# Terence-23/RayTracing-in-a-weekend

Measured on AMD Instinct MI355X. Metric: Msamples/s (rays x bounces) at 1920x1080x500spp, higher is better.
Workload: dtype f32

## Files before the change

### include/rtw.h

```cpp
#ifndef RTW_H
#define RTW_H

#include <stdint.h>
#include <stddef.h>

#ifdef __cplusplus
extern "C" {
#endif

#define RTW_ABI_VERSION 4

#define RTW_OK              0
#define RTW_E_INVALID      -1
#define RTW_E_NO_DEVICE    -2
#define RTW_E_HIP          -3
#define RTW_E_NOMEM        -4
#define RTW_E_UNSUPPORTED  -5
#define RTW_E_NO_SCENE     -6
#define RTW_E_INTERNAL     -7
#define RTW_E_RUNTIME_CONFLICT -8

enum {
    RTW_INTEGRATOR_GRADIENT = 0,
    RTW_INTEGRATOR_BG_COLOR = 1,
// ... 12 lines not shown
};

enum {
    RTW_ACCEL_BRUTE = 0,
    RTW_ACCEL_BVH   = 1
};


typedef struct RtwCamera {
    float origin[3];
    float u[3];
    float v[3];
    float pixel00[3];
    float delta_u[3];
    float delta_v[3];
    float lens_radius;
    float time0;
    float shutter;
} RtwCamera;

typedef struct RtwSphere {
    float center[3];
    float radius;
    float velocity[3];
    float col_mod[3];
    float tex_color[3];
    float metallicness;
    float opacity;
    float ir;
    float emitted[3];
    int32_t tex;
} RtwSphere;

typedef struct RtwTexture {
    uint32_t row;
    uint32_t col;
    uint32_t texel_offset;
    uint32_t emit_tex;
} RtwTexture;

typedef struct RtwQuad {
    float origin[3];
    float u[3];
    float v[3];
    float velocity[3];
    float tex_color[3];
    float metallicness;
    float opacity;
    float ir;
    float emitted[3];
    int32_t tex;
} RtwQuad;

enum { RTW_MEDIUM_SURFACE = 0, RTW_MEDIUM_CONST_DENSITY = 1 };
typedef struct RtwInstance {
    uint32_t first_sphere, n_spheres;
    uint32_t first_quad, n_quads;
    float translation[3];
    float rotation[3];
    float density;
    uint32_t medium;
} RtwInstance;

typedef struct RtwScene {
    const RtwSphere  *spheres;
    const RtwTexture *textures;
    const float      *texels;
    uint32_t n_spheres;
    uint32_t n_textures;
    uint32_t n_texels;
    float    background[3];
    const RtwQuad     *quads;
    const RtwInstance *instances;
    const RtwSphere   *inst_spheres;
    const RtwQuad     *inst_quads;
    uint32_t n_quads;
    uint32_t n_instances;
    uint32_t n_inst_spheres;
    uint32_t n_inst_quads;
} RtwScene;

typedef struct RtwParams {
    uint32_t width, height;
    uint32_t samples;
    uint32_t depth;
    float    gamma;
    float    mint, maxt;
    uint32_t integrator;
    uint32_t sampler;
    uint32_t accel;
    uint32_t flags;
    uint64_t seed;
    uint32_t row_block;
    uint32_t part_index;
    uint32_t part_count;
    uint32_t reserved;
} RtwParams;

#define RTW_FLAG_NONE            0u
#define RTW_FLAG_RECURSIVE_ORDER 1u
#define RTW_FLAG_CPP_DIELECTRIC  2u
#define RTW_FLAG_GLOBAL_NODES    4u
#define RTW_FLAG_CPP_DIFFUSE     8u
#define RTW_FLAG_CHUNK_SUMS     16u
#define RTW_SUM_CHUNK            4u
#define RTW_FLAG_MIXED_MATERIAL 32u

typedef struct RtwStats {
    uint64_t camera_rays;
    uint64_t segments;
    uint64_t sphere_tests;
    uint64_t node_tests;
    uint32_t nan_pixels;
    uint32_t rows;
    float    kernel_ms;
    float    total_ms;
    uint64_t phase_steps[6];
    uint64_t phase_lanes[6];
    uint64_t quad_tests;
    float    enqueue_ms;
    float    start_ms;
} RtwStats;

typedef struct rtw_ctx rtw_ctx;


int         rtw_abi_version(void);
int         rtw_device_count(void);
const char *rtw_strerror(int status);
int         rtw_last_hip_error(void);
int         rtw_hip_runtime_count(void);

int  rtw_ctx_create(int device, rtw_ctx **out);
void rtw_ctx_destroy(rtw_ctx *ctx);
int  rtw_ctx_set_stream(rtw_ctx *ctx, void *hip_stream);
int  rtw_ctx_set_scene(rtw_ctx *ctx, const RtwScene *scene, float t_begin, float t_end);
int  rtw_ctx_render(rtw_ctx *ctx, const RtwCamera *cam, const RtwParams *params,
                    float *out_rgb, RtwStats *stats);
int  rtw_ctx_render_multi(rtw_ctx *ctx, const RtwCamera *cam, const RtwParams *params, float fps,
                          uint32_t start_frame, uint32_t n_frames, float *out_rgb, RtwStats *stats);
int  rtw_render(const RtwCamera *cam, const RtwScene *scene, const RtwParams *params,
                float *out_rgb, RtwStats *stats);

enum {
    RTW_OPT_CHUNK_LEN        = 1,
    RTW_OPT_SAMPLE_BANK_GB   = 2,
    RTW_OPT_LDS_GEOM         = 3,
    RTW_OPT_BLOCKS_PER_CU    = 4,
    RTW_OPT_LIST_WALK_MAX    = 5,
    RTW_OPT_TILE_ORDER       = 6,
    RTW_OPT_GRAB_BLOCKS      = 7,
    RTW_OPT_TAIL_UNITS       = 9,
    RTW_OPT_SUB_QUEUES       = 8,
    RTW_OPT_GUIDED_LAYOUT    = 10
};
int  rtw_ctx_set_option(rtw_ctx *ctx, uint32_t key, double value);

typedef struct rtw_mgpu rtw_mgpu;
int  rtw_mgpu_create(const int *devices, uint32_t n_devices, rtw_mgpu **out);
void rtw_mgpu_destroy(rtw_mgpu *m);
int  rtw_mgpu_set_scene(rtw_mgpu *m, const RtwScene *scene, float t_begin, float t_end);
int  rtw_mgpu_set_option(rtw_mgpu *m, uint32_t key, double value);
int  rtw_mgpu_render(rtw_mgpu *m, const RtwCamera *cam, const RtwParams *params, float *out_rgb,
                     RtwStats *per_device, RtwStats *total);
int  rtw_render_multi_gpu(const int *devices, uint32_t n_devices, const RtwCamera *cam, const RtwScene *scene,
                          const RtwParams *params, float *out_rgb, RtwStats *per_device);

typedef struct RtwPerlin {
    float   ranvec[256][3];
    uint8_t perm_x[256], perm_y[256], perm_z[256];
} RtwPerlin;
typedef struct RtwTextureNoise {
    int32_t perlin;
    float   scale;
} RtwTextureNoise;
int rtw_perlin_new(uint64_t seed, RtwPerlin *out);
int rtw_perlin_eval(const RtwPerlin *t, const float *points, uint32_t n, uint32_t turb_depth, float *out);
int rtw_ctx_perlin_eval(rtw_ctx *ctx, const RtwPerlin *t, const float *points, uint32_t n, uint32_t turb_depth, float *out);
int rtw_ctx_set_texture_noise(rtw_ctx *ctx, const RtwPerlin *tables, uint32_t n_tables,
                              const RtwTextureNoise *per_texture, uint32_t n_textures);
int rtw_mgpu_set_texture_noise(rtw_mgpu *m, const RtwPerlin *tables, uint32_t n_tables,
                               const RtwTextureNoise *per_texture, uint32_t n_textures);

#define RTW_BILATERAL_MAX_SIZE 64u
enum { RTW_PROXIMITY_SQUARE = 0, RTW_PROXIMITY_EDGES = 1 };
enum { RTW_PIXELS_U8 = 0,
       RTW_PIXELS_F32_RUST2 = 1 };
typedef struct RtwBilateral {
    uint32_t size;
    uint32_t proximity;
    uint32_t in_format;
    float    avg_gradient;
} RtwBilateral;
typedef struct RtwFilterStats {
    float    avg_gradient;
    float    spatial;
    float    gradient_ms;
    float    table_ms;
    float    filter_ms;
    float    total_ms;
    uint64_t taps;
} RtwFilterStats;
int rtw_bilateral_filter(const void *in, uint32_t w, uint32_t h, const RtwBilateral *params, uint8_t *out, RtwFilterStats *stats);
int rtw_ctx_bilateral_filter(rtw_ctx *ctx, const void *in, uint32_t w, uint32_t h, const RtwBilateral *params, uint8_t *out,
                             RtwFilterStats *stats);

typedef struct RtwGuidedFilter {
    RtwBilateral base;
    float    sigma_depth;
    float    sigma_normal;
    uint32_t same_object;
} RtwGuidedFilter;
int rtw_guided_filter(const void *in, uint32_t w, uint32_t h, const float *depth, const float *normal, const int32_t *idx,
                      const RtwGuidedFilter *params, uint8_t *out, RtwFilterStats *stats);
int rtw_ctx_guided_filter(rtw_ctx *ctx, const void *in, uint32_t w, uint32_t h, const float *depth, const float *normal,
                          const int32_t *idx, const RtwGuidedFilter *params, uint8_t *out, RtwFilterStats *stats);

typedef struct RtwTriangle {
    float origin[3];
    float u[3];
    float v[3];
    float normal[3];
    float d;
    float w[3];
    float tex_color[3];
    float metallicness;
    float opacity;
    float ir;
    float emitted[3];
    int32_t tex;
} RtwTriangle;
int rtw_triangle_new(const float origin[3], const float u[3], const float v[3], const float *mat3, const float *emitted,
                     const float color[3], int32_t tex, RtwTriangle *out);
int rtw_ctx_set_triangles(rtw_ctx *ctx, const RtwTriangle *tris, uint32_t n);
int rtw_mgpu_set_triangles(rtw_mgpu *m, const RtwTriangle *tris, uint32_t n);
int rtw_triangle_bvh_validate(const RtwTriangle *tris, uint32_t n, uint32_t *n_nodes, uint32_t *depth, uint32_t *list_walk);
int rtw_triangle_hits(const RtwTriangle *tris, uint32_t n, const float *rays, uint32_t n_rays, float mint, float maxt,
                      float *t_out, int32_t *idx_out);
int rtw_ctx_triangle_hits(rtw_ctx *ctx, const float *rays, uint32_t n_rays, float mint, float maxt, uint32_t accel,
                          float *t_out, int32_t *idx_out, RtwStats *stats);

int rtw_depth_rays(const RtwCamera *cam, uint32_t width, uint32_t height, float *rays_out );
int rtw_ctx_scene_hits(rtw_ctx *ctx, const float *rays, uint32_t n_rays, float time, float mint, float maxt, uint32_t accel,
                       float *t_out, int32_t *idx_out, float *normal_out, RtwStats *stats);
int rtw_ctx_depth_map(rtw_ctx *ctx, const RtwCamera *cam, uint32_t width, uint32_t height, float time, float mint, float maxt,
                      uint32_t accel, float *depth_out, int32_t *idx_out, float *normal_out, RtwStats *stats);

#define RTW_MAX_LIGHTS 16u
enum { RTW_LIGHT_SPHERE = 0, RTW_LIGHT_QUAD = 1 };
typedef struct RtwLight {
    uint32_t kind;
    uint32_t index;
} RtwLight;
int rtw_ctx_set_lights(rtw_ctx *ctx, const RtwLight *lights, uint32_t n, float biased_weight);
int rtw_mgpu_set_lights(rtw_mgpu *m, const RtwLight *lights, uint32_t n, float biased_weight);
int rtw_lights_validate(const RtwScene *scene, const RtwLight *lights, uint32_t n);
int rtw_light_mid(const RtwScene *scene, const RtwLight *light, float mid[3]);
float rtw_material_pdf(const float mat3[3], const float p[3], const float n[3], const float dir_in[3], float time_in,
                       const float ray_o[3], const float ray_d[3], float ray_time);
int rtw_light_term(uint32_t integrator, float pdf, const float e[3], float t, const float dir[3], float biased_weight, float S[3], float *count);

int rtw_mixed_validate(const RtwScene *scene, const RtwParams *params, uint32_t n_triangles, uint32_t texture_noise);
int rtw_mixed_dir(float exp, float xi_phi, float xi_cos, const float n[3], float out_dir[3]);
int rtw_mixed_pdf(float exp, const float p[3], const float n[3], const float dir_in[3], const float ray_o[3], const float ray_d[3], float *out);
int rtw_pow_plain(const float *x, const float *y, size_t n, float *out);
int rtw_exp_plain(const float *x, size_t n, float *out);
int rtw_sin_plain(const float *phi, size_t n, float *out);
int rtw_cos_plain(const float *phi, size_t n, float *out);

int rtw_ctx_set_instance_rotations(rtw_ctx *ctx, const float (*quat)[4] , uint32_t n);
int rtw_mgpu_set_instance_rotations(rtw_mgpu *m, const float (*quat)[4], uint32_t n);
int rtw_instance_rotations_validate(const RtwScene *scene, const float (*quat)[4], uint32_t n);
int rtw_quat_rotate(const float q[4], const float v[3], float out[3]);
int rtw_quat_mul(const float a[4], const float b[4], float out[4]);
int rtw_quat_from_axis(float angle, const float axis[3], float out[4]);
int rtw_quat_from_euler(const float euler[3], float out[4]);


int rtw_viewport_new(uint32_t width, float aspect_ratio, const float *vfov, const float *origin,
                     const float *direction, const float *vup, const float *lens_radius,
                     RtwCamera *cam, uint32_t *height);
int rtw_viewport_new_from_res(uint32_t width, uint32_t height, const float *vfov, const float *origin,
                              const float *direction, const float *vup, const float *lens_radius,
                              RtwCamera *cam, uint32_t *height_out);
int rtw_camera2_new(float aspect, const float origin[3], const float vup[3], const float dir[3], float vfov,
                    float lens_radius, RtwCamera *cam);
int rtw_sphere_new(const float origin[3], float radius, const float *col_mod,
                   const float *mat3 , const float *velocity,
                   RtwSphere *out);
int rtw_sphere_new_with_texture(const float origin[3], float radius, const float *col_mod,
                                const float *mat3, const float *velocity, int32_t tex, RtwSphere *out);
int rtw_quad_new(const float origin[3], const float u[3], const float v[3], const float *mat3,
                 const float *emitted, const float color[3], RtwQuad *out);
int rtw_box_quads(const float a[3], const float b[3], const float *mat3, const float color[3], RtwQuad quads6[6]);
void rtw_vec3_rotated(const float v[3], const float rot[3], float out[3]);
int rtw_tile_order(uint32_t mode, uint32_t width, uint32_t height, const RtwCamera *cam, const RtwScene *scene,
                   uint32_t *order, uint32_t cap);
uint32_t rtw_part_rows(uint32_t height, uint32_t row_block, uint32_t part_index, uint32_t part_count);
void rtw_quantize_u8(const float *rgb, size_t n_values, uint8_t *out);
void rtw_quantize_u8_rust2(const float *rgb, size_t n_values, uint8_t *out);

size_t rtw_scene_to_json(const RtwScene *scene, char *buf, size_t cap);
int rtw_scene_from_json(const char *text, size_t len,
                        RtwSphere *spheres, uint32_t sphere_cap, uint32_t *n_spheres,
                        RtwTexture *textures, uint32_t texture_cap, uint32_t *n_textures,
                        float *texels, uint32_t texel_cap, uint32_t *n_texels);
int rtw_write_png_f32(const char *path, const float *rgb, uint32_t width, uint32_t height);
int rtw_write_ppm_f32(const char *path, const float *rgb, uint32_t width, uint32_t height);

// ... 31 lines not shown
```

### raytracing-in-a-weekend_amd/__init__.py

```python
from __future__ import annotations

import ctypes as C
import os
from typing import Optional, Sequence

import numpy as np

_HERE = os.path.dirname(os.path.abspath(__file__))
LIB_PATH = os.environ.get("RTW_HIP_LIB", os.path.join(_HERE, "librtw_hip.so"))

RTW_OK = 0
INTEGRATOR_GRADIENT, INTEGRATOR_BG_COLOR, INTEGRATOR_NORMAL, INTEGRATOR_FLAG, INTEGRATOR_RUST2 = 0, 1, 2, 3, 4
INTEGRATOR_LIGHT_CAST, INTEGRATOR_LIGHT_BIASED = 5, 6
LIGHT_SPHERE, LIGHT_QUAD = 0, 1
MAX_LIGHTS = 16
SAMPLER_ROW, SAMPLER_STRATIFIED, SAMPLER_CENTRES, SAMPLER_NO_RAND = 0, 1, 2, 3
ACCEL_BRUTE, ACCEL_BVH = 0, 1
FLAG_RECURSIVE_ORDER, FLAG_CPP_DIELECTRIC, FLAG_GLOBAL_NODES, FLAG_CPP_DIFFUSE, FLAG_CHUNK_SUMS = 1, 2, 4, 8, 16
FLAG_CPP = FLAG_CPP_DIELECTRIC | FLAG_CPP_DIFFUSE
FLAG_MIXED_MATERIAL = 32
OPT_CHUNK_LEN, OPT_SAMPLE_BANK_GB, OPT_LDS_GEOM, OPT_BLOCKS_PER_CU, OPT_LIST_WALK_MAX, OPT_TILE_ORDER, OPT_GRAB_BLOCKS, OPT_SUB_QUEUES = 1, 2, 3, 4, 5, 6, 7, 8
OPT_TAIL_UNITS = 9
OPT_GUIDED_LAYOUT = 10
SCENE_C1, SCENE_C2, SCENE_C4, SCENE_C5, SCENE_METAL_TEST, SCENE_QUAD_TEST, SCENE_PRESENTATION, SCENE_FIRST_FRAME = 1, 2, 4, 5, 6, 7, 8, 9
MEDIUM_SURFACE, MEDIUM_CONST_DENSITY = 0, 1
PROXIMITY_SQUARE, PROXIMITY_EDGES = 0, 1
PIXELS_U8, PIXELS_F32_RUST2 = 0, 1
BILATERAL_MAX_SIZE = 64

METALLIC_M = (1.0, 0.0, 1.0)
SCATTER_M = (0.0, 0.0, 1.0)
FUZZY3_M = (0.7, 0.0, 1.0)
GLASS_M = (1.0, 1.0, 1.5)
GLASSR_M = (1.0, 1.0, float(np.float32(1.0) / np.float32(1.5)))
EMPTY_M = SCATTER_M


class RtwError(RuntimeError):
    def __init__(self, status: int, what: str):
        super().__init__(f"{what}: status {status} ({_strerror(status)})")
        self.status = status


class RtwCamera(C.Structure):
    _fields_ = [("origin", C.c_float * 3), ("u", C.c_float * 3), ("v", C.c_float * 3),
                ("pixel00", C.c_float * 3), ("delta_u", C.c_float * 3), ("delta_v", C.c_float * 3),
                ("lens_radius", C.c_float), ("time0", C.c_float), ("shutter", C.c_float)]


class RtwSphere(C.Structure):
    _fields_ = [("center", C.c_float * 3), ("radius", C.c_float), ("velocity", C.c_float * 3),
                ("col_mod", C.c_float * 3), ("tex_color", C.c_float * 3),
                ("metallicness", C.c_float), ("opacity", C.c_float), ("ir", C.c_float),
                ("emitted", C.c_float * 3), ("tex", C.c_int32)]


class RtwTexture(C.Structure):
    _fields_ = [("row", C.c_uint32), ("col", C.c_uint32), ("texel_offset", C.c_uint32), ("emit_tex", C.c_uint32)]


class RtwQuad(C.Structure):
    _fields_ = [("origin", C.c_float * 3), ("u", C.c_float * 3), ("v", C.c_float * 3), ("velocity", C.c_float * 3),
                ("tex_color", C.c_float * 3), ("metallicness", C.c_float), ("opacity", C.c_float), ("ir", C.c_float),
                ("emitted", C.c_float * 3), ("tex", C.c_int32)]


class RtwTriangle(C.Structure):
    _fields_ = [("origin", C.c_float * 3), ("u", C.c_float * 3), ("v", C.c_float * 3), ("normal", C.c_float * 3), ("d", C.c_float),
                ("w", C.c_float * 3), ("tex_color", C.c_float * 3), ("metallicness", C.c_float), ("opacity", C.c_float), ("ir", C.c_float),
                ("emitted", C.c_float * 3), ("tex", C.c_int32)]


class RtwLight(C.Structure):
    _fields_ = [("kind", C.c_uint32), ("index", C.c_uint32)]


class RtwInstance(C.Structure):
    _fields_ = [("first_sphere", C.c_uint32), ("n_spheres", C.c_uint32), ("first_quad", C.c_uint32), ("n_quads", C.c_uint32),
                ("translation", C.c_float * 3), ("rotation", C.c_float * 3), ("density", C.c_float), ("medium", C.c_uint32)]


class RtwScene(C.Structure):
    _fields_ = [("spheres", C.POINTER(RtwSphere)), ("textures", C.POINTER(RtwTexture)),
                ("texels", C.POINTER(C.c_float)), ("n_spheres", C.c_uint32), ("n_textures", C.c_uint32),
                ("n_texels", C.c_uint32), ("background", C.c_float * 3),
                ("quads", C.POINTER(RtwQuad)), ("instances", C.POINTER(RtwInstance)),
                ("inst_spheres", C.POINTER(RtwSphere)), ("inst_quads", C.POINTER(RtwQuad)),
                ("n_quads", C.c_uint32), ("n_instances", C.c_uint32), ("n_inst_spheres", C.c_uint32), ("n_inst_quads", C.c_uint32)]


class RtwParams(C.Structure):
    _fields_ = [("width", C.c_uint32), ("height", C.c_uint32), ("samples", C.c_uint32), ("depth", C.c_uint32),
                ("gamma", C.c_float), ("mint", C.c_float), ("maxt", C.c_float),
                ("integrator", C.c_uint32), ("sampler", C.c_uint32), ("accel", C.c_uint32), ("flags", C.c_uint32),
                ("seed", C.c_uint64),
                ("row_block", C.c_uint32), ("part_index", C.c_uint32), ("part_count", C.c_uint32), ("reserved", C.c_uint32)]


class RtwStats(C.Structure):
    _fields_ = [("camera_rays", C.c_uint64), ("segments", C.c_uint64), ("sphere_tests", C.c_uint64),
                ("node_tests", C.c_uint64), ("nan_pixels", C.c_uint32), ("rows", C.c_uint32),
                ("kernel_ms", C.c_float), ("total_ms", C.c_float),
                ("phase_steps", C.c_uint64 * 6), ("phase_lanes", C.c_uint64 * 6), ("quad_tests", C.c_uint64),
                ("enqueue_ms", C.c_float), ("start_ms", C.c_float)]

    def as_dict(self):
        return {k: (list(getattr(self, k)) if k.startswith("phase_") else getattr(self, k)) for k, _ in self._fields_}


class RtwPerlin(C.Structure):
    _fields_ = [("ranvec", (C.c_float * 3) * 256), ("perm_x", C.c_uint8 * 256), ("perm_y", C.c_uint8 * 256), ("perm_z", C.c_uint8 * 256)]


class RtwTextureNoise(C.Structure):
    _fields_ = [("perlin", C.c_int32), ("scale", C.c_float)]


class RtwBilateral(C.Structure):
    _fields_ = [("size", C.c_uint32), ("proximity", C.c_uint32), ("in_format", C.c_uint32), ("avg_gradient", C.c_float)]


class RtwGuidedFilter(C.Structure):
    _fields_ = [("base", RtwBilateral), ("sigma_depth", C.c_float), ("sigma_normal", C.c_float), ("same_object", C.c_uint32)]


class RtwFilterStats(C.Structure):
    _fields_ = [("avg_gradient", C.c_float), ("spatial", C.c_float), ("gradient_ms", C.c_float), ("table_ms", C.c_float),
                ("filter_ms", C.c_float), ("total_ms", C.c_float), ("taps", C.c_uint64)]

    def as_dict(self):
        return {k: getattr(self, k) for k, _ in self._fields_}


_lib = None


def lib() -> C.CDLL:
    global _lib
    if _lib is not None:
        return _lib
    if not os.path.exists(LIB_PATH):
        raise ImportError(f"{LIB_PATH} is missing: run `python -c 'import __graft_entry__ as g; g.build()'` "
                          f"(hipcc --offload-arch=gfx950); there is no CPU fallback")
    L = C.CDLL(LIB_PATH)
    fp = C.POINTER(C.c_float)
    L.rtw_abi_version.restype = C.c_int
    L.rtw_device_count.restype = C.c_int
    L.rtw_strerror.restype = C.c_char_p
    L.rtw_strerror.argtypes = [C.c_int]
    L.rtw_last_hip_error.restype = C.c_int
    L.rtw_ctx_create.argtypes = [C.c_int, C.POINTER(C.c_void_p)]
    L.rtw_ctx_destroy.argtypes = [C.c_void_p]
    L.rtw_ctx_destroy.restype = None
    L.rtw_ctx_set_stream.argtypes = [C.c_void_p, C.c_void_p]
    L.rtw_ctx_set_scene.argtypes = [C.c_void_p, C.POINTER(RtwScene), C.c_float, C.c_float]
    L.rtw_ctx_render.argtypes = [C.c_void_p, C.POINTER(RtwCamera), C.POINTER(RtwParams), C.c_void_p, C.POINTER(RtwStats)]
    L.rtw_ctx_render_multi.argtypes = [C.c_void_p, C.POINTER(RtwCamera), C.POINTER(RtwParams), C.c_float, C.c_uint32, C.c_uint32,
                                       C.c_void_p, C.POINTER(RtwStats)]
    L.rtw_render.argtypes = [C.POINTER(RtwCamera), C.POINTER(RtwScene), C.POINTER(RtwParams), C.c_void_p, C.POINTER(RtwStats)]
    L.rtw_ctx_set_option.argtypes = [C.c_void_p, C.c_uint32, C.c_double]
    L.rtw_mgpu_create.argtypes = [C.POINTER(C.c_int), C.c_uint32, C.POINTER(C.c_void_p)]
    L.rtw_mgpu_destroy.argtypes = [C.c_void_p]
    L.rtw_mgpu_destroy.restype = None
    L.rtw_mgpu_set_scene.argtypes = [C.c_void_p, C.POINTER(RtwScene), C.c_float, C.c_float]
    L.rtw_mgpu_set_option.argtypes = [C.c_void_p, C.c_uint32, C.c_double]
    L.rtw_mgpu_render.argtypes = [C.c_void_p, C.POINTER(RtwCamera), C.POINTER(RtwParams), C.c_void_p, C.POINTER(RtwStats), C.POINTER(RtwStats)]
    L.rtw_render_multi_gpu.argtypes = [C.POINTER(C.c_int), C.c_uint32, C.POINTER(RtwCamera), C.POINTER(RtwScene), C.POINTER(RtwParams),
                                       C.c_void_p, C.POINTER(RtwStats)]
    L.rtw_viewport_new.argtypes = [C.c_uint32, C.c_float, fp, fp, fp, fp, fp, C.POINTER(RtwCamera), C.POINTER(C.c_uint32)]
    L.rtw_viewport_new_from_res.argtypes = [C.c_uint32, C.c_uint32, fp, fp, fp, fp, fp, C.POINTER(RtwCamera), C.POINTER(C.c_uint32)]
    L.rtw_sphere_new.argtypes = [fp, C.c_float, fp, fp, fp, C.POINTER(RtwSphere)]
    L.rtw_sphere_new_with_texture.argtypes = [fp, C.c_float, fp, fp, fp, C.c_int32, C.POINTER(RtwSphere)]
    L.rtw_vec3_rotated.restype = None
    L.rtw_vec3_rotated.argtypes = [fp, fp, fp]
    L.rtw_tile_order.argtypes = [C.c_uint32, C.c_uint32, C.c_uint32, C.POINTER(RtwCamera), C.POINTER(RtwScene), C.POINTER(C.c_uint32), C.c_uint32]
    L.rtw_part_rows.restype = C.c_uint32
    L.rtw_part_rows.argtypes = [C.c_uint32] * 4
    L.rtw_quantize_u8.restype = None
    L.rtw_quantize_u8.argtypes = [fp, C.c_size_t, C.POINTER(C.c_uint8)]
    L.rtw_camera2_new.argtypes = [C.c_float, fp, fp, fp, C.c_float, C.c_float, C.POINTER(RtwCamera)]
    L.rtw_quantize_u8_rust2.restype = None
    L.rtw_quantize_u8_rust2.argtypes = [fp, C.c_size_t, C.POINTER(C.c_uint8)]
    L.rtw_scene_to_json.restype = C.c_size_t
    L.rtw_scene_to_json.argtypes = [C.POINTER(RtwScene), C.c_char_p, C.c_size_t]
    L.rtw_scene_from_json.argtypes = [C.c_char_p, C.c_size_t, C.POINTER(RtwSphere), C.c_uint32, C.POINTER(C.c_uint32),
                                      C.POINTER(RtwTexture), C.c_uint32, C.POINTER(C.c_uint32), fp, C.c_uint32, C.POINTER(C.c_uint32)]
    L.rtw_write_png_f32.argtypes = [C.c_char_p, fp, C.c_uint32, C.c_uint32]
    L.rtw_write_ppm_f32.argtypes = [C.c_char_p, fp, C.c_uint32, C.c_uint32]
    L.rtw_bvh_validate.argtypes = [C.POINTER(RtwScene), C.c_float, C.c_float] + [C.POINTER(C.c_uint32)] * 4
    L.rtw_bvh_dump.argtypes = [C.POINTER(RtwScene), C.c_float, C.c_float, C.c_void_p, C.c_uint32, C.POINTER(C.c_uint32), C.POINTER(C.c_int32),
                               C.POINTER(C.c_uint32), C.POINTER(C.c_uint32), C.c_void_p, C.c_uint32, C.POINTER(C.c_uint32), C.c_void_p]
    L.rtw_bvh_query_host.argtypes = [C.POINTER(RtwScene), C.c_float, C.c_float, C.c_void_p, C.c_uint32, C.c_float, C.c_float, C.c_float,
                                     C.c_uint32, C.c_void_p, C.c_void_p, C.c_void_p]
    L.rtw_scene_generate.argtypes = [C.c_uint32, C.c_uint64, C.POINTER(RtwSphere), C.c_uint32, C.POINTER(C.c_uint32),
                                     C.POINTER(RtwTexture), C.c_uint32, C.POINTER(C.c_uint32),
                                     fp, C.c_uint32, C.POINTER(C.c_uint32)]
    L.rtw_scene_default_view.argtypes = [C.c_uint32, C.POINTER(RtwCamera), C.POINTER(RtwParams)]
    L.rtw_quad_new.argtypes = [fp, fp, fp, fp, fp, fp, C.POINTER(RtwQuad)]
    L.rtw_box_quads.argtypes = [fp, fp, fp, fp, C.POINTER(RtwQuad)]
    L.rtw_scene_generate_geom.argtypes = [C.c_uint32, C.c_uint64, C.POINTER(RtwSphere), C.POINTER(RtwQuad), C.POINTER(RtwInstance),
                                          C.POINTER(RtwSphere), C.POINTER(RtwQuad), C.POINTER(C.c_uint32), C.POINTER(C.c_uint32), fp]
    L.rtw_perlin_new.argtypes = [C.c_uint64, C.POINTER(RtwPerlin)]
    L.rtw_perlin_eval.argtypes = [C.POINTER(RtwPerlin), fp, C.c_uint32, C.c_uint32, fp]
    L.rtw_ctx_perlin_eval.argtypes = [C.c_void_p, C.POINTER(RtwPerlin), fp, C.c_uint32, C.c_uint32, fp]
    L.rtw_ctx_set_texture_noise.argtypes = [C.c_void_p, C.POINTER(RtwPerlin), C.c_uint32, C.POINTER(RtwTextureNoise), C.c_uint32]
    L.rtw_mgpu_set_texture_noise.argtypes = [C.c_void_p, C.POINTER(RtwPerlin), C.c_uint32, C.POINTER(RtwTextureNoise), C.c_uint32]
    L.rtw_bilateral_filter.argtypes = [C.c_void_p, C.c_uint32, C.c_uint32, C.POINTER(RtwBilateral), C.c_void_p, C.POINTER(RtwFilterStats)]
    L.rtw_ctx_bilateral_filter.argtypes = [C.c_void_p, C.c_void_p, C.c_uint32, C.c_uint32, C.POINTER(RtwBilateral), C.c_void_p,
                                           C.POINTER(RtwFilterStats)]
    L.rtw_guided_filter.argtypes = [C.c_void_p, C.c_uint32, C.c_uint32, C.c_void_p, C.c_void_p, C.c_void_p, C.POINTER(RtwGuidedFilter), C.c_void_p,
                                    C.POINTER(RtwFilterStats)]
    L.rtw_ctx_guided_filter.argtypes = [C.c_void_p, C.c_void_p, C.c_uint32, C.c_uint32, C.c_void_p, C.c_void_p, C.c_void_p,
                                        C.POINTER(RtwGuidedFilter), C.c_void_p, C.POINTER(RtwFilterStats)]
    L.rtw_triangle_new.argtypes = [fp, fp, fp, fp, fp, fp, C.c_int32, C.POINTER(RtwTriangle)]
    L.rtw_ctx_set_triangles.argtypes = [C.c_void_p, C.POINTER(RtwTriangle), C.c_uint32]
    L.rtw_mgpu_set_triangles.argtypes = [C.c_void_p, C.POINTER(RtwTriangle), C.c_uint32]
    L.rtw_triangle_bvh_validate.argtypes = [C.POINTER(RtwTriangle), C.c_uint32] + [C.POINTER(C.c_uint32)] * 3
    L.rtw_triangle_hits.argtypes = [C.POINTER(RtwTriangle), C.c_uint32, fp, C.c_uint32, C.c_float, C.c_float, fp, C.POINTER(C.c_int32)]
    L.rtw_ctx_triangle_hits.argtypes = [C.c_void_p, fp, C.c_uint32, C.c_float, C.c_float, C.c_uint32, fp, C.POINTER(C.c_int32),
                                        C.POINTER(RtwStats)]
    L.rtw_depth_rays.argtypes = [C.POINTER(RtwCamera), C.c_uint32, C.c_uint32, fp]
    L.rtw_ctx_scene_hits.argtypes = [C.c_void_p, C.c_void_p, C.c_uint32, C.c_float, C.c_float, C.c_float, C.c_uint32, C.c_void_p, C.c_void_p,
                                     C.c_void_p, C.POINTER(RtwStats)]
    L.rtw_ctx_depth_map.argtypes = [C.c_void_p, C.POINTER(RtwCamera), C.c_uint32, C.c_uint32, C.c_float, C.c_float, C.c_float, C.c_uint32,
                                    C.c_void_p, C.c_void_p, C.c_void_p, C.POINTER(RtwStats)]
    L.rtw_ctx_set_lights.argtypes = [C.c_void_p, C.POINTER(RtwLight), C.c_uint32, C.c_float]
    L.rtw_mgpu_set_lights.argtypes = [C.c_void_p, C.POINTER(RtwLight), C.c_uint32, C.c_float]
    L.rtw_lights_validate.argtypes = [C.POINTER(RtwScene), C.POINTER(RtwLight), C.c_uint32]
    L.rtw_light_mid.argtypes = [C.POINTER(RtwScene), C.POINTER(RtwLight), fp]
    L.rtw_material_pdf.argtypes = [fp, fp, fp, fp, C.c_float, fp, fp, C.c_float]
    L.rtw_material_pdf.restype = C.c_float
    L.rtw_light_term.argtypes = [C.c_uint32, C.c_float, fp, C.c_float, fp, C.c_float, fp, fp]
    L.rtw_mixed_validate.argtypes = [C.POINTER(RtwScene), C.POINTER(RtwParams), C.c_uint32, C.c_uint32]
    L.rtw_mixed_dir.argtypes = [C.c_float, C.c_float, C.c_float, fp, fp]
    L.rtw_mixed_pdf.argtypes = [C.c_float, fp, fp, fp, fp, fp, fp]
    L.rtw_ctx_set_instance_rotations.argtypes = [C.c_void_p, fp, C.c_uint32]
    L.rtw_mgpu_set_instance_rotations.argtypes = [C.c_void_p, fp, C.c_uint32]
    L.rtw_instance_rotations_validate.argtypes = [C.POINTER(RtwScene), fp, C.c_uint32]
    L.rtw_quat_rotate.argtypes = [fp, fp, fp]
    L.rtw_quat_mul.argtypes = [fp, fp, fp]
    L.rtw_quat_from_axis.argtypes = [C.c_float, fp, fp]
    L.rtw_quat_from_euler.argtypes = [fp, fp]
    L.rtw_pow_plain.argtypes = [fp, fp, C.c_size_t, fp]
    L.rtw_sin_plain.argtypes = [fp, C.c_size_t, fp]
    L.rtw_exp_plain.argtypes = [fp, C.c_size_t, fp]
    L.rtw_cos_plain.argtypes = [fp, C.c_size_t, fp]
    _lib = L
    return L


def _strerror(status: int) -> str:
    try:
        return lib().rtw_strerror(status).decode()
    except Exception:
        return "?"


def _check(status: int, what: str):
    if status != RTW_OK:
        raise RtwError(status, what)


def _f3(v) -> Optional[C.Array]:
    if v is None:
        return None
    return (C.c_float * 3)(*[float(x) for x in v])


def _fptr(arr):
    return None if arr is None else C.cast(arr, C.POINTER(C.c_float))


def _f1(v):
    return None if v is None else C.pointer(C.c_float(float(v)))


class Sphere:

    def __init__(self, pod: RtwSphere):
        self.pod = pod

    @staticmethod
    def new(origin, r, col_mod=None, mat=None) -> "Sphere":
        s = RtwSphere()
        _check(lib().rtw_sphere_new(_fptr(_f3(origin)), float(r), _fptr(_f3(col_mod)), _fptr(_f3(mat)), None, C.byref(s)), "rtw_sphere_new")
        return Sphere(s)

    @staticmethod
    def new_moving(origin, r, col_mod, mat, velocity) -> "Sphere":
        s = RtwSphere()
        _check(lib().rtw_sphere_new(_fptr(_f3(origin)), float(r), _fptr(_f3(col_mod)), _fptr(_f3(mat)), _fptr(_f3(velocity)), C.byref(s)), "rtw_sphere_new")
        return Sphere(s)

    @staticmethod
    def new_with_texture(origin, r, col_mod, mat, tex_index: int, velocity=None) -> "Sphere":
        s = RtwSphere()
        _check(lib().rtw_sphere_new_with_texture(_fptr(_f3(origin)), float(r), _fptr(_f3(col_mod)), _fptr(_f3(mat)),
                                                 _fptr(_f3(velocity)), int(tex_index), C.byref(s)), "rtw_sphere_new_with_texture")
        return Sphere(s)

    @staticmethod
    def with_albedo(origin, r, albedo, mat=None, velocity=None) -> "Sphere":
        sp = Sphere.new_moving(origin, r, (1.0, 1.0, 1.0), mat, velocity or (0.0, 0.0, 0.0))
        for k in range(3):
            sp.pod.tex_color[k] = float(albedo[k])
        return sp


class Quad:

    def __init__(self, pod: RtwQuad):
        self.pod = pod

# ... 388 lines not shown
    def new_sphere(spheres: Sequence) -> "Scene":
        return Scene(spheres)

    @staticmethod
    def new_quad(quads: Sequence) -> "Scene":
        return Scene((), quads=quads)

    @staticmethod
    def new(spheres: Sequence, quads: Sequence, instances: Sequence) -> "Scene":
        return Scene(spheres, quads=quads, instances=instances)

    @staticmethod
    def generate_geom(which: int, scene_seed: int = 42) -> "Scene":
        L = lib()
        counts = (C.c_uint32 * 5)()
        bg = (C.c_float * 3)()
        _check(L.rtw_scene_generate_geom(which, scene_seed, None, None, None, None, None, None, counts, bg), "rtw_scene_generate_geom")
        n = [int(x) for x in counts]
        sp, qd, ins = (RtwSphere * max(1, n[0]))(), (RtwQuad * max(1, n[1]))(), (RtwInstance * max(1, n[2]))()
        isp, iqd = (RtwSphere * max(1, n[3]))(), (RtwQuad * max(1, n[4]))()
        caps = (C.c_uint32 * 5)(*n)
        _check(L.rtw_scene_generate_geom(which, scene_seed, sp, qd, ins, isp, iqd, caps, counts, bg), "rtw_scene_generate_geom")
        sc = Scene(list(sp)[:n[0]], background=tuple(bg))
        sc._install_geom(list(qd)[:n[1]], list(ins)[:n[2]], list(isp)[:n[3]], list(iqd)[:n[4]])
        return sc

    def noise_pods(self):
        if not self.noise:
            return None
        tables, index = [], {}
        per = (RtwTextureNoise * max(1, self.n_textures))(*[RtwTextureNoise(-1, 1.0) for _ in range(max(1, self.n_textures))])
        for t, (perlin, scale) in self.noise.items():
            if not 0 <= int(t) < self.n_textures:
                raise RtwError(-1, f"noise for texture {t}: the scene has {self.n_textures} textures")
            if id(perlin) not in index:
                index[id(perlin)] = len(tables)
                tables.append(perlin.pod)
            per[int(t)] = RtwTextureNoise(index[id(perlin)], float(scale))
        tb = (RtwPerlin * len(tables))(*tables)
        return tb, len(tables), per, self.n_textures

    def to_json(self) -> str:
        n = lib().rtw_scene_to_json(C.byref(self.pod), None, 0)
        buf = C.create_string_buffer(n + 1)
        lib().rtw_scene_to_json(C.byref(self.pod), buf, n + 1)
        return buf.value.decode()

    @staticmethod
    def from_json(text: str) -> "Scene":
        L = lib()
        raw = text.encode()
        ns, nt, nx = C.c_uint32(), C.c_uint32(), C.c_uint32()
        _check(L.rtw_scene_from_json(raw, len(raw), None, 0, C.byref(ns), None, 0, C.byref(nt), None, 0, C.byref(nx)), "rtw_scene_from_json")
        sp = (RtwSphere * max(1, ns.value))()
        tx = (RtwTexture * max(1, nt.value))()
        tl = np.zeros((max(1, nx.value), 3), np.float32)
        _check(L.rtw_scene_from_json(raw, len(raw), sp, ns.value, C.byref(ns), tx, nt.value, C.byref(nt),
                                     tl.ctypes.data_as(C.POINTER(C.c_float)), nx.value, C.byref(nx)), "rtw_scene_from_json")
        return Scene._from_arrays(sp, ns.value, tx, nt.value, tl, nx.value)

    @staticmethod
    def _from_arrays(sp, ns, tx, nt, tl, nx) -> "Scene":
        sc = Scene(list(sp)[:ns])
        sc._textures, sc.n_textures, sc._texels, sc.n_texels = tx, nt, tl, nx
        sc.pod.textures = C.cast(tx, C.POINTER(RtwTexture))
        sc.pod.texels = tl.ctypes.data_as(C.POINTER(C.c_float))
        sc.pod.n_textures, sc.pod.n_texels = nt, nx
        return sc

    @staticmethod
    def generate(which: int, scene_seed: int = 42) -> "Scene":
        L = lib()
        ns, nt, nx = C.c_uint32(), C.c_uint32(), C.c_uint32()
        _check(L.rtw_scene_generate(which, scene_seed, None, 0, C.byref(ns), None, 0, C.byref(nt), None, 0, C.byref(nx)), "rtw_scene_generate")
        sp = (RtwSphere * max(1, ns.value))()
        tx = (RtwTexture * max(1, nt.value))()
        tl = np.zeros((max(1, nx.value), 3), np.float32)
        _check(L.rtw_scene_generate(which, scene_seed, sp, ns.value, C.byref(ns), tx, nt.value, C.byref(nt),
                                    tl.ctypes.data_as(C.POINTER(C.c_float)), nx.value, C.byref(nx)), "rtw_scene_generate")
        return Scene._from_arrays(sp, ns.value, tx, nt.value, tl, nx.value)


class Viewport:

    def __init__(self, cam: RtwCamera, width: int, height: int, samples: int, depth: int, gamma: float):
        self.cam, self.width, self.height = cam, width, height
        self.samples, self.depth, self.gamma = samples, depth, gamma
        self.shutter_speed, self.fps, self.frame = 0.0, 30.0, 0
        self.seed = 1
        self.mint, self.maxt = 0.001, 100000.0
        self.flags = 0

    @staticmethod
    def new(width, aspect_ratio, samples, depth, gamma, vfov=None, origin=None, direction=None, vup=None, msg=None, lens_radius=None):
        cam, h = RtwCamera(), C.c_uint32()
        _check(lib().rtw_viewport_new(int(width), float(aspect_ratio), _f1(vfov), _fptr(_f3(origin)), _fptr(_f3(direction)),
                                      _fptr(_f3(vup)), _f1(lens_radius), C.byref(cam), C.byref(h)), "rtw_viewport_new")
        return Viewport(cam, int(width), h.value, samples, depth, gamma)

    @staticmethod
    def new_from_res(width, height, samples, depth, gamma, vfov=None, origin=None, direction=None, vup=None, msg=None, lens_radius=None):
        cam, h = RtwCamera(), C.c_uint32()
        _check(lib().rtw_viewport_new_from_res(int(width), int(height), _f1(vfov), _fptr(_f3(origin)), _fptr(_f3(direction)),
                                               _fptr(_f3(vup)), _f1(lens_radius), C.byref(cam), C.byref(h)), "rtw_viewport_new_from_res")
        return Viewport(cam, int(width), h.value, samples, depth, gamma)

    def params(self, integrator=INTEGRATOR_GRADIENT, sampler=SAMPLER_STRATIFIED, accel=ACCEL_BVH) -> RtwParams:
        p = RtwParams()
        p.width, p.height, p.samples, p.depth = self.width, self.height, self.samples, self.depth
        p.gamma, p.mint, p.maxt = self.gamma, self.mint, self.maxt
        p.integrator, p.sampler, p.accel, p.flags, p.seed = integrator, sampler, accel, int(self.flags), self.seed
        p.row_block, p.part_index, p.part_count = 8, 0, 1
        return p

    def camera(self) -> RtwCamera:
        cam = RtwCamera.from_buffer_copy(self.cam)
        cam.time0 = float(np.float32(self.frame) / np.float32(self.fps))
        cam.shutter = float(self.shutter_speed)
        return cam

    def render(self, ray_color: int, scene: Scene, device: int = 0, accel: int = ACCEL_BVH) -> np.ndarray:
        return self._render(ray_color, SAMPLER_STRATIFIED, scene, device, accel)

    def async_render(self, ray_color: int, scene: Scene, device: int = 0, accel: int = ACCEL_BVH) -> np.ndarray:
        return self._render(ray_color, SAMPLER_ROW, scene, device, accel)

    def render_multi(self, ray_color: int, scene: Scene, device: int = 0, accel: int = ACCEL_BVH):
        start = getattr(self, "start_frame", 0)
        count = getattr(self, "number_of_frames", 1)
        with Renderer(device) as r:
            t0 = float(np.float32(start) / np.float32(self.fps))
            t1 = float(np.float32(start + max(count, 1) - 1) / np.float32(self.fps)) + float(self.shutter_speed)
            r.set_scene(scene, t0, t1)
            p = self.params(ray_color, SAMPLER_ROW, accel)
            video = np.empty((max(count, 0), self.height, self.width, 3), np.float32)
            st = (RtwStats * max(count, 1))()
            cam = self.camera()
            _check(lib().rtw_ctx_render_multi(r._h, C.byref(cam), C.byref(p), float(self.fps), int(start), int(count),
                                              C.c_void_p(video.ctypes.data), st), "rtw_ctx_render_multi")
        self.frame = start + max(count, 1) - 1
        return [video[i] for i in range(count)]

    def render_no_rand(self, ray_color: int, scene: Scene, device: int = 0, accel: int = ACCEL_BVH) -> np.ndarray:
        return self._render(ray_color, SAMPLER_NO_RAND, scene, device, accel)

    def _render(self, ray_color, sampler, scene, device, accel):
        with Renderer(device) as r:
            cam = self.camera()
            r.set_scene(scene, cam.time0, cam.time0 + cam.shutter)
            img, _ = r.render(cam, self.params(ray_color, sampler, accel))
        return img


class Renderer:

    def __init__(self, device: int = 0):
        self._h = C.c_void_p()
        _check(lib().rtw_ctx_create(int(device), C.byref(self._h)), "rtw_ctx_create")
        self._scene = None

    def close(self):
        if self._h:
            lib().rtw_ctx_destroy(self._h)
            self._h = C.c_void_p()

    def __enter__(self):
        return self

    def __exit__(self, *a):
        self.close()

    def __del__(self):
        try:
            self.close()
        except Exception:
            pass

    def set_stream(self, hip_stream: int):
        _check(lib().rtw_ctx_set_stream(self._h, C.c_void_p(hip_stream)), "rtw_ctx_set_stream")

    def set_scene(self, scene: Scene, t_begin: float = 0.0, t_end: float = 0.0):
        self._scene = scene
        _check(lib().rtw_ctx_set_scene(self._h, C.byref(scene.pod), float(t_begin), float(t_end)), "rtw_ctx_set_scene")
        nz = scene.noise_pods()
        if nz is not None:
            _check(lib().rtw_ctx_set_texture_noise(self._h, *nz), "rtw_ctx_set_texture_noise")
        if scene.n_triangles:
            _check(lib().rtw_ctx_set_triangles(self._h, scene.triangles, scene.n_triangles), "rtw_ctx_set_triangles")

    def set_triangles(self, triangles=None):
        if triangles is None or len(triangles) == 0:
            _check(lib().rtw_ctx_set_triangles(self._h, None, 0), "rtw_ctx_set_triangles")
            return
        self._tris = _triangle_array(triangles)
        _check(lib().rtw_ctx_set_triangles(self._h, *self._tris), "rtw_ctx_set_triangles")

    def set_lights(self, lights=None, biased_weight: float = 100.0):
        arr, n = _light_array(lights)
        _check(lib().rtw_ctx_set_lights(self._h, arr, n, float(biased_weight)), "rtw_ctx_set_lights")

    def set_instance_rotations(self, quats=None):
        ptr, n, _keep = _quat_array(quats)
        _check(lib().rtw_ctx_set_instance_rotations(self._h, ptr, n), "rtw_ctx_set_instance_rotations")

    def triangle_hits(self, rays, mint: float, maxt: float, accel: int = ACCEL_BVH):
        r = _rays(rays)
        t = np.empty(len(r), np.float32)
        idx = np.empty(len(r), np.int32)
        st = RtwStats()
        _check(lib().rtw_ctx_triangle_hits(self._h, r.ctypes.data_as(C.POINTER(C.c_float)), len(r), float(mint), float(maxt), int(accel),
                                           t.ctypes.data_as(C.POINTER(C.c_float)), idx.ctypes.data_as(C.POINTER(C.c_int32)), C.byref(st)),
               "rtw_ctx_triangle_hits")
        return t, idx, st

    def scene_hits(self, rays, mint: float, maxt: float, time: float = 0.0, accel: int = ACCEL_BVH, normals: bool = False):
        r = _rays(rays)
        t = np.empty(len(r), np.float32)
        idx = np.empty(len(r), np.int32)
        nrm = np.empty((len(r), 3), np.float32) if normals else None
        st = RtwStats()
        _check(lib().rtw_ctx_scene_hits(self._h, r.ctypes.data, len(r), float(time), float(mint), float(maxt), int(accel), t.ctypes.data,
                                        idx.ctypes.data, nrm.ctypes.data if normals else None, C.byref(st)), "rtw_ctx_scene_hits")
        return (t, idx, nrm, st) if normals else (t, idx, st)

    def depth_map(self, cam: RtwCamera, width: int, height: int, mint: float, maxt: float, time: float = 0.0, accel: int = ACCEL_BVH,
                  ids: bool = False, normals: bool = False):
        width, height = int(width), int(height)
        depth = np.empty((height, width), np.float32)
        idx = np.empty((height, width), np.int32) if ids else None
        nrm = np.empty((height, width, 3), np.float32) if normals else None
        st = RtwStats()
        _check(lib().rtw_ctx_depth_map(self._h, C.byref(cam), width, height, float(time), float(mint), float(maxt), int(accel), depth.ctypes.data,
                                       idx.ctypes.data if ids else None, nrm.ctypes.data if normals else None, C.byref(st)), "rtw_ctx_depth_map")
        return (depth,) + ((idx,) if ids else ()) + ((nrm,) if normals else ()) + (st,)

    def set_texture_noise(self, tables=None, n_tables: int = 0, per_texture=None, n_textures: int = 0):
        _check(lib().rtw_ctx_set_texture_noise(self._h, tables, n_tables, per_texture, n_textures), "rtw_ctx_set_texture_noise")

    def perlin_eval(self, perlin: PerlinNoise, p, depth: int = 0) -> np.ndarray:
        pts = np.ascontiguousarray(p, dtype=np.float32).reshape(-1, 3)
        out = np.empty(len(pts), np.float32)
        _check(lib().rtw_ctx_perlin_eval(self._h, C.byref(perlin.pod), pts.ctypes.data_as(C.POINTER(C.c_float)), len(pts), int(depth),
                                         out.ctypes.data_as(C.POINTER(C.c_float))), "rtw_ctx_perlin_eval")
        return out

    def set_option(self, key: int, value: float):
        _check(lib().rtw_ctx_set_option(self._h, int(key), float(value)), "rtw_ctx_set_option")

    def bilateral_filter(self, img, size: int, proximity: int = PROXIMITY_SQUARE, avg_gradient: float = 0.0, out=None, shape=None,
                         in_format: Optional[int] = None):
        src, w, h, fmt, _keep = _filter_source("bilateral_filter", img, shape, in_format)
        out, dst = _filter_out(out, h, w)
        st = RtwFilterStats()
        prm = RtwBilateral(int(size), int(proximity), fmt, float(avg_gradient))
        _check(lib().rtw_ctx_bilateral_filter(self._h, src, w, h, C.byref(prm), dst, C.byref(st)), "rtw_ctx_bilateral_filter")
        return out, st

    def guided_filter(self, img, size: int, depth=None, normal=None, ids=None, sigma_depth: float = 0.0, sigma_normal: float = 0.0,
                      same_object: bool = False, proximity: int = PROXIMITY_SQUARE, avg_gradient: float = 0.0, out=None, shape=None,
                      in_format: Optional[int] = None):
        src, w, h, fmt, _keep = _filter_source("guided_filter", img, shape, in_format)
        guides, _keep_g = _guide_pointers(h, w, depth, normal, ids)
        out, dst = _filter_out(out, h, w)
        st = RtwFilterStats()
        prm = RtwGuidedFilter(RtwBilateral(int(size), int(proximity), fmt, float(avg_gradient)), float(sigma_depth), float(sigma_normal),
                              int(same_object))
        _check(lib().rtw_ctx_guided_filter(self._h, src, w, h, *guides, C.byref(prm), dst, C.byref(st)), "rtw_ctx_guided_filter")
        return out, st

    def render(self, cam: RtwCamera, params: RtwParams, out=None):
        rows = lib().rtw_part_rows(params.height, params.row_block, params.part_index, params.part_count)
        st = RtwStats()
        if out is None:
            out = np.empty((rows, params.width, 3), np.float32)
        if isinstance(out, np.ndarray):
            assert out.dtype == np.float32 and out.flags["C_CONTIGUOUS"] and out.size == rows * params.width * 3
            ptr = C.c_void_p(out.ctypes.data)
        else:
            ptr = C.c_void_p(int(out))
        _check(lib().rtw_ctx_render(self._h, C.byref(cam), C.byref(params), ptr, C.byref(st)), "rtw_ctx_render")
        return out, st


class MultiRenderer:

    def __init__(self, devices: Sequence[int]):
        self._h = C.c_void_p()
        self.n = len(devices)
        arr = (C.c_int * max(1, self.n))(*[int(d) for d in devices])
        _check(lib().rtw_mgpu_create(arr, self.n, C.byref(self._h)), "rtw_mgpu_create")
        self._scene = None

    def close(self):
        if self._h:
            lib().rtw_mgpu_destroy(self._h)
            self._h = C.c_void_p()

    def __enter__(self):
        return self

    def __exit__(self, *a):
        self.close()

    def __del__(self):
        try:
            self.close()
        except Exception:
            pass

    def set_scene(self, scene: Scene, t_begin: float = 0.0, t_end: float = 0.0):
        self._scene = scene
        _check(lib().rtw_mgpu_set_scene(self._h, C.byref(scene.pod), float(t_begin), float(t_end)), "rtw_mgpu_set_scene")
        nz = scene.noise_pods()
        if nz is not None:
            _check(lib().rtw_mgpu_set_texture_noise(self._h, *nz), "rtw_mgpu_set_texture_noise")
        if scene.n_triangles:
            _check(lib().rtw_mgpu_set_triangles(self._h, scene.triangles, scene.n_triangles), "rtw_mgpu_set_triangles")

    def set_triangles(self, triangles=None):
        if triangles is None or len(triangles) == 0:
            _check(lib().rtw_mgpu_set_triangles(self._h, None, 0), "rtw_mgpu_set_triangles")
            return
        self._tris = _triangle_array(triangles)
        _check(lib().rtw_mgpu_set_triangles(self._h, *self._tris), "rtw_mgpu_set_triangles")

    def set_lights(self, lights=None, biased_weight: float = 100.0):
        arr, n = _light_array(lights)
        _check(lib().rtw_mgpu_set_lights(self._h, arr, n, float(biased_weight)), "rtw_mgpu_set_lights")

    def set_instance_rotations(self, quats=None):
        ptr, n, _keep = _quat_array(quats)
        _check(lib().rtw_mgpu_set_instance_rotations(self._h, ptr, n), "rtw_mgpu_set_instance_rotations")

    def set_option(self, key: int, value: float):
        _check(lib().rtw_mgpu_set_option(self._h, int(key), float(value)), "rtw_mgpu_set_option")

    def render(self, cam: RtwCamera, params: RtwParams, out=None):
        if out is None:
            out = np.empty((params.height, params.width, 3), np.float32)
        if isinstance(out, np.ndarray):
            assert out.dtype == np.float32 and out.flags["C_CONTIGUOUS"] and out.size == params.height * params.width * 3
            ptr = C.c_void_p(out.ctypes.data)
        else:
            ptr = C.c_void_p(int(out))
        per = (RtwStats * max(1, self.n))()
        tot = RtwStats()
        _check(lib().rtw_mgpu_render(self._h, C.byref(cam), C.byref(params), ptr, per, C.byref(tot)), "rtw_mgpu_render")
        return out, tot, list(per)[: self.n]


def default_view(which: int):
    cam, p = RtwCamera(), RtwParams()
    _check(lib().rtw_scene_default_view(which, C.byref(cam), C.byref(p)), "rtw_scene_default_view")
    return cam, p


def quantize_u8(img: np.ndarray) -> np.ndarray:
    a = np.ascontiguousarray(img, np.float32)
    out = np.empty(a.shape, np.uint8)
    lib().rtw_quantize_u8(a.ctypes.data_as(C.POINTER(C.c_float)), a.size, out.ctypes.data_as(C.POINTER(C.c_uint8)))
    return out


def camera2_new(aspect, origin, vup, direction, vfov, lens_radius) -> RtwCamera:
    cam = RtwCamera()
    _check(lib().rtw_camera2_new(float(aspect), _fptr(_f3(origin)), _fptr(_f3(vup)), _fptr(_f3(direction)), float(vfov),
                                 float(lens_radius), C.byref(cam)), "rtw_camera2_new")
    return cam


def quantize_u8_rust2(img: np.ndarray) -> np.ndarray:
    a = np.ascontiguousarray(img, np.float32)
    out = np.empty(a.shape, np.uint8)
    lib().rtw_quantize_u8_rust2(a.ctypes.data_as(C.POINTER(C.c_float)), a.size, out.ctypes.data_as(C.POINTER(C.c_uint8)))
    return out


def _pixel_format(img: np.ndarray) -> int:
    if img.dtype == np.uint8:
        return PIXELS_U8
    if img.dtype == np.float32:
        return PIXELS_F32_RUST2
    raise ValueError(f"bilateral_filter: dtype {img.dtype}, expected uint8 or float32")


def _filter_source(what, img, shape, in_format):
    if isinstance(img, np.ndarray):
        fmt = _pixel_format(img) if in_format is None else int(in_format)
        a = np.ascontiguousarray(img, np.uint8 if fmt == PIXELS_U8 else np.float32)
        if a.ndim != 3 or a.shape[2] != 3:
            raise ValueError(f"{what}: image of shape {a.shape}, expected [h][w][3]")
        return C.c_void_p(a.ctypes.data), a.shape[1], a.shape[0], fmt, a
    if shape is None or in_format is None:
        raise ValueError(f"{what}: a device pointer needs shape=(h, w) and in_format")
    h, w = (int(v) for v in shape)
    return C.c_void_p(int(img)), w, h, int(in_format), None


def _filter_out(out, h, w):
    if out is None:
# ... 63 lines not shown
```

### raytracing-in-a-weekend_amd/csrc/rtw_kernels.h

```cpp
#pragma once
#include "rtw_device.h"
#include "rtw_tri.h"
#include "rtw_light.h"
#include "rtw_mixed.h"
#include "rtw_host.h"

#define RTW_QUEUE_BYTES 4096u
#define RTW_QUEUE_STRIDE 256u
#ifndef RTW_SUB_SHIFT
#define RTW_SUB_SHIFT 3u
#endif
#ifndef RTW_BLOCK
#define RTW_BLOCK 256
#endif
#define RTW_N_STATS 64
#ifndef RTW_LIST_WALK_MAX_DEFAULT
#define RTW_LIST_WALK_MAX_DEFAULT 48u
#endif

namespace rtw {

struct DevBvh {
    const BvhNode *nodes;
    const BvhNode16 *nodes16;
    uint32_t n_nodes;
    const f4 *big_geom;
    const f4 *big_vel;
    const uint32_t *big_index;
    uint32_t n_big;
    uint32_t depth;
    int32_t root;
    float cx, cy, cz;
    float centre_radius;
    float r_max2;
    float inv_2rmin;
    float abs_max;
};

struct KArgs {
    RtwCamera cam;
    DevScene  sc;
    DevBvh    bvh;
    DevGeom   geom;
    uint32_t width, height;
    uint32_t k_base, k_end;
    uint32_t n_tiles;
    uint32_t chunk_len, n_chunks;
    uint32_t bank_len;
    uint32_t reg_q1, reg_q2;
    uint32_t reg_len[3], reg_nc[3];
    uint32_t flags;
    float *samples;
    uint32_t row_block, part_index, part_count;
    uint32_t tiles_x;
    uint32_t total_work;
    uint32_t sub_shift;
    uint32_t grab_shift, grab_max;
    const uint32_t *tile_order;
    uint32_t n_samples;
    uint32_t s_root;
    uint32_t sampler, integrator, depth;
    uint32_t has_textures;
    uint32_t lds_bytes;
    uint32_t lds_stack_off, lds_geom_off;
    uint32_t seed_lo, seed_hi;
    float inv_gamma, mint, maxt;
    float bg[3];
    float *out;
    uint32_t *queue;
    unsigned long long endtimes_ref;
    unsigned long long *stats;
    DevNoise noise;
    DevTris tris;
    DevLights lights;
    const f4 *inst_quats;
};

void launch_render(const KArgs &a, bool moving, uint32_t accel, uint32_t grid, hipStream_t stream);
void launch_perlin_eval(const RtwPerlin *t, const float *points, uint32_t n, uint32_t depth, float *out, hipStream_t stream);
void launch_tri_hits(const DevTris &T, const float *rays, uint32_t n, float mint, float maxt, float *t_out, int32_t *idx_out,
                     unsigned long long *counters, hipStream_t stream);
struct QueryArgs {
    DevScene sc;
    DevBvh   bvh;
    DevGeom  geom;
    DevTris  tris;
    const f4 *inst_quats;
    RtwCamera cam;
    uint32_t width, height;
    const float *rays;
    uint32_t n;
    uint32_t levels;
    float time, mint, maxt;
    float miss_t;
    float span;
    float *t_out;
    int32_t *idx_out;
    float *normal_out;
    unsigned long long *counters;
};
#define RTW_QUERY_SLOTS 64u
#define RTW_QUERY_STRIDE 16u
void launch_scene_hits(const QueryArgs &q, bool from_camera, bool tree, hipStream_t stream);
uint32_t kernel_blocks_per_cu(const KArgs &a, bool moving, uint32_t accel, bool lds_nodes);
bool kernel_has_lds_geom(const KArgs &a);
const void *kernel_id(const KArgs &a, bool moving, uint32_t accel, bool lds_nodes);

}
```

### raytracing-in-a-weekend_amd/csrc/rtw_kernels.hip

```cpp
#include "rtw_kernels.h"
#include <type_traits>

#ifndef RTW_MAX_TRIPS
#define RTW_MAX_TRIPS 0x30000000u
#endif

namespace rtw {


constexpr bool gradient_spec(int spec) { return spec >= 1 && spec <= 3; }
constexpr bool generic_spec(int spec) { return spec == 0 || spec == 7 || spec == 8 || spec == 9 || spec == 10 || spec == 11; }
constexpr bool light_spec(int spec) { return spec == 9 || spec == 10 || spec == 11; }
constexpr int mixed_spec(int spec) { return spec == 10 ? 1 : spec == 11 ? 2 : 0; }
constexpr bool quat_spec(int spec) { return spec == 11; }
constexpr bool noise_spec(int spec) { return spec == 7; }
constexpr bool tri_spec(int spec) { return spec == 8; }
template <int SPEC> __device__ __forceinline__ uint32_t integ(const KArgs &A) {
    return SPEC == 5 ? (uint32_t)RTW_INTEGRATOR_RUST2 : SPEC == 4 ? (uint32_t)RTW_INTEGRATOR_BG_COLOR : !generic_spec(SPEC) ? (uint32_t)RTW_INTEGRATOR_GRADIENT : A.integrator;
}
template <int SPEC> __device__ __forceinline__ uint32_t samp(const KArgs &A) {
    return SPEC == 6 ? (uint32_t)RTW_SAMPLER_STRATIFIED : SPEC == 5 ? (uint32_t)RTW_SAMPLER_CENTRES : !generic_spec(SPEC) ? (uint32_t)RTW_SAMPLER_ROW : A.sampler;
}

struct Pixel {
    uint32_t ij;
    uint32_t rng_base;
    uint32_t s;
    uint32_t slot;
};
__device__ __forceinline__ uint32_t px_i(const Pixel &px) { return px.ij & 0xFFFFu; }
__device__ __forceinline__ uint32_t px_j(const Pixel &px) { return px.ij >> 16; }
__device__ __forceinline__ uint32_t px_s(const Pixel &px) { return px.s & 0xFFFFFFu; }
__device__ __forceinline__ bool px_advance(Pixel &px) { px.s += 1u - (1u << 24); return px.s < (1u << 24); }

struct Path {
    v3 o, d;
    float tm;
    v3 thr;
    v3 L;
    uint32_t k;
    Rng rng;
    bool poison;
};

struct Reserve {
    uint32_t next, end;
    uint32_t limit;
    uint32_t sub, tries;
    uint32_t i0, k0;
    uint32_t s0, s1;
    uint32_t slot0;
#ifdef RTW_ENDTIMES
    unsigned long long t_dry;
#endif
};

struct SubQ { uint32_t t1, t2, b1, b2, total; };
__device__ __forceinline__ SubQ subq_layout(const KArgs &A, uint32_t sub) {
    const uint32_t up = (1u << A.sub_shift) - 1u - sub;
    SubQ q;
    q.t1 = (A.reg_q1 + up) >> A.sub_shift; q.t2 = (A.reg_q2 + up) >> A.sub_shift;
    const uint32_t t3 = (A.n_tiles + up) >> A.sub_shift;
    q.b1 = q.t1 * A.reg_nc[0]; q.b2 = q.b1 + (q.t2 - q.t1) * A.reg_nc[1];
    q.total = (q.b2 + (t3 - q.t2) * A.reg_nc[2]) * 64u;
    return q;
}

__device__ __forceinline__ bool fetch_pixel(const KArgs &A, bool need, Pixel &px, bool &exhausted, Reserve &rs) {
    const unsigned long long m = ballot64(need);
    if (m == 0ull) return false;
    if (rs.next == rs.end) {
        if (rs.end == rs.limit) {
            const uint32_t n_sub = 1u << A.sub_shift;
            const uint32_t leader = (uint32_t)__ffsll((long long)m) - 1u;
            bool got = false;
            while (rs.tries < n_sub) {
                const uint32_t total = subq_layout(A, rs.sub).total;
                uint32_t grab = 64u;
                if (rs.tries == 0u && rs.limit < total) {
                    grab = ((total - rs.limit) >> A.grab_shift) & ~63u;
                    grab = grab > A.grab_max ? A.grab_max : (grab < 64u ? 64u : grab);
                }
                uint32_t base = 0;
                if ((threadIdx.x & 63u) == leader) base = atomicAdd(A.queue + rs.sub * (RTW_QUEUE_STRIDE / 4u), grab);
                base = (uint32_t)__builtin_amdgcn_readlane((int)base, (int)leader);
                if (base < total) {
                    rs.next = base;
                    rs.limit = total - base > grab ? base + grab : total;
                    got = true;
                    break;
                }
                rs.sub = (rs.sub + 1u) & (n_sub - 1u); rs.tries++; rs.limit = 0u;
            }
            if (!got) {
                rs.next = rs.limit = 0u;
#ifdef RTW_ENDTIMES
                if (rs.t_dry == 0ull) rs.t_dry = wall_clock64();
#endif
            }
        }
        rs.end = rs.next + (rs.next < rs.limit ? 64u : 0u);
        if (rs.next < rs.limit) {
            uint32_t u = rs.next >> 6;
            const SubQ sq = subq_layout(A, rs.sub);
            uint32_t lt, chunk, len;
            if (u < sq.b1) { lt = u / A.reg_nc[0]; chunk = u - lt * A.reg_nc[0]; len = A.reg_len[0]; }
            else if (u < sq.b2) { u -= sq.b1; lt = u / A.reg_nc[1]; chunk = u - lt * A.reg_nc[1]; lt += sq.t1; len = A.reg_len[1]; }
            else { u -= sq.b2; lt = u / A.reg_nc[2]; chunk = u - lt * A.reg_nc[2]; lt += sq.t2; len = A.reg_len[2]; }
            const uint32_t qt = (lt << A.sub_shift) + rs.sub;
            const uint32_t tile = A.tile_order ? A.tile_order[qt] : qt;
            const uint32_t trow = tile / A.tiles_x, tcol = tile - trow * A.tiles_x;
            rs.i0 = tcol * 8u;
            rs.k0 = A.k_base + trow * 8u;
            rs.s0 = chunk * len;
            rs.s1 = rs.s0 + len < A.n_samples ? rs.s0 + len : A.n_samples;
            rs.slot0 = (A.bank_len ? tile * A.n_chunks + chunk : tile * A.n_samples + rs.s0) * 64u;
        }
    }
    const uint32_t avail = rs.end - rs.next;
    const uint32_t rank = __builtin_amdgcn_mbcnt_hi((uint32_t)(m >> 32), __builtin_amdgcn_mbcnt_lo((uint32_t)m, 0u));
    const uint32_t w = rs.next + rank;
    const uint32_t cnt = (uint32_t)__popcll(m);
    rs.next += cnt < avail ? cnt : avail;
    if (!need) return false;
    if (avail == 0u) { exhausted = true; return false; }
    if (rank >= avail) return false;
    const uint32_t p = w & 63u;
    const uint32_t i = rs.i0 + (p & 7u);
    const uint32_t k = rs.k0 + (p >> 3);
    if (!(i < A.width && k < A.k_end)) return false;
    uint32_t j = k;
    if (A.part_count > 1) {
        if (A.row_block == 8u) j = ((rs.k0 >> 3) * A.part_count + A.part_index) * 8u + (p >> 3);
        else j = ((k / A.row_block) * A.part_count + A.part_index) * A.row_block + (k % A.row_block);
    }
    px.ij = i | (j << 16);
    px.rng_base = rng_pixel_base(A.seed_lo, A.seed_hi, j * A.width + i);
    px.s = rs.s0 | ((rs.s1 - rs.s0) << 24);
    px.slot = rs.slot0 + (w & 63u);
    return rs.s0 < rs.s1;
}

struct CamRegs { RtwCamera c; };
typedef float f16v __attribute__((ext_vector_type(16)));
typedef float f8v __attribute__((ext_vector_type(8)));
static_assert(sizeof(RtwCamera) == 84 && offsetof(KArgs, cam) == 0, "start_path reads KArgs.cam as 16 + 8 dwords at offset 0");
__device__ __forceinline__ RtwCamera load_camera() {
    f16v lo; f8v hi;
    asm volatile("s_load_dwordx16 %0, %2, 0x0\n\ts_load_dwordx8 %1, %2, 0x40\n\ts_waitcnt lgkmcnt(0)"
                 : "=&s"(lo), "=&s"(hi) : "s"(__builtin_amdgcn_kernarg_segment_ptr()));
    RtwCamera c;
    c.origin[0] = lo[0]; c.origin[1] = lo[1]; c.origin[2] = lo[2]; c.u[0] = lo[3]; c.u[1] = lo[4]; c.u[2] = lo[5];
    c.v[0] = lo[6]; c.v[1] = lo[7]; c.v[2] = lo[8]; c.pixel00[0] = lo[9]; c.pixel00[1] = lo[10]; c.pixel00[2] = lo[11];
    c.delta_u[0] = lo[12]; c.delta_u[1] = lo[13]; c.delta_u[2] = lo[14]; c.delta_v[0] = lo[15]; c.delta_v[1] = hi[0]; c.delta_v[2] = hi[1];
    c.lens_radius = hi[2]; c.time0 = hi[3]; c.shutter = hi[4];
    return c;
}

template <int SPEC>
__device__ __forceinline__ void start_path(const KArgs &A, const Pixel &px, Path &pt, Cen *cn = nullptr) {
    RTW_CEN(cn, CEN_START_PATH);
    const RtwCamera cam = load_camera();
    const v3 cam_o = ld3(cam.origin), p00 = ld3(cam.pixel00), du = ld3(cam.delta_u), dv = ld3(cam.delta_v);
    pt.rng = rng_start(px.rng_base, px_s(px));
    pt.thr = mk(1.0f, 1.0f, 1.0f); pt.L = mk(0, 0, 0); pt.poison = false; pt.k = 0;
    v3 o, d; float tm = 0.0f;
    if (samp<SPEC>(A) == RTW_SAMPLER_NO_RAND) {
        o = cam_o;
        d = (p00 + du * (float)px_i(px)) + dv * (float)px_j(px);
    } else {
        float jx, jy, rx, ry;
        if (samp<SPEC>(A) == RTW_SAMPLER_CENTRES) {
            const uint32_t kx = px_s(px) / A.s_root, ly = px_s(px) % A.s_root;
            jx = ((float)px_i(px) + ((float)kx + 0.5f) / (float)A.s_root) / (float)A.width;
            jy = ((float)px_j(px) + ((float)ly + 0.5f) / (float)A.s_root) / (float)A.height;
            random_in_unit_disk(pt.rng, rx, ry, false, cn);
            o = cam_o + mk(rx, ry, 0.0f) * cam.lens_radius;
        } else {
            random_in_unit_disk(pt.rng, rx, ry, generic_spec(SPEC) && (A.flags & RTW_FLAG_CPP_DIFFUSE), cn);
            o = cam_o + (ld3(cam.u) * rx + ld3(cam.v) * ry) * cam.lens_radius;
            if (samp<SPEC>(A) == RTW_SAMPLER_ROW) {
                jx = rng_offset(pt.rng, (float)px_i(px));
                jy = rng_offset(pt.rng, (float)px_j(px));
                tm = cam.time0 + cam.shutter * rng_f32(pt.rng);
            } else {
                const uint32_t sx = px_s(px) / A.s_root, sy = px_s(px) % A.s_root;
                jx = (float)px_i(px) + (((float)sx + rng_f32(pt.rng)) / (float)A.s_root);
                jy = (float)px_j(px) + (((float)sy + rng_f32(pt.rng)) / (float)A.s_root);
            }
        }
        d = (p00 + du * jx) + dv * jy;
    }
    pt.o = o; pt.d = d; pt.tm = tm;
}

template <int SPEC>
__device__ __forceinline__ void shade_miss(const KArgs &A, Path &pt, v3 ud) {
    v3 miss;
    if (integ<SPEC>(A) == RTW_INTEGRATOR_BG_COLOR || integ<SPEC>(A) == RTW_INTEGRATOR_RUST2) miss = ld3(A.bg);
    else if (integ<SPEC>(A) == RTW_INTEGRATOR_FLAG) miss = mk(0.0f, 0.0f, 1.0f);
    else miss = sky_gradient(ud);
    if (gradient_spec(SPEC)) pt.L = miss * pt.thr;
    else pt.L = pt.L + miss * pt.thr;
}

template <int SPEC>
__device__ __forceinline__ bool shade_surface(const KArgs &A, Path &pt, v3 ud, v3 point, v3 normal, v3 cm, MatP mat, v3 emitted, Cen *cn = nullptr) {
    if (integ<SPEC>(A) == RTW_INTEGRATOR_NORMAL) {
        pt.L = mk(normal.x + 1.0f, normal.y + 1.0f, normal.z + 1.0f) * 0.5f;
        return true;
    }
    if (integ<SPEC>(A) == RTW_INTEGRATOR_FLAG && mat.metallicness != 1.0f) {
        pt.L = mk(1.0f, 1.0f, 0.0f) * pt.thr;
        return true;
    }
    if (integ<SPEC>(A) == RTW_INTEGRATOR_RUST2) {
        const v3 nd2 = on_hit_rust2(mat, normal, pt.d, pt.rng, A.flags);
        pt.L = pt.L + emitted * pt.thr;
        pt.thr = pt.thr * cm;
        pt.o = point; pt.d = nd2;
        pt.k++;
        if (pt.k >= A.depth) { pt.L = pt.L + ld3(A.bg) * pt.thr; return true; }
        return false;
    }
    float cos_theta;
    const v3 nd = on_hit(mat, point, normal, pt.d, ud, pt.rng, cos_theta, generic_spec(SPEC) ? A.flags : 0u, cn);
    if (integ<SPEC>(A) == RTW_INTEGRATOR_BG_COLOR) {
        const float pdf = cos_theta > 0.0f ? cos_theta * 0.318309886183790671538f : 0.0f;
        if (mat.metallicness != 1.0f && !(pdf > 0.0f)) pt.poison = true;
        pt.L = pt.L + emitted * pt.thr;
    }
    pt.thr = pt.thr * cm;
    pt.o = point; pt.d = nd;
    pt.k++;
    if (pt.k >= A.depth) {
        RTW_CEN(cn, CEN_DEPTH_END);
        if (integ<SPEC>(A) != RTW_INTEGRATOR_BG_COLOR) pt.L = mk(0, 0, 0);
        return true;
    }
    return false;
}

template <bool MOVING, int SPEC>
__device__ __forceinline__ bool shade_hit(const KArgs &A, Path &pt, v3 ud, int best, float best_t, Cen *cn = nullptr) {
    RTW_CEN(cn, CEN_HIT);
    const DevScene &sc = A.sc;
    f4 g = sc.geom[best];
    v3 c = mk(g.x, g.y, g.z);
    if (MOVING) { f4 vv = sc.vel[best]; c = c + mk(vv.x, vv.y, vv.z) * pt.tm; }
    const v3 point = pt.o + pt.d * best_t;
    const v3 normal = unit(point - c);
    const DevMat mat = sc.mat[best];
    v3 cm, emitted = ld3(mat.emitted);
    if ((generic_spec(SPEC) || SPEC == 5) && integ<SPEC>(A) == RTW_INTEGRATOR_RUST2 && mat.tex >= 0) rust2_sphere_color(sc, mat, normal, cm, emitted);
    else if constexpr (noise_spec(SPEC)) cm = sphere_albedo_noise(sc, A.noise, mat, normal, point);
    else cm = (SPEC == 1 || SPEC == 3) ? ld3(mat.cm) : sphere_albedo(sc, mat, normal);
    return shade_surface<SPEC>(A, pt, ud, point, normal, cm, mat_params(mat), emitted, cn);
}

template <bool MOVING, int SPEC>
__device__ __forceinline__ bool shade(const KArgs &A, Path &pt, int best, float best_t, Cen *cn = nullptr) {
    RTW_CEN(cn, CEN_INFLIGHT);
    const v3 ud = unit(pt.d);
    if (best < 0) { RTW_CEN(cn, CEN_MISS); shade_miss<SPEC>(A, pt, ud); return true; }
    return shade_hit<MOVING, SPEC>(A, pt, ud, best, best_t, cn);
}

template <bool MOVING, int SPEC>
__device__ __forceinline__ void shade_hit_first(const KArgs &A, Path &pt, v3 ud, int best, float best_t, bool &need_ball, v3 &nrm, float &metal, bool &front, Cen *cn = nullptr) {
    RTW_CEN(cn, CEN_HIT);
// ... 82 lines not shown

template <int MIXED>
__device__ __forceinline__ bool light_walks_on(const KArgs &A) {
    return MIXED ? A.integrator != RTW_INTEGRATOR_LIGHT_CAST : A.integrator == RTW_INTEGRATOR_LIGHT_BIASED;
}
template <int MIXED>
__device__ __forceinline__ bool mixed_surface(const KArgs &A, float opacity) {
    if (MIXED == 2) return (A.flags & RTW_FLAG_MIXED_MATERIAL) != 0u && opacity < 0.0f;
    return MIXED && opacity < 0.0f;
}
template <int MIXED>
__device__ __forceinline__ void light_surface(const KArgs &A, Path &pt, v3 point, v3 normal, v3 cm, const MatP m, v3 emitted, v3 din, LightPath &lp) {
    const bool biased = light_walks_on<MIXED>(A);
    lp.n = normal; lp.din = din; lp.tm = pt.tm;
    lp.metallicness = m.metallicness; lp.opacity = m.opacity; lp.ir = m.ir;
    lp.cm = cm; lp.e = emitted;
    lp.S = mk(0, 0, 0); lp.count = biased ? 1.0f : 0.0f;
    v3 scat = mk(0, 0, 0);
    if (biased) {
        if (mixed_surface<MIXED>(A, m.opacity)) {
            const float xi_phi = rng_f32(pt.rng), xi_cos = rng_f32(pt.rng);
            const lv3 dir = mixed_dir(m.ir, xi_phi, xi_cos, tol(normal));
            scat = mk(dir.x, dir.y, dir.z);
        } else {
            scat = on_hit_rust2(m, normal, din, pt.rng, A.flags);
        }
    }
    lp.scat = scat;
    pt.o = point;
}

__device__ __forceinline__ void light_ray(uint32_t i, Path &pt) {
    const f4 row = light_row((uint32_t)offsetof(KArgs, lights), i);
    const v3 mid = mk(row.x, row.y, row.z);
    const v3 to = mid - pt.o;
    pt.d = to / len(to);
    pt.tm = 0.0f;
}

template <bool MOVING, bool GEOM, int MIXED, bool QUAT>
__device__ __forceinline__ void light_result(const KArgs &A, uint32_t i, const Path &pt, int best, float best_t, LightPath &lp, uint32_t &n_sph, uint32_t &n_quad) {
    uint32_t code = best >= 0 ? (uint32_t)best : LIGHT_HIT_NONE;
    float t = best_t;
    if constexpr (GEOM) {
        float tg;
        uint32_t cg;
        if constexpr (QUAT) cg = shadow_geom_pick<true>(A.geom, pt.o, pt.d, pt.tm, A.mint, A.maxt, best >= 0, best_t, tg, n_sph, n_quad, A.inst_quats);
        else cg = shadow_geom_pick(A.geom, pt.o, pt.d, pt.tm, A.mint, A.maxt, best >= 0, best_t, tg, n_sph, n_quad);
        if (cg != LIGHT_HIT_NONE) { code = cg; t = tg; }
    }
    const f4 row = light_row((uint32_t)offsetof(KArgs, lights), i);
    const float code_bits = row.w;
    if (code != __float_as_uint(code_bits) || code >= LIGHT_HIT_NONE) return;
    v3 e;
    if (code & LIGHT_HIT_QUAD) {
        e = ld3(A.geom.quads[code & ~LIGHT_HIT_QUAD].emitted);
    } else {
        const DevMat mat = A.sc.mat[code];
        e = ld3(mat.emitted);
        if (mat.tex >= 0) {
            f4 g = A.sc.geom[code];
            v3 c = mk(g.x, g.y, g.z);
            if (MOVING) { f4 vv = A.sc.vel[code]; c = c + mk(vv.x, vv.y, vv.z) * pt.tm; }
            v3 cm_unused;
            rust2_sphere_color(A.sc, mat, unit((pt.o + pt.d * t) - c), cm_unused, e);
        }
    }
    float pdf;
    if (mixed_surface<MIXED>(A, lp.opacity)) pdf = mixed_pdf(lp.ir, tol(pt.o), tol(lp.n), tol(lp.din), tol(pt.o), tol(pt.d));
    else pdf = light_material_pdf(lp.metallicness, lp.opacity, lp.ir, tol(pt.o), tol(lp.n), tol(lp.din), lp.tm, tol(pt.o), tol(pt.d), pt.tm);
    lv3 S = tol(lp.S);
    light_add(light_walks_on<MIXED>(A), pdf, tol(e), t, tol(pt.d), A.lights.weight, S, lp.count);
    lp.S = mk(S.x, S.y, S.z);
}

template <int MIXED>
__device__ __forceinline__ bool light_finish(const KArgs &A, Path &pt, const LightPath &lp) {
    if (!light_walks_on<MIXED>(A)) {
        v3 c = mk(0, 0, 0);
        if (lp.count != 0.0f) c = (lp.S * lp.cm) / lp.count;
        pt.L = c + lp.e;
        return true;
    }
    pt.L = pt.L + pt.thr * ((lp.S * lp.cm) / lp.count + lp.e);
    pt.thr = pt.thr * (lp.cm / lp.count);
    pt.d = lp.scat; pt.tm = lp.tm;
    if (mixed_surface<MIXED>(A, lp.opacity)) pt.tm = 0.0f;
    pt.k++;
    if (pt.k >= A.depth) { pt.L = pt.L + ld3(A.bg) * pt.thr; return true; }
    return false;
}

template <bool MOVING, bool GEOM, int MIXED, bool QUAT>
__device__ __forceinline__ bool light_step_brute(const KArgs &A, Path &pt, int best, float best_t, uint32_t &n_seg, uint32_t &n_sph, uint32_t &n_quad) {
    v3 point, normal, cm, emitted, din; MatP m;
    if (!light_path_hit<MOVING, GEOM, QUAT>(A, pt, best, best_t, point, normal, cm, m, emitted, din, n_sph, n_quad)) {
        pt.L = pt.L + ld3(A.bg) * pt.thr;
        return true;
    }
    LightPath lp;
    light_surface<MIXED>(A, pt, point, normal, cm, m, emitted, din, lp);
    const uint32_t n = A.lights.n;
    for (uint32_t i = 0; i < n; ++i) {
        light_ray(i, pt);
        int sb; float st;
        closest_brute<MOVING>(A.sc, pt.o, pt.d, pt.tm, A.mint, A.maxt, sb, st);
        n_seg++;
        light_result<MOVING, GEOM, MIXED, QUAT>(A, i, pt, sb, st, lp, n_sph, n_quad);
    }
    return light_finish<MIXED>(A, pt, lp);
}

template <bool MOVING, bool GEOM, int MIXED, bool QUAT>
__device__ __forceinline__ bool light_step_bvh(const KArgs &A, Path &pt, LightPath &lp, uint32_t &fl, int best, float best_t, uint32_t &n_sph, uint32_t &n_quad) {
    const uint32_t n = A.lights.n;
    if (!(fl & LF_SHADOW)) {
        v3 point, normal, cm, emitted, din; MatP m;
        if (!light_path_hit<MOVING, GEOM, QUAT>(A, pt, best, best_t, point, normal, cm, m, emitted, din, n_sph, n_quad)) {
            pt.L = pt.L + ld3(A.bg) * pt.thr;
            return true;
        }
        light_surface<MIXED>(A, pt, point, normal, cm, m, emitted, din, lp);
        if (n == 0u) return light_finish<MIXED>(A, pt, lp);
        fl |= LF_SHADOW;
        light_ray(0u, pt);
        return false;
    }
    uint32_t i = (fl & LF_LIGHT_MASK) >> LF_LIGHT_SHIFT;
    light_result<MOVING, GEOM, MIXED, QUAT>(A, i, pt, best, best_t, lp, n_sph, n_quad);
    i++;
    if (i < n) { fl += 1u << LF_LIGHT_SHIFT; light_ray(i, pt); return false; }
    fl &= ~(LF_SHADOW | LF_LIGHT_MASK);
    return light_finish<MIXED>(A, pt, lp);
}

template <int SPEC>
__device__ __forceinline__ bool finish_path(const KArgs &A, Pixel &px, Path &pt, Cen *cn = nullptr) {
    RTW_CEN(cn, CEN_BANK);
    if (pt.poison) { const float qn = __builtin_nanf(""); pt.L = mk(qn, qn, qn); }
    float3 *dst = reinterpret_cast<float3 *>(A.samples + 3 * (size_t)px.slot);
    if (SPEC == 3 || (generic_spec(SPEC) && (A.flags & RTW_FLAG_CHUNK_SUMS))) {
        if (px_s(px) & (RTW_SUM_CHUNK - 1u)) {
            const float3 acc = *dst;
            pt.L = mk(acc.x, acc.y, acc.z) + pt.L;
        }
        *dst = make_float3(pt.L.x, pt.L.y, pt.L.z);
        return px_advance(px);
    }
    *dst = make_float3(pt.L.x, pt.L.y, pt.L.z);
    px.slot += 64u;
    return px_advance(px);
}

__global__ __launch_bounds__(RTW_BLOCK) void resolve_kernel(const KArgs A) {
    const uint32_t w = blockIdx.x * RTW_BLOCK + threadIdx.x;
    const uint32_t tile = w >> 6, p = w & 63u;
    uint32_t nan = 0;
    if (tile < A.n_tiles) {
        const uint32_t tcol = tile % A.tiles_x, trow = tile / A.tiles_x;
        const uint32_t i = tcol * 8u + (p & 7u), k = A.k_base + trow * 8u + (p >> 3);
        if (i < A.width && k < A.k_end) {
            v3 acc = mk(0, 0, 0);
            const uint32_t n_slots = A.bank_len ? A.n_chunks : A.n_samples;
            const float *src = A.samples + 3 * ((size_t)tile * n_slots * 64u + p);
            for (uint32_t q = 0; q < n_slots; q++) acc = acc + ld3(src + 3 * 64u * (size_t)q);
            v3 col = acc / (float)A.n_samples;
            if (A.inv_gamma != 1.0f) col = mk(powf(col.x, A.inv_gamma), powf(col.y, A.inv_gamma), powf(col.z, A.inv_gamma));
            *reinterpret_cast<float3 *>(A.out + 3 * ((size_t)k * A.width + i)) = make_float3(col.x, col.y, col.z);
            if (col.x != col.x || col.y != col.y || col.z != col.z) nan = 1;
        }
    }
    const unsigned long long m = ballot64(nan != 0);
    if ((threadIdx.x & 63u) == 0 && m) atomicAdd(&A.stats[4], (unsigned long long)__popcll(m));
}

__device__ __forceinline__ void flush_counters(const KArgs &A, uint32_t n_seg, uint32_t n_rays,
                                               unsigned long long tests, uint32_t n_nodes) {
    unsigned long long seg = n_seg, rays = n_rays, nodes = n_nodes;
    for (int off = 32; off > 0; off >>= 1) {
        seg += __shfl_down(seg, off);
        rays += __shfl_down(rays, off);
        nodes += __shfl_down(nodes, off);
        tests += __shfl_down(tests, off);
    }
    if ((threadIdx.x & 63u) == 0) {
        atomicAdd(&A.stats[0], rays);
        atomicAdd(&A.stats[1], seg);
        atomicAdd(&A.stats[2], tests);
        atomicAdd(&A.stats[3], nodes);
    }
}

__device__ __forceinline__ void flush_tests(const KArgs &A, uint32_t n) {
    unsigned long long q = n;
    for (int off = 32; off > 0; off >>= 1) q += __shfl_down(q, off);
    if ((threadIdx.x & 63u) == 0) atomicAdd(&A.stats[2], q);
}

__device__ __forceinline__ void tri_nodes_begin(const KArgs &A) {
    if (threadIdx.x == 0) *tri_node_counter(A.tris) = 0u;
    __syncthreads();
}
__device__ __forceinline__ void tri_nodes_end(const KArgs &A) {
    __syncthreads();
    if (threadIdx.x == 0) atomicAdd(&A.stats[3], (unsigned long long)*tri_node_counter(A.tris));
}

__device__ __forceinline__ void flush_quads(const KArgs &A, uint32_t n_quad) {
    unsigned long long q = n_quad;
    for (int off = 32; off > 0; off >>= 1) q += __shfl_down(q, off);
    if ((threadIdx.x & 63u) == 0) atomicAdd(&A.stats[14], q);
}

template <bool MOVING>
__device__ __forceinline__ void closest_brute(const DevScene &sc, v3 o, v3 d, float tm, float mint, float maxt,
                                              int &best, float &best_t) {
    cf4_ptr geom = (cf4_ptr)(uintptr_t)sc.geom;
    cf4_ptr vel = (cf4_ptr)(uintptr_t)sc.vel;
    const float a = dot(d, d);
    const float ra = rcp_refined(a);
    const bool a_plain = ballot64(!in_range(a, 0x1p-20f, 0x1p20f)) == 0ull;
    best = -1; best_t = 0.0f;
    const uint32_t n = sc.n;
    auto test = [&](f4 g, f4 vv, uint32_t s) {
        float cx = g.x, cy = g.y, cz = g.z;
        if (MOVING) { cx = cx + vv.x * tm; cy = cy + vv.y * tm; cz = cz + vv.z * tm; }
        float ocx = o.x - cx, ocy = o.y - cy, ocz = o.z - cz;
        float b = ocx * d.x + ocy * d.y + ocz * d.z;
        float c = (ocx * ocx + ocy * ocy + ocz * ocz) - g.w;
        float disc = b * b - a * c;
        if (!(disc < 0.0f)) {
            const float x = sphere_root(b, disc, a, ra, a_plain, mint);
            const bool take = !(x < mint || x > maxt) && (best < 0 || best_t > x);
            best = take ? (int)s : best; best_t = take ? x : best_t;
        }
    };
    const f4 zero = { 0, 0, 0, 0 };
    uint32_t s = 0;
    f4 n0 = zero, n1 = zero, n2 = zero, n3 = zero, w0 = zero, w1 = zero, w2 = zero, w3 = zero;
    if (n >= 4) {
        n0 = geom[0]; n1 = geom[1]; n2 = geom[2]; n3 = geom[3];
        if (MOVING) { w0 = vel[0]; w1 = vel[1]; w2 = vel[2]; w3 = vel[3]; }
    }
    for (; s + 4 <= n; s += 4) {
        const f4 g0 = n0, g1 = n1, g2 = n2, g3 = n3, v0 = w0, v1 = w1, v2 = w2, v3 = w3;
        if (s + 8 <= n) {
            n0 = geom[s + 4]; n1 = geom[s + 5]; n2 = geom[s + 6]; n3 = geom[s + 7];
            if (MOVING) { w0 = vel[s + 4]; w1 = vel[s + 5]; w2 = vel[s + 6]; w3 = vel[s + 7]; }
        }
        test(g0, v0, s); test(g1, v1, s + 1); test(g2, v2, s + 2); test(g3, v3, s + 3);
    }
    for (; s < n; ++s) test(geom[s], MOVING ? vel[s] : zero, s);
}

#ifndef RTW_GEOM_BRUTE_WAVES
#define RTW_GEOM_BRUTE_WAVES 4
#endif
template <bool MOVING, int SPEC, bool GEOM>
__global__ __launch_bounds__(RTW_BLOCK, GEOM ? RTW_GEOM_BRUTE_WAVES : 1) void render_brute(const KArgs A) {
    bool dead = false, have = false, newpath = false;
    Pixel px; px.ij = px.rng_base = px.s = px.slot = 0;
    Reserve rs; rs.next = rs.end = rs.limit = rs.i0 = rs.k0 = rs.s0 = rs.s1 = rs.slot0 = rs.tries = 0; rs.sub = blockIdx.x & ((1u << A.sub_shift) - 1u);
#ifdef RTW_ENDTIMES
    rs.t_dry = 0ull;
#endif
    Path pt; pt.o = pt.d = pt.L = mk(0, 0, 0); pt.thr = mk(1, 1, 1); pt.tm = 0; pt.k = 0; pt.poison = false; pt.rng.state = 0; pt.rng.inc = 1;
    uint32_t n_seg = 0, n_rays = 0, n_isph = 0, n_quad = 0;
    uint32_t trips = 0; bool aborted = false;
    if constexpr (tri_spec(SPEC)) tri_nodes_begin(A);

    for (;;) {
        if (fetch_pixel(A, !have && !dead, px, dead, rs)) { have = true; newpath = true; }
        if (ballot64(!dead) == 0ull) break;
        if (++trips > RTW_MAX_TRIPS) { aborted = true; break; }
        if (have && newpath) { newpath = false; start_path<SPEC>(A, px, pt); n_rays++; }
        if (have) {
            bool finished;
            if (light_spec(SPEC) ? (A.depth == 0 && (mixed_spec(SPEC) ? A.integrator != RTW_INTEGRATOR_LIGHT_CAST : A.integrator == RTW_INTEGRATOR_LIGHT_BIASED))
                                 : (generic_spec(SPEC) && A.depth == 0 && A.integrator != RTW_INTEGRATOR_NORMAL)) {
                pt.L = (light_spec(SPEC) || A.integrator == RTW_INTEGRATOR_RUST2) ? ld3(A.bg) : mk(0, 0, 0); finished = true;
            } else {
                int best; float best_t;
                closest_brute<MOVING>(A.sc, pt.o, pt.d, pt.tm, A.mint, A.maxt, best, best_t);
                n_seg++;
                if constexpr (light_spec(SPEC)) finished = light_step_brute<MOVING, GEOM, mixed_spec(SPEC), quat_spec(SPEC)>(A, pt, best, best_t, n_seg, n_isph, n_quad);
                else finished = GEOM ? shade_geom<MOVING, SPEC>(A, pt, best, best_t, n_isph, n_quad) : shade<MOVING, SPEC>(A, pt, best, best_t);
            }
            if (finished) {
                if (finish_path<SPEC>(A, px, pt)) have = false;
                else newpath = true;
            }
        }
    }
    if constexpr (tri_spec(SPEC)) tri_nodes_end(A);
    flush_counters(A, n_seg, n_rays, (unsigned long long)n_seg * A.sc.n + n_isph, 0);
    if (GEOM) flush_quads(A, n_quad);
    if (aborted && (threadIdx.x & 63u) == 0) atomicAdd(&A.stats[23], 1ull);
}


template <bool MOVING>
__device__ __forceinline__ void exact_sphere(f4 g, f4 vv, uint32_t s, v3 o, v3 d, float tm, float a, float ra, bool a_plain, float mint, float maxt,
                                             int &best, float &best_t) {
    float cx = g.x, cy = g.y, cz = g.z;
    if (MOVING) { cx = cx + vv.x * tm; cy = cy + vv.y * tm; cz = cz + vv.z * tm; }
    float ocx = o.x - cx, ocy = o.y - cy, ocz = o.z - cz;
    float b = ocx * d.x + ocy * d.y + ocz * d.z;
    float c = (ocx * ocx + ocy * ocy + ocz * ocz) - g.w;
    float disc = b * b - a * c;
    if (!(disc < 0.0f)) {
        const float x = sphere_root(b, disc, a, ra, a_plain, mint);
        const bool take = !(x < mint || x > maxt) && (x < best_t || (x == best_t && s < (uint32_t)best));
        best = take ? (int)s : best; best_t = take ? x : best_t;
    }
}

#define RTW_KU 1.4305115e-6f
#ifndef RTW_S_HI
#define RTW_S_HI 52u
#endif
#ifndef RTW_TRAV_UNROLL
#define RTW_TRAV_UNROLL 3
#endif
#ifndef RTW_T_LO
#define RTW_T_LO 6u
#endif
// ... 83 lines not shown
    const float M = (__builtin_fabsf(ex) + __builtin_fabsf(ey) + __builtin_fabsf(ez)) * 1.0001f + bv.centre_radius;
#endif
    const float q = (M * M + bv.r_max2) * RTW_KU;
    const float sq_q = __builtin_amdgcn_sqrtf(q) * 1.0001f;
    float rho = fminf(q * bv.inv_2rmin, sq_q);
    rho = rho * 1.0001f + 4.8e-7f * (fabsf(o.x) + fabsf(o.y) + fabsf(o.z) + bv.abs_max);
    tr.tau_t = sq_q * 1.0002f * __builtin_amdgcn_rsqf(tr.a) + 1e-30f;
    float ix = __builtin_amdgcn_rcpf(d.x), iy = __builtin_amdgcn_rcpf(d.y), iz = __builtin_amdgcn_rcpf(d.z);
#ifdef RTW_BEGIN_GUARD_PER_LANE
    if (!(fabsf(d.x) >= 1e-20f)) ix = copysignf(1e20f, d.x);
    if (!(fabsf(d.y) >= 1e-20f)) iy = copysignf(1e20f, d.y);
    if (!(fabsf(d.z) >= 1e-20f)) iz = copysignf(1e20f, d.z);
#else
    if (ballot64(!(fminf(fminf(fabsf(d.x), fabsf(d.y)), fabsf(d.z)) >= 1e-20f) || d.x != d.x || d.y != d.y || d.z != d.z) != 0ull) {
        if (!(fabsf(d.x) >= 1e-20f)) ix = copysignf(1e20f, d.x);
        if (!(fabsf(d.y) >= 1e-20f)) iy = copysignf(1e20f, d.y);
        if (!(fabsf(d.z) >= 1e-20f)) iz = copysignf(1e20f, d.z);
    }
#endif
    tr.ix = ix; tr.iy = iy; tr.iz = iz;
    if (sizeof(S) == 2) {
        const float ox = -o.x * ix, oy = -o.y * iy, oz = -o.z * iz;
        const float rx = rho * fabsf(ix), ry = rho * fabsf(iy), rz = rho * fabsf(iz);
        tr.kpx = ox - rx; tr.kpy = oy - ry; tr.kpz = oz - rz;
        tr.kmx = ox + rx; tr.kmy = oy + ry; tr.kmz = oz + rz;
        const uint32_t ID = 0x03020100u, FLIP = 0x03020100u ^ 0x01000302u;
        tr.selx = ID ^ ((uint32_t)((int32_t)__float_as_uint(ix) >> 31) & FLIP);
        tr.sely = ID ^ ((uint32_t)((int32_t)__float_as_uint(iy) >> 31) & FLIP);
        tr.selz = ID ^ ((uint32_t)((int32_t)__float_as_uint(iz) >> 31) & FLIP);
    } else {
        tr.kpx = -(o.x + rho) * ix; tr.kpy = -(o.y + rho) * iy; tr.kpz = -(o.z + rho) * iz;
        tr.kmx = -(o.x - rho) * ix; tr.kmy = -(o.y - rho) * iy; tr.kmz = -(o.z - rho) * iz;
    }
    tr.lo_lim = A.mint - tr.tau_t;
    tr.hi_lim = tr.best_t + tr.tau_t;
}


template <class S>
__device__ __forceinline__ void trav_pop(Trav &tr) {
    tr.node = (int)(uint32_t)lds_get<typename std::make_unsigned<S>::type>(tr.sp);
    tr.sp -= RTW_BLOCK * (uint32_t)sizeof(S);
}

template <class S> __device__ __forceinline__ int entry_to_node(uint32_t raw);
template <> __device__ __forceinline__ int entry_to_node<short>(uint32_t raw) { return (int)(raw & 0xFFFFu); }
template <> __device__ __forceinline__ int entry_to_node<int>(uint32_t raw) { return (int)raw; }

template <class S>
__device__ __forceinline__ void trav_descend(Trav &tr, float e0, float x0, float e1, float x1,
                                             uint32_t c0, uint32_t c1, uint32_t popped) {
    const float n0 = fmaxf(e0, tr.lo_lim), n1 = fmaxf(e1, tr.lo_lim);
    const bool h0 = n0 <= fminf(x0, tr.hi_lim);
    const bool h1 = n1 <= fminf(x1, tr.hi_lim);
    const bool le = n0 <= n1;
    const bool both = h0 && h1, none = !(h0 || h1);
    const bool near0 = h0 && (!h1 || le);
    const uint32_t level = RTW_BLOCK * (uint32_t)sizeof(S);
    if (sizeof(S) == 2) {
        const uint64_t H0 = __builtin_amdgcn_ballot_w64(h0), H1 = __builtin_amdgcn_ballot_w64(h1), LE = __builtin_amdgcn_ballot_w64(le);
        const bool far0 = __builtin_amdgcn_inverse_ballot_w64(~H0 | (H1 & ~LE));
        const uint32_t nf = __builtin_amdgcn_alignbit(c0, c0, far0 ? 16u : 0u);
        lds_put<unsigned short>(tr.sp + level, (unsigned short)(nf >> 16));
        tr.node = entry_to_node<S>(none ? popped : nf);
    } else {
        lds_put<S>(tr.sp + level, (S)(near0 ? c1 : c0));
        tr.node = entry_to_node<S>(none ? popped : (near0 ? c0 : c1));
    }
    tr.sp = (tr.sp + (both ? level : 0u)) - (none ? level : 0u);
}

typedef unsigned int u4 __attribute__((ext_vector_type(4)));
typedef unsigned int u3 __attribute__((ext_vector_type(3)));
typedef unsigned int u32a2 __attribute__((aligned(2)));
__device__ __forceinline__ float h_lo(unsigned int w) { return (float)__builtin_bit_cast(_Float16, (unsigned short)(w & 0xFFFFu)); }
__device__ __forceinline__ float h_hi(unsigned int w) { return (float)__builtin_bit_cast(_Float16, (unsigned short)(w >> 16)); }

__device__ __forceinline__ void trav_node_lds(const u4 *lnodes, Trav &tr) {
    const uint32_t popped = lds_get<unsigned short>(tr.sp);
    const uint32_t at = (uint32_t)tr.node;
    const u4 r0 = lds_get<u4>(at);
    const u3 r1 = lds_get<u3>(at + 16u);
#ifdef RTW_LDS_PROBE
    {
        const uint32_t pa = (uint32_t)tr.node * 32u + ((tr.selx & 1u) << RTW_LDS_PROBE_SH);
        #pragma unroll
        for (int k = 0; k < RTW_LDS_PROBE; k++) { const uint32_t x = lds_get<u32a2>(pa + 4u * k); asm volatile("" :: "v"(x)); }
    }
#endif
    const uint32_t c0 = r1.z, c1 = 0;
    const uint32_t ax = __builtin_amdgcn_perm(r0.x, r0.x, tr.selx), ay = __builtin_amdgcn_perm(r0.y, r0.y, tr.sely), az = __builtin_amdgcn_perm(r0.z, r0.z, tr.selz);
    const uint32_t bx = __builtin_amdgcn_perm(r0.w, r0.w, tr.selx), by = __builtin_amdgcn_perm(r1.x, r1.x, tr.sely), bz = __builtin_amdgcn_perm(r1.y, r1.y, tr.selz);
    const float e0 = fmaxf(fmaxf(__builtin_fmaf(h_lo(ax), tr.ix, tr.kpx), __builtin_fmaf(h_lo(ay), tr.iy, tr.kpy)), __builtin_fmaf(h_lo(az), tr.iz, tr.kpz));
    const float x0 = fminf(fminf(__builtin_fmaf(h_hi(ax), tr.ix, tr.kmx), __builtin_fmaf(h_hi(ay), tr.iy, tr.kmy)), __builtin_fmaf(h_hi(az), tr.iz, tr.kmz));
    const float e1 = fmaxf(fmaxf(__builtin_fmaf(h_lo(bx), tr.ix, tr.kpx), __builtin_fmaf(h_lo(by), tr.iy, tr.kpy)), __builtin_fmaf(h_lo(bz), tr.iz, tr.kpz));
    const float x1 = fminf(fminf(__builtin_fmaf(h_hi(bx), tr.ix, tr.kmx), __builtin_fmaf(h_hi(by), tr.iy, tr.kmy)), __builtin_fmaf(h_hi(bz), tr.iz, tr.kmz));
    trav_descend<short>(tr, e0, x0, e1, x1, c0, c1, popped);
}

__device__ __forceinline__ void trav_node(const DevBvh &bv, Trav &tr) {
    const uint32_t popped = lds_get<uint32_t>(tr.sp);
    const f4 *np = (const f4 *)(bv.nodes + tr.node);
    const f4 n0 = np[0], n1 = np[1], n2 = np[2];
    const uint32_t c0 = (uint32_t)bv.nodes[tr.node].c0, c1 = (uint32_t)bv.nodes[tr.node].c1;
    float t1, t2;
    t1 = __builtin_fmaf(n0.x, tr.ix, tr.kpx); t2 = __builtin_fmaf(n0.w, tr.ix, tr.kmx);
    float e0 = fminf(t1, t2), x0 = fmaxf(t1, t2);
    t1 = __builtin_fmaf(n0.y, tr.iy, tr.kpy); t2 = __builtin_fmaf(n1.x, tr.iy, tr.kmy);
    e0 = fmaxf(e0, fminf(t1, t2)); x0 = fminf(x0, fmaxf(t1, t2));
    t1 = __builtin_fmaf(n0.z, tr.iz, tr.kpz); t2 = __builtin_fmaf(n1.y, tr.iz, tr.kmz);
    e0 = fmaxf(e0, fminf(t1, t2)); x0 = fminf(x0, fmaxf(t1, t2));
    t1 = __builtin_fmaf(n1.z, tr.ix, tr.kpx); t2 = __builtin_fmaf(n2.y, tr.ix, tr.kmx);
    float e1 = fminf(t1, t2), x1 = fmaxf(t1, t2);
    t1 = __builtin_fmaf(n1.w, tr.iy, tr.kpy); t2 = __builtin_fmaf(n2.z, tr.iy, tr.kmy);
    e1 = fmaxf(e1, fminf(t1, t2)); x1 = fminf(x1, fmaxf(t1, t2));
    t1 = __builtin_fmaf(n2.x, tr.iz, tr.kpz); t2 = __builtin_fmaf(n2.w, tr.iz, tr.kmz);
    e1 = fmaxf(e1, fminf(t1, t2)); x1 = fminf(x1, fmaxf(t1, t2));
    trav_descend<int>(tr, e0, x0, e1, x1, c0, c1, popped);
}

#ifdef RTW_STAMP
#define RTW_SUB_STAMP(k) do { asm volatile("s_waitcnt vmcnt(0) lgkmcnt(0)" ::: "memory"); const unsigned long long t_now = __builtin_amdgcn_s_memtime(); sub[k] += t_now - t_sub; t_sub = t_now; } while (0)
#else
#define RTW_SUB_STAMP(k) do { } while (0)
#endif
#ifndef RTW_BVH_WAVES
#define RTW_BVH_WAVES 4
#endif
template <bool MOVING, class S>
__device__ __forceinline__ void wild_ray_query(const KArgs &A, const Path &pt, Trav &tr, uint32_t &n_tests) {
    const float m = (__builtin_fabsf(pt.o.x) + __builtin_fabsf(pt.o.y) + __builtin_fabsf(pt.o.z)) +
                    (__builtin_fabsf(pt.d.x) + __builtin_fabsf(pt.d.y) + __builtin_fabsf(pt.d.z));
    if (m < 0x1p60f) return;
    closest_brute<MOVING>(A.sc, pt.o, pt.d, pt.tm, A.mint, A.maxt, tr.best, tr.best_t);
    tr.node = (int)Code<S>::END;
    n_tests += A.sc.n - A.bvh.n_big;
}

#ifndef RTW_BVH_WAVES_GEOM
#define RTW_BVH_WAVES_GEOM 2
#endif
#ifndef RTW_BVH_WAVES_GEOM_SPEC
#define RTW_BVH_WAVES_GEOM_SPEC 5
#endif
#ifndef RTW_BVH_WAVES_SPEC
#define RTW_BVH_WAVES_SPEC 7
#endif
#ifndef RTW_BVH_WAVES_SPEC2
#define RTW_BVH_WAVES_SPEC2 RTW_BVH_WAVES_SPEC
#endif
#ifndef RTW_BVH_WAVES_FOLDED
#define RTW_BVH_WAVES_FOLDED RTW_BVH_WAVES
#endif
constexpr bool two_halves_step(int spec, bool geom, bool moving) {
#ifdef RTW_NO_TWO_HALVES
    return false;
#else
    return gradient_spec(spec) && !geom && !(moving && spec == 2);
#endif
}
template <bool MOVING, int NODES, int SPEC, bool GEOM>
__global__ __launch_bounds__(RTW_BLOCK, GEOM ? (!generic_spec(SPEC) ? RTW_BVH_WAVES_GEOM_SPEC : RTW_BVH_WAVES_GEOM) : (two_halves_step(SPEC, GEOM, MOVING) ? (SPEC == 2 ? RTW_BVH_WAVES_SPEC2 : RTW_BVH_WAVES_SPEC) : (gradient_spec(SPEC) ? RTW_BVH_WAVES_SPEC2 : (!generic_spec(SPEC) ? RTW_BVH_WAVES_FOLDED : RTW_BVH_WAVES)))) void render_bvh(const KArgs A) {
    constexpr bool LDSN = NODES != 0, geom_in_lds = NODES == 2;
    typedef typename std::conditional<LDSN, short, int>::type stack_t;
    extern __shared__ __attribute__((aligned(16))) unsigned char lds_raw[];
    *(stack_t *)(lds_raw + A.lds_stack_off + threadIdx.x * (uint32_t)sizeof(stack_t)) = (stack_t)Code<stack_t>::END;
    u4 *lnodes = (u4 *)lds_raw;
    if (LDSN && lds_addr(lds_raw) != 0u) { if (threadIdx.x == 0) atomicAdd(&A.stats[23], 1ull); return; }
    f4 *lgeom = (f4 *)(lds_raw + A.lds_geom_off);
    const DevScene &sc = A.sc;
    if (LDSN) {
        const u4 *src = (const u4 *)A.bvh.nodes16;
        for (uint32_t i = threadIdx.x; i < A.bvh.n_nodes * 2u; i += RTW_BLOCK) lnodes[i] = src[i];
        if (geom_in_lds) for (uint32_t i = threadIdx.x; i < sc.n; i += RTW_BLOCK) lgeom[i] = sc.geom[i];
        __syncthreads();
    }
    if constexpr (tri_spec(SPEC)) tri_nodes_begin(A);

    enum : uint32_t { F_HAVE = 1u,
                      F_INFLIGHT = 2u,
                      F_NEWPATH = 4u,
                      F_DONE = 8u,
                      F_K_SHIFT = 8u };
    uint32_t fl = 0u;
    Pixel px; px.ij = px.rng_base = px.s = px.slot = 0;
    Reserve rs; rs.next = rs.end = rs.limit = rs.i0 = rs.k0 = rs.s0 = rs.s1 = rs.slot0 = rs.tries = 0; rs.sub = blockIdx.x & ((1u << A.sub_shift) - 1u);
#ifdef RTW_ENDTIMES
    rs.t_dry = 0ull;
#endif
    Path pt; pt.o = pt.d = pt.L = mk(0, 0, 0); pt.thr = mk(1, 1, 1); pt.tm = 0; pt.k = 0; pt.poison = false; pt.rng.state = 0; pt.rng.inc = 1;
    typename std::conditional<light_spec(SPEC), LightPath, char>::type lp{};
    Trav tr; tr.node = (int)Code<stack_t>::END; tr.sp = 0; tr.best = -1; tr.best_t = 0; tr.a = tr.ra = 1; tr.ix = tr.iy = tr.iz = 0;
    tr.kpx = tr.kpy = tr.kpz = tr.kmx = tr.kmy = tr.kmz = 0; tr.selx = tr.sely = tr.selz = 0; tr.tau_t = tr.lo_lim = tr.hi_lim = 0;
    uint32_t w_seg = 0, w_rays = 0;
    uint32_t t_lo = RTW_T_LO;
    uint32_t trips = 0; bool aborted = false;
    bool a_plain = true;
    uint32_t n_isph = 0, n_quad = 0;
    uint32_t c_steps[3] = { 0, 0, 0 };
    uint32_t c_lanes[3] = { 0, 0, 0 };
#ifdef RTW_STAMP
    unsigned long long c_time[3] = { 0, 0, 0 };
    unsigned long long sub[5] = { 0, 0, 0, 0, 0 }, t_sub = 0;
#endif
#ifdef RTW_CENSUS
    Cen cen_store; for (int k = 0; k < CEN_N; k++) cen_store.n[k] = cen_store.w[k] = 0u;
    Cen *const cn = &cen_store;
#else
    Cen *const cn = nullptr;
#endif

#ifdef RTW_ENDTIMES
    const unsigned long long t_wave_start = __builtin_amdgcn_s_memtime();
    const unsigned long long rt_wave_start = wall_clock64();
    uint32_t dry_trips = 0, dry_steps[3] = { 0, 0, 0 }, dry_lanes[3] = { 0, 0, 0 };
    uint32_t dry_queries = 0;
#endif
    for (;;) {
        uint32_t nT = lanes_in(in_trav<stack_t>(tr.node));
        const uint32_t nL = lanes_in(in_leaf<stack_t>(tr.node));
        const uint32_t nS = lanes_in(in_shade<stack_t>(tr.node));
        if ((nT | nL | nS) == 0u) break;
        if (++trips > RTW_MAX_TRIPS) { aborted = true; break; }
        RTW_CEN(cn, CEN_BIG_ROOT);
        const bool run_shade = nS >= RTW_S_HI || (nT < t_lo && nL < t_lo && nS > 0u);
        const bool run_leaf = nL > nT;
#ifdef RTW_ENDTIMES
        if (rs.t_dry) {
            dry_trips++;
            const int ph = run_shade ? 2 : (run_leaf ? 1 : 0);
            dry_steps[ph]++; dry_lanes[ph] += ph == 2 ? nS : (ph == 1 ? nL : nT);
            if (run_shade && in_shade<stack_t>(tr.node) && (fl & F_INFLIGHT)) dry_queries++;
        }
#endif
#ifdef RTW_STAMP
        const unsigned long long t_begin = __builtin_amdgcn_s_memtime();
        const int which = run_shade ? 2 : (run_leaf ? 1 : 0);
#endif
        bool burst = false;
        if (run_shade) {
            c_steps[2]++; c_lanes[2] += nS;
            bool need_unit = false, started = false, a_odd = false;
            const bool shading = in_shade<stack_t>(tr.node);
            w_seg += (uint32_t)__popcll(ballot64(shading && (fl & F_INFLIGHT) != 0u));
#ifdef RTW_STAMP
            t_sub = t_begin;
#endif
            if constexpr (two_halves_step(SPEC, GEOM, MOVING)) {
            bool need_ball = false, need_disk = false, front = false;
            v3 nrm, ud; float metal;
            bool hit = false;
            if (shading) {
                RTW_CEN(cn, CEN_SHADING);
                if (fl & F_INFLIGHT) {
                    fl &= ~F_INFLIGHT;
                    RTW_CEN(cn, CEN_INFLIGHT);
                    ud = unit(pt.d);
                    if (tr.best < 0) { RTW_CEN(cn, CEN_MISS); fl |= F_DONE; }
                    else if ((fl >> F_K_SHIFT) + 1u >= A.depth) { RTW_CEN(cn, CEN_DEPTH_END); fl |= F_DONE; }
                    else { hit = true; fl += 1u << F_K_SHIFT; }
                }
            }
            RTW_SUB_STAMP(0);
            if (shading) {
                if (fl & F_DONE) {
                    fl &= ~F_DONE;
                    if (tr.best < 0) shade_miss<SPEC>(A, pt, ud); else pt.L = mk(0, 0, 0);
                    if (finish_path<SPEC>(A, px, pt, cn)) fl &= ~F_HAVE; else fl |= F_NEWPATH;
                }
                need_unit = (fl & F_HAVE) == 0u;
                if (need_unit) RTW_CEN(cn, CEN_NEED_UNIT);
            }
            bool exhausted = false;
            const bool got = fetch_pixel(A, need_unit, px, exhausted, rs);
            if (ballot64(exhausted) != 0ull) t_lo = RTW_T_LO_DRAIN;
            RTW_SUB_STAMP(1);
            if (shading) {
                if (got) fl |= F_HAVE | F_NEWPATH;
                if (exhausted) tr.node = (int)Code<stack_t>::DEAD;
                if ((fl & F_HAVE) && (fl & F_NEWPATH)) { fl &= F_HAVE | F_INFLIGHT | F_DONE; start_path_first(px, pt, cn); need_disk = true; started = true; }
            }
            if (hit) shade_hit_first<MOVING, SPEC>(A, pt, ud, tr.best, tr.best_t, need_ball, nrm, metal, front, cn);
            float sx, sy, sz, sl2;
            sample_ball_or_disk(pt.rng, need_ball || need_disk, need_ball, sx, sy, sz, sl2, cn);
            if (need_ball) pt.d = on_hit_second(metal, nrm, pt.d, front, mk(sx, sy, sz), sl2);
            if (need_disk) start_path_second(px, pt, sx, sy);
            RTW_SUB_STAMP(2);
            if (shading && (fl & F_HAVE)) {
                trav_begin<MOVING, stack_t>(A, pt, tr, lds_addr(lds_raw) + A.lds_stack_off + threadIdx.x * (uint32_t)sizeof(stack_t), a_plain, a_odd, cn);
                fl |= F_INFLIGHT;
            }
            RTW_SUB_STAMP(3);
            } else {
            if (shading) {
                RTW_CEN(cn, CEN_SHADING);
                if (fl & F_INFLIGHT) {
                    fl &= ~F_INFLIGHT;
                    bool done;
                    if constexpr (light_spec(SPEC)) done = light_step_bvh<MOVING, GEOM, mixed_spec(SPEC), quat_spec(SPEC)>(A, pt, lp, fl, tr.best, tr.best_t, n_isph, n_quad);
                    else done = GEOM ? shade_geom<MOVING, SPEC>(A, pt, tr.best, tr.best_t, n_isph, n_quad) : shade<MOVING, SPEC>(A, pt, tr.best, tr.best_t, cn);
                    if (done) fl |= F_DONE;
                }
            }
            RTW_SUB_STAMP(0);
            if (shading) {
                if (fl & F_DONE) { fl &= ~F_DONE; if (finish_path<SPEC>(A, px, pt, cn)) fl &= ~F_HAVE; else fl |= F_NEWPATH; }
                need_unit = (fl & F_HAVE) == 0u;
                if (need_unit) RTW_CEN(cn, CEN_NEED_UNIT);
            }
            bool exhausted = false;
            const bool got = fetch_pixel(A, need_unit, px, exhausted, rs);
            if (ballot64(exhausted) != 0ull) t_lo = RTW_T_LO_DRAIN;
            RTW_SUB_STAMP(1);
#ifdef RTW_STAMP
            if (shading) {
                if (got) fl |= F_HAVE | F_NEWPATH;
                if (exhausted) tr.node = (int)Code<stack_t>::DEAD;
                if ((fl & F_HAVE) && (fl & F_NEWPATH)) { fl &= ~F_NEWPATH; start_path<SPEC>(A, px, pt); started = true; }
            }
            RTW_SUB_STAMP(2);
#endif
            if (shading) {
                if (got) fl |= F_HAVE | F_NEWPATH;
                if (exhausted) tr.node = (int)Code<stack_t>::DEAD;
                if (fl & F_HAVE) {
                    if (fl & F_NEWPATH) { fl &= ~F_NEWPATH; start_path<SPEC>(A, px, pt, cn); started = true; }
                    if (light_spec(SPEC) ? (A.depth == 0 && (mixed_spec(SPEC) ? A.integrator != RTW_INTEGRATOR_LIGHT_CAST : A.integrator == RTW_INTEGRATOR_LIGHT_BIASED))
                                         : (generic_spec(SPEC) && A.depth == 0 && A.integrator != RTW_INTEGRATOR_NORMAL)) {
                        pt.L = (light_spec(SPEC) || A.integrator == RTW_INTEGRATOR_RUST2) ? ld3(A.bg) : mk(0, 0, 0);
                        fl |= F_DONE;
                    } else {
                        trav_begin<MOVING, stack_t>(A, pt, tr, lds_addr(lds_raw) + A.lds_stack_off + threadIdx.x * (uint32_t)sizeof(stack_t), a_plain, a_odd, cn);
                        if constexpr (GEOM || light_spec(SPEC)) wild_ray_query<MOVING, stack_t>(A, pt, tr, n_isph);
                        fl |= F_INFLIGHT;
                    }
                }
            }
            RTW_SUB_STAMP(3);
            }
            w_rays += (uint32_t)__popcll(ballot64(started));
            if (ballot64(a_odd) != 0ull) a_plain = false;
#ifndef RTW_STAMP
            nT = lanes_in(in_trav<stack_t>(tr.node)); burst = nT >= 33u;
#endif
        } else {
            burst = !run_leaf;
            if (run_leaf) {
                c_steps[1]++; c_lanes[1] += nL;
                if (in_leaf<stack_t>(tr.node)) {
                    const uint32_t s = leaf_sphere<stack_t>(tr.node);
                    const f4 gs = geom_in_lds ? lgeom[s] : sc.geom[s];
                    exact_sphere<MOVING>(gs, MOVING ? sc.vel[s] : f4{ 0, 0, 0, 0 }, s, pt.o, pt.d, pt.tm, tr.a, tr.ra, a_plain, A.mint, A.maxt, tr.best, tr.best_t);
                    tr.hi_lim = tr.best_t + tr.tau_t;
                    trav_pop<stack_t>(tr);
                }
#ifndef RTW_STAMP
                nT = lanes_in(in_trav<stack_t>(tr.node)); burst = nT >= 33u;
#endif
            }
        }
        if (burst) {
            static_assert(RTW_S_HI > 31u && RTW_T_LO <= 33u, "the shortcut below assumes the thresholds of the scheduler");
            uint32_t live = nT;
            for (;;) {
                uint32_t b_steps = 0, b_lanes = 0;
                for (int u = 0; u < RTW_TRAV_UNROLL; u++) {
                    b_steps++; b_lanes += live;
                    if (in_trav<stack_t>(tr.node)) { if (LDSN) trav_node_lds((const u4 *)lnodes, tr); else trav_node(A.bvh, tr); }
                    if (u + 1 >= RTW_TRAV_UNROLL) break;
                    live = lanes_in(in_trav<stack_t>(tr.node));
                    if (live == 0u) break;
                }
                asm volatile("" : "+s"(b_steps), "+s"(b_lanes));
                c_steps[0] += b_steps; c_lanes[0] += b_lanes;
#ifdef RTW_STAMP
                break;
#else
                if (live == 0u) break;
                live = lanes_in(in_trav<stack_t>(tr.node));
                if (live < 33u) break;
                if (++trips > RTW_MAX_TRIPS) break;
#endif
            }
        }
#ifdef RTW_STAMP
        asm volatile("s_waitcnt vmcnt(0) lgkmcnt(0)" ::: "memory");
        c_time[which] += __builtin_amdgcn_s_memtime() - t_begin;
#endif
    }
    if constexpr (tri_spec(SPEC)) tri_nodes_end(A);
    if (GEOM || light_spec(SPEC)) { flush_quads(A, n_quad); flush_tests(A, n_isph); }
#ifdef RTW_CENSUS
    for (int k = 0; k < CEN_N; k++) {
        unsigned long long w = cn->w[k], n = cn->n[k];
        for (int off = 32; off > 0; off >>= 1) { w += __shfl_down(w, off); n += __shfl_down(n, off); }
        if ((threadIdx.x & 63u) == 0) { atomicAdd(&A.stats[32 + 2 * k], w); atomicAdd(&A.stats[33 + 2 * k], n); }
    }
#endif
#ifdef RTW_ENDTIMES
    uint32_t dry_q_max = dry_queries, dry_q_sum = dry_queries;
    for (int off = 32; off > 0; off >>= 1) { const uint32_t o = __shfl_down(dry_q_max, off); dry_q_max = o > dry_q_max ? o : dry_q_max; dry_q_sum += __shfl_down(dry_q_sum, off); }
#endif
    if ((threadIdx.x & 63u) == 0) {
        atomicAdd(&A.stats[0], (unsigned long long)w_rays);
        atomicAdd(&A.stats[1], (unsigned long long)w_seg);
        atomicAdd(&A.stats[2], (unsigned long long)c_lanes[1] + (unsigned long long)w_seg * A.bvh.n_big);
        atomicAdd(&A.stats[3], (unsigned long long)c_lanes[0]);
        for (int k = 0; k < 3; k++) { atomicAdd(&A.stats[5 + k], (unsigned long long)c_steps[k]); atomicAdd(&A.stats[8 + k], (unsigned long long)c_lanes[k]); }
        if (aborted) atomicAdd(&A.stats[23], 1ull);
#ifdef RTW_STAMP
        for (int k = 0; k < 3; k++) atomicAdd(&A.stats[11 + k], c_time[k]);
        for (int k = 0; k < 4; k++) atomicAdd(&A.stats[16 + k], sub[k]);
#endif
#ifdef RTW_ENDTIMES
        const unsigned long long t_end = __builtin_amdgcn_s_memtime();
        atomicMax(&A.stats[12], t_end - t_wave_start);
        if (A.endtimes_ref) {
            const unsigned long long bin = (t_end - t_wave_start) * 32ull / A.endtimes_ref;
            const unsigned long long b = bin >= 32ull ? 11ull : (bin >= 21ull ? bin - 21ull : 0ull);
            atomicAdd(&A.stats[20 + b], 1ull);
        }
        atomicAdd(&A.stats[13], t_end - t_wave_start);
        atomicAdd(&A.stats[15], 1ull);
        const unsigned long long rt_end = wall_clock64();
        atomicMin(&A.stats[24 + 8 - 8], rt_wave_start + 0ull);
        atomicMax(&A.stats[25], rt_wave_start);
        atomicMin(&A.stats[26], rt_end);
        atomicMax(&A.stats[27], rt_end);
        if (rs.t_dry) { atomicMin(&A.stats[28], rs.t_dry); atomicMax(&A.stats[29], rs.t_dry); atomicMax(&A.stats[30], rt_end - rs.t_dry); atomicAdd(&A.stats[31], rt_end - rs.t_dry); }
        if (rs.t_dry && rt_end - rs.t_dry >= 60000ull) {
            atomicAdd(&A.stats[40], 1ull); atomicAdd(&A.stats[41], rt_end - rs.t_dry); atomicAdd(&A.stats[42], (unsigned long long)dry_trips);
            for (int k = 0; k < 3; k++) { atomicAdd(&A.stats[43 + k], (unsigned long long)dry_steps[k]); atomicAdd(&A.stats[46 + k], (unsigned long long)dry_lanes[k]); }
            atomicAdd(&A.stats[49], (unsigned long long)dry_q_max); atomicAdd(&A.stats[50], (unsigned long long)dry_q_sum);
        }
#endif
    }
}

typedef void (*kernel_fn)(const KArgs);
static bool is_common_config(const KArgs &a) {
    return a.integrator == RTW_INTEGRATOR_GRADIENT && a.sampler == RTW_SAMPLER_ROW && a.depth >= 1 &&
           (a.flags & (RTW_FLAG_CPP_DIELECTRIC | RTW_FLAG_CPP_DIFFUSE)) == 0u;
}
static bool is_demo_config(const KArgs &a) {
    return a.integrator == RTW_INTEGRATOR_BG_COLOR && a.sampler == RTW_SAMPLER_ROW && a.depth >= 1 &&
           (a.flags & (RTW_FLAG_CPP_DIELECTRIC | RTW_FLAG_CPP_DIFFUSE)) == 0u;
}
static bool is_serial_config(const KArgs &a) {
    return a.integrator == RTW_INTEGRATOR_GRADIENT && a.sampler == RTW_SAMPLER_STRATIFIED && a.depth >= 1 &&
           (a.flags & (RTW_FLAG_CPP_DIELECTRIC | RTW_FLAG_CPP_DIFFUSE)) == 0u;
}
static bool is_rust2_config(const KArgs &a) {
    return a.integrator == RTW_INTEGRATOR_RUST2 && a.sampler == RTW_SAMPLER_CENTRES && a.depth >= 1 &&
           (a.flags & (RTW_FLAG_CPP_DIELECTRIC | RTW_FLAG_CPP_DIFFUSE)) == 0u;
}
template <int SPEC>
static kernel_fn pick_kernel_spec(bool moving, uint32_t accel, int nodes) {
    if (accel == RTW_ACCEL_BVH) {
        if (nodes == 2) return moving ? render_bvh<true, 2, SPEC, false> : render_bvh<false, 2, SPEC, false>;
        if (nodes == 1) return moving ? render_bvh<true, 1, SPEC, false> : render_bvh<false, 1, SPEC, false>;
        return moving ? render_bvh<true, 0, SPEC, false> : render_bvh<false, 0, SPEC, false>;
    }
    return moving ? render_brute<true, SPEC, false> : render_brute<false, SPEC, false>;
}
template <int SPEC>
static kernel_fn pick_kernel_geom(bool moving, uint32_t accel, int nodes) {
    if (accel == RTW_ACCEL_BVH) {
        if (nodes) return moving ? render_bvh<true, 1, SPEC, true> : render_bvh<false, 1, SPEC, true>;
        return moving ? render_bvh<true, 0, SPEC, true> : render_bvh<false, 0, SPEC, true>;
    }
    return moving ? render_brute<true, SPEC, true> : render_brute<false, SPEC, true>;
}
static kernel_fn pick_kernel(const KArgs &a, bool moving, uint32_t accel, bool lds_nodes) {
    const int nodes = lds_nodes ? (a.lds_geom_off ? 2 : 1) : 0;
    if (a.inst_quats) return pick_kernel_geom<11>(moving, accel, nodes);
    if (a.flags & RTW_FLAG_MIXED_MATERIAL)
        return (a.geom.n_quads || a.geom.n_inst) ? pick_kernel_geom<10>(moving, accel, nodes) : pick_kernel_spec<10>(moving, accel, nodes);
    if (a.integrator == RTW_INTEGRATOR_LIGHT_CAST || a.integrator == RTW_INTEGRATOR_LIGHT_BIASED)
        return (a.geom.n_quads || a.geom.n_inst) ? pick_kernel_geom<9>(moving, accel, nodes) : pick_kernel_spec<9>(moving, accel, nodes);
    if (a.noise.tex) return (a.geom.n_quads || a.geom.n_inst) ? pick_kernel_geom<7>(moving, accel, nodes) : pick_kernel_spec<7>(moving, accel, nodes);
    if (a.tris.n) return pick_kernel_geom<8>(moving, accel, nodes);
    if (a.geom.n_quads || a.geom.n_inst) {
#ifndef RTW_GEOM_GENERIC_ONLY
        if (is_common_config(a) && !(a.flags & RTW_FLAG_CHUNK_SUMS)) return pick_kernel_geom<2>(moving, accel, nodes);
        if (is_demo_config(a) && !(a.flags & RTW_FLAG_CHUNK_SUMS)) return pick_kernel_geom<4>(moving, accel, nodes);
        if (is_rust2_config(a) && !(a.flags & RTW_FLAG_CHUNK_SUMS)) return pick_kernel_geom<5>(moving, accel, nodes);
        if (is_serial_config(a) && !(a.flags & RTW_FLAG_CHUNK_SUMS)) return pick_kernel_geom<6>(moving, accel, nodes);
#endif
        return pick_kernel_geom<0>(moving, accel, nodes);
    }
#ifndef RTW_GEOM_GENERIC_ONLY
    if (is_demo_config(a) && !(a.flags & RTW_FLAG_CHUNK_SUMS)) return pick_kernel_spec<4>(moving, accel, nodes);
    if (is_rust2_config(a) && !(a.flags & RTW_FLAG_CHUNK_SUMS)) return pick_kernel_spec<5>(moving, accel, nodes);
    if (is_serial_config(a) && !(a.flags & RTW_FLAG_CHUNK_SUMS)) return pick_kernel_spec<6>(moving, accel, nodes);
#endif
    if (!is_common_config(a)) return pick_kernel_spec<0>(moving, accel, nodes);
    if (a.flags & RTW_FLAG_CHUNK_SUMS) return a.has_textures ? pick_kernel_spec<0>(moving, accel, nodes) : pick_kernel_spec<3>(moving, accel, nodes);
    return a.has_textures ? pick_kernel_spec<2>(moving, accel, nodes) : pick_kernel_spec<1>(moving, accel, nodes);
}

__global__ __launch_bounds__(RTW_BLOCK) void perlin_eval_kernel(const RtwPerlin *t, const float *points, uint32_t n, uint32_t depth, float *out) {
    const uint32_t i = blockIdx.x * RTW_BLOCK + threadIdx.x;
    if (i >= n) return;
    out[i] = perlin_eval(*t, points[3 * (size_t)i], points[3 * (size_t)i + 1], points[3 * (size_t)i + 2], depth);
}

void launch_perlin_eval(const RtwPerlin *t, const float *points, uint32_t n, uint32_t depth, float *out, hipStream_t stream) {
    hipLaunchKernelGGL(perlin_eval_kernel, dim3((n + RTW_BLOCK - 1) / RTW_BLOCK), dim3(RTW_BLOCK), 0, stream, t, points, n, depth, out);
}

__global__ __launch_bounds__(RTW_BLOCK) void tri_hits_kernel(const DevTris T, const float *rays, uint32_t n, float mint, float maxt, float *t_out,
                                                             int32_t *idx_out, unsigned long long *counters) {
    const uint32_t i = blockIdx.x * RTW_BLOCK + threadIdx.x;
    uint32_t n_tests = 0, n_nodes = 0;
    if (i < n) {
        const float *r = rays + 6 * (size_t)i;
        float t;
        const int k = tri_closest(T, mk(r[0], r[1], r[2]), mk(r[3], r[4], r[5]), mint, maxt, false, 0.0f, t, n_tests, n_nodes);
        t_out[i] = k >= 0 ? t : __builtin_inff();
        idx_out[i] = k;
    }
    unsigned long long a = n_tests, b = n_nodes;
    for (int off = 32; off > 0; off >>= 1) { a += __shfl_down(a, off); b += __shfl_down(b, off); }
    if ((threadIdx.x & 63u) == 0) { atomicAdd(&counters[0], a); atomicAdd(&counters[1], b); }
}

void launch_tri_hits(const DevTris &T, const float *rays, uint32_t n, float mint, float maxt, float *t_out, int32_t *idx_out,
                     unsigned long long *counters, hipStream_t stream) {
    hipLaunchKernelGGL(tri_hits_kernel, dim3((n + RTW_BLOCK - 1) / RTW_BLOCK), dim3(RTW_BLOCK), 0, stream, T, rays, n, mint, maxt, t_out, idx_out, counters);
}

bool kernel_has_lds_geom(const KArgs &a) { return !(a.geom.n_quads || a.geom.n_inst || a.tris.n); }

void launch_render(const KArgs &a, bool moving, uint32_t accel, uint32_t grid, hipStream_t stream) {
    hipLaunchKernelGGL(pick_kernel(a, moving, accel, a.bvh.nodes16 != nullptr), dim3(grid), dim3(RTW_BLOCK), a.lds_bytes, stream, a);
    hipLaunchKernelGGL(resolve_kernel, dim3((a.n_tiles * 64u + RTW_BLOCK - 1) / RTW_BLOCK), dim3(RTW_BLOCK), 0, stream, a);
}

uint32_t kernel_blocks_per_cu(const KArgs &a, bool moving, uint32_t accel, bool lds_nodes) {
    int n = 0;
    if (hipOccupancyMaxActiveBlocksPerMultiprocessor(&n, pick_kernel(a, moving, accel, lds_nodes), RTW_BLOCK, a.lds_bytes) != hipSuccess || n < 1) n = 1;
    return (uint32_t)(n > 8 ? 8 : n);
}

const void *kernel_id(const KArgs &a, bool moving, uint32_t accel, bool lds_nodes) {
    return (const void *)pick_kernel(a, moving, accel, lds_nodes);
}

}
```

### raytracing-in-a-weekend_amd/csrc/rtw_shim.hip

```cpp
#include "rtw_kernels.h"
#include "rtw_host.h"
#include "rtw_filter.h"
#include "rtw_devmem.h"
#include "rtw_exp.h"

#include <link.h>

#include <chrono>
#include <cmath>
#include <cstdio>
#include <cstdlib>
#include <cstring>
#include <limits>
#include <map>
#include <new>
#include <utility>
#include <vector>

using namespace rtw;

static thread_local int g_last_hip = 0;

#define HIP_TRY(expr)                                                     \
    do {                                                                  \
        hipError_t e_ = (expr);                                           \
        if (e_ != hipSuccess) { g_last_hip = (int)e_; return RTW_E_HIP; } \
    } while (0)

struct SceneMem {
    DevMem geom, vel, mat, tex, texels;
    DevMem quads, inst, igeom, ivel, imat, iquads;
    DevMem nodes, nodes16, big_geom, big_vel, big_index;
};
struct NoiseMem { DevMem perlin, tex_noise; };
struct TriMem { DevMem list, leaf, nodes; };
struct QuatMem { DevMem rows; };
struct ScratchMem {
    DevMem queue, stats;
    PinnedMem h_stats;
    DevMem qstats; PinnedMem h_qstats;
    DevMem out;
    PinnedMem h_out;
    DevMem order;
    DevMem samples;
};

struct rtw_ctx {
    int device = 0;
    int n_cu = 0;
    hipStream_t own_stream = nullptr, stream = nullptr;
    hipEvent_t ev0 = nullptr, ev1 = nullptr;
    hipEvent_t ev_mark = nullptr;
    bool has_scene = false;
    bool has_textures = false;
    bool bvh_ok = true;
    double scene_span = 0.0;
    float t_begin = 0.0f, t_end = 0.0f;
    DevScene sc{};
    float bg[3] = { 0, 0, 0 };
    DevGeom geom{};
    DevBvh bvh{};
    SceneMem scene_mem;
    uint32_t n_textures = 0;
    std::vector<uint8_t> tex_used;
    bool noise_active = false;
    DevNoise noise{};
    NoiseMem noise_mem;
    FilterScratch *filter = nullptr;
    DevTris tris{};
    bool tri_tree = false;
    TriMem tri_mem;
    DevLights lights{};
    std::vector<RtwSphere> h_spheres;
    std::vector<RtwQuad> h_quads;
    bool has_medium = false;
    std::vector<RtwInstance> h_instances;
    const f4 *inst_quats = nullptr;
    QuatMem quat_mem;
    bool has_mixed = false, mixed_bad = false;
    ScratchMem scr;
    TileOrderKey order_key{};
    SceneCull cull{};
    uint32_t scene_serial = 0;
    uint32_t opt_chunk_len = 0;
    uint64_t opt_bank_bytes = 48ull << 30;
    int opt_lds_geom = -1;
    uint32_t opt_blocks_per_cu = 0;
    uint32_t opt_list_walk_max = RTW_LIST_WALK_MAX_DEFAULT;
    uint32_t opt_tile_order = 0;
    uint32_t opt_sub_queues = 0;
    double opt_tail_units = 0.0;
    uint32_t opt_guided_layout = 0;
    uint32_t opt_grab_blocks = 2;

    std::map<std::pair<const void *, uint32_t>, uint32_t> occupancy;
    bool attr_on_device = false; int attr_device = -1;
    struct Pending {
        bool active = false;
        bool marked = false;
        uint32_t n_rows = 0;
        std::chrono::steady_clock::time_point t0;
        float enqueue_ms = 0.0f;
        float *dst = nullptr; bool scatter = false, direct = false, staged = false;
        uint32_t width = 0, height = 0, row_block = 1, part_index = 0, part_count = 1;
        size_t out_bytes = 0;
    } pend;
};

struct OutSpec {
    float *base;
    bool scatter;
};

static void prepare_spheres(const RtwSphere *sp, uint32_t n, const RtwTexture *tex, std::vector<f4> &geom, std::vector<f4> &vel, std::vector<DevMat> &mat, bool &moving) {
    geom.resize(n); vel.resize(n); mat.resize(n);
    for (uint32_t i = 0; i < n; i++) {
        const RtwSphere &s = sp[i];
        geom[i] = f4{ s.center[0], s.center[1], s.center[2], host_mul(s.radius, s.radius) };
        vel[i] = f4{ s.velocity[0], s.velocity[1], s.velocity[2], 0.0f };
        if (s.velocity[0] != 0.0f || s.velocity[1] != 0.0f || s.velocity[2] != 0.0f) moving = true;
        DevMat &m = mat[i];
        std::memset(&m, 0, sizeof m);
        for (int k = 0; k < 3; k++) {
            m.cm[k] = s.tex < 0 ? host_mul(host_mul(s.tex_color[k], 1.0f), s.col_mod[k]) : s.col_mod[k];
            m.emitted[k] = s.emitted[k];
        }
        m.metallicness = s.metallicness; m.opacity = s.opacity; m.ir = s.ir; m.tex = s.tex;
        if (s.tex >= 0 && tex) { m.tex_row = tex[s.tex].row; m.tex_col = tex[s.tex].col; m.tex_offset = tex[s.tex].texel_offset; }
        m.inv_ir = host_div(1.0f, s.ir);
        m.r0_front = schlick_r0(m.inv_ir); m.r0_back = schlick_r0(s.ir);
    }
}

static void prepare_quads(const RtwQuad *q, uint32_t n, std::vector<DevQuad> &out) {
    out.resize(n);
    for (uint32_t i = 0; i < n; i++) {
        const RtwQuad &s = q[i];
        DevQuad &d = out[i];
        std::memset(&d, 0, sizeof d);
        const float nx = s.u[1] * s.v[2] - s.u[2] * s.v[1], ny = s.u[2] * s.v[0] - s.u[0] * s.v[2], nz = s.u[0] * s.v[1] - s.u[1] * s.v[0];
        const float len = std::sqrt(nx * nx + ny * ny + nz * nz);
        d.normal[0] = nx / len; d.normal[1] = ny / len; d.normal[2] = nz / len;
        d.d = d.normal[0] * s.origin[0] + d.normal[1] * s.origin[1] + d.normal[2] * s.origin[2];
        const float nn = nx * nx + ny * ny + nz * nz;
        d.w[0] = nx / nn; d.w[1] = ny / nn; d.w[2] = nz / nn;
        for (int k = 0; k < 3; k++) {
            d.origin[k] = s.origin[k]; d.u[k] = s.u[k]; d.v[k] = s.v[k];
            d.albedo[k] = host_mul(s.tex_color[k], 1.0f);
            d.emitted[k] = s.emitted[k];
        }
        d.metallicness = s.metallicness; d.opacity = s.opacity; d.ir = s.ir; d.tex = s.tex;
    }
}

template <class T>
static int upload(DevMem &dst, const std::vector<T> &src) {
    HIP_TRY(dst.reserve(src.empty() ? sizeof(T) : src.size() * sizeof(T)));
    if (!src.empty()) HIP_TRY(hipMemcpy(dst.ptr, src.data(), src.size() * sizeof(T), hipMemcpyHostToDevice));
    return RTW_OK;
}

static int count_hip_runtimes_cb(struct dl_phdr_info *info, size_t, void *data) {
    if (info->dlpi_name && std::strstr(info->dlpi_name, "libamdhip64")) ++*(int *)data;
    return 0;
}

extern "C" {

int rtw_abi_version(void) { return RTW_ABI_VERSION; }

int rtw_hip_runtime_count(void) {
    int n = 0;
    dl_iterate_phdr(count_hip_runtimes_cb, &n);
    return n;
}

int rtw_last_hip_error(void) { return g_last_hip; }

int rtw_device_count(void) {
    int n = 0;
    if (hipGetDeviceCount(&n) != hipSuccess) return 0;
    return n;
}

const char *rtw_strerror(int status) {
    switch (status) {
    case RTW_OK: return "ok";
    case RTW_E_INVALID: return "invalid argument";
    case RTW_E_NO_DEVICE: return "no HIP device";
    case RTW_E_HIP: return "HIP runtime error";
    case RTW_E_NOMEM: return "out of memory";
    case RTW_E_UNSUPPORTED: return "not implemented on the device";
    case RTW_E_NO_SCENE: return "no scene set";
    case RTW_E_INTERNAL: return "a render kernel gave up (internal error): the image is incomplete";
    case RTW_E_RUNTIME_CONFLICT: return "two copies of the HIP runtime (libamdhip64) are loaded in this process -- typically PyTorch imported AFTER the first rtw_* call: "
                                        "import torch before using this library (the runtimes then share one copy), or link both against the same runtime";
    default: return "unknown status";
    }
}

int rtw_ctx_create(int device, rtw_ctx **out) {
    if (!out) return RTW_E_INVALID;
    *out = nullptr;
    if (rtw_hip_runtime_count() > 1) return RTW_E_RUNTIME_CONFLICT;
    int n = rtw_device_count();
    if (n <= 0 || device < 0 || device >= n) return RTW_E_NO_DEVICE;
    rtw_ctx *c = new (std::nothrow) rtw_ctx();
    if (!c) return RTW_E_NOMEM;
    c->device = device;
    hipError_t e = hipSetDevice(device);
    hipDeviceProp_t prop;
    if (e == hipSuccess) e = hipGetDeviceProperties(&prop, device);
    if (e == hipSuccess) { c->n_cu = prop.multiProcessorCount; e = hipStreamCreateWithFlags(&c->own_stream, hipStreamNonBlocking); }
    if (e == hipSuccess) e = hipEventCreate(&c->ev0);
    if (e == hipSuccess) e = hipEventCreate(&c->ev1);
    if (e == hipSuccess) e = hipEventCreate(&c->ev_mark);
    if (e == hipSuccess) e = c->scr.queue.reserve(RTW_QUEUE_BYTES);
    if (e == hipSuccess) e = c->scr.stats.reserve(RTW_N_STATS * sizeof(unsigned long long));
    if (e == hipSuccess) e = c->scr.h_stats.reserve(RTW_N_STATS * sizeof(unsigned long long));
    if (e == hipSuccess) e = c->scr.qstats.reserve(RTW_QUERY_SLOTS * RTW_QUERY_STRIDE * sizeof(unsigned long long));
    if (e == hipSuccess) e = c->scr.h_qstats.reserve(RTW_QUERY_SLOTS * RTW_QUERY_STRIDE * sizeof(unsigned long long));
    if (e != hipSuccess) { g_last_hip = (int)e; rtw_ctx_destroy(c); return RTW_E_HIP; }
    c->stream = c->own_stream;
    *out = c;
    return RTW_OK;
}

static void free_noise(rtw_ctx *c) {
    c->noise_mem = NoiseMem{};
    c->noise = DevNoise{};
    c->noise_active = false;
}

static void free_tris(rtw_ctx *c) {
    c->tri_mem = TriMem{};
    c->tris = DevTris{};
    c->tri_tree = false;
}

static void free_quats(rtw_ctx *c) {
    c->quat_mem = QuatMem{};
    c->inst_quats = nullptr;
}

static void free_scene(rtw_ctx *c) {
// ... 490 lines not shown
    if (!c->has_scene) return RTW_E_NO_SCENE;
    HIP_TRY(hipSetDevice(c->device));
    bool tree = accel == RTW_ACCEL_BVH && c->bvh_ok && c->sc.n > c->opt_list_walk_max;
    if (mint != mint || maxt != maxt || time != time) tree = false;
    if (!(c->scene_span <= 1e18)) tree = false;
    if (c->sc.moving && !(time >= c->t_begin && time <= c->t_end)) tree = false;

    QueryArgs q;
    std::memset(&q, 0, sizeof q);
    q.sc = c->sc; q.bvh = c->bvh; q.geom = c->geom; q.inst_quats = c->inst_quats;
    if (c->tris.n) q.tris = tri_view(c, accel, mint, maxt);
    if (cam) { q.cam = *cam; q.width = width; q.height = height; }
    q.n = n; q.levels = c->bvh.depth + 2u;
    q.time = time; q.mint = mint; q.maxt = maxt; q.miss_t = miss_t; q.span = (float)c->scene_span;
    q.counters = c->scr.qstats.as<unsigned long long>();

    const size_t ray_bytes = 6 * sizeof(float) * (size_t)n, t_bytes = sizeof(float) * (size_t)n, i_bytes = sizeof(int32_t) * (size_t)n;
    DevMem d_r, d_t, d_i, d_n;
    hipError_t e = hipSuccess;
    if (rays) {
        if (query_on_device(c, rays)) q.rays = rays;
        else {
            e = d_r.reserve(ray_bytes);
            if (e == hipSuccess) e = hipMemcpyAsync(d_r.ptr, rays, ray_bytes, hipMemcpyDefault, c->stream);
            q.rays = d_r.as<const float>();
        }
    }
    if (query_on_device(c, t_out)) q.t_out = t_out;
    else { if (e == hipSuccess) e = d_t.reserve(t_bytes); q.t_out = d_t.as<float>(); }
    if (idx_out) {
        if (query_on_device(c, idx_out)) q.idx_out = idx_out;
        else { if (e == hipSuccess) e = d_i.reserve(i_bytes); q.idx_out = d_i.as<int32_t>(); }
    }
    if (normal_out) {
        if (query_on_device(c, normal_out)) q.normal_out = normal_out;
        else { if (e == hipSuccess) e = d_n.reserve(3 * t_bytes); q.normal_out = d_n.as<float>(); }
    }
    const size_t q_bytes = RTW_QUERY_SLOTS * RTW_QUERY_STRIDE * sizeof(unsigned long long);
    if (e == hipSuccess) e = hipMemsetAsync(c->scr.qstats.ptr, 0, q_bytes, c->stream);
    if (e == hipSuccess) e = hipEventRecord(c->ev0, c->stream);
    if (e == hipSuccess) {
        launch_scene_hits(q, cam != nullptr, tree, c->stream);
        e = hipGetLastError();
    }
    if (e == hipSuccess) e = hipEventRecord(c->ev1, c->stream);
    if (e == hipSuccess && d_t.ptr) e = hipMemcpyAsync(t_out, d_t.ptr, t_bytes, hipMemcpyDefault, c->stream);
    if (e == hipSuccess && d_i.ptr) e = hipMemcpyAsync(idx_out, d_i.ptr, i_bytes, hipMemcpyDefault, c->stream);
    if (e == hipSuccess && d_n.ptr) e = hipMemcpyAsync(normal_out, d_n.ptr, 3 * t_bytes, hipMemcpyDefault, c->stream);
    if (e == hipSuccess) e = hipMemcpyAsync(c->scr.h_qstats.ptr, c->scr.qstats.ptr, q_bytes, hipMemcpyDeviceToHost, c->stream);
    if (e == hipSuccess) e = hipStreamSynchronize(c->stream);
    float ms = 0.0f;
    if (e == hipSuccess) e = hipEventElapsedTime(&ms, c->ev0, c->ev1);
    if (const int rc = call_status(c, e)) return rc;
    const unsigned long long *h_qstats = c->scr.h_qstats.as<unsigned long long>();
    unsigned long long sum[4] = { 0, 0, 0, 0 };
    for (uint32_t s = 0; s < RTW_QUERY_SLOTS; s++) for (int k = 0; k < 4; k++) sum[k] += h_qstats[s * RTW_QUERY_STRIDE + k];
    if (stats) {
        std::memset(stats, 0, sizeof *stats);
        stats->segments = n;
        stats->sphere_tests = sum[0]; stats->node_tests = sum[1]; stats->quad_tests = sum[2];
        stats->kernel_ms = ms;
    }
    return sum[3] ? RTW_E_INTERNAL : RTW_OK;
}

int rtw_ctx_scene_hits(rtw_ctx *c, const float *rays, uint32_t n_rays, float time, float mint, float maxt, uint32_t accel,
                       float *t_out, int32_t *idx_out, float *normal_out, RtwStats *stats) {
    if (!c || !rays || !t_out || !idx_out || n_rays == 0 || accel > RTW_ACCEL_BVH) return RTW_E_INVALID;
    return scene_query(c, nullptr, 0, 0, rays, n_rays, time, mint, maxt, accel, std::numeric_limits<float>::infinity(), t_out, idx_out, normal_out, stats);
}

int rtw_ctx_depth_map(rtw_ctx *c, const RtwCamera *cam, uint32_t width, uint32_t height, float time, float mint, float maxt, uint32_t accel,
                      float *depth_out, int32_t *idx_out, float *normal_out, RtwStats *stats) {
    if (!c || !cam || !depth_out || width == 0 || height == 0 || accel > RTW_ACCEL_BVH) return RTW_E_INVALID;
    if ((uint64_t)width * height > 0xFFFFFFFFull) return RTW_E_INVALID;
    return scene_query(c, cam, width, height, nullptr, width * height, time, mint, maxt, accel, host_mul(maxt, 1.6f), depth_out, idx_out, normal_out, stats);
}

int rtw_perlin_eval(const RtwPerlin *t, const float *points, uint32_t n, uint32_t turb_depth, float *out) {
    if (!t || !points || !out || n == 0) return RTW_E_INVALID;
    for (uint32_t i = 0; i < n; i++) out[i] = perlin_eval(*t, points[3 * (size_t)i], points[3 * (size_t)i + 1], points[3 * (size_t)i + 2], turb_depth);
    return RTW_OK;
}

int rtw_ctx_perlin_eval(rtw_ctx *c, const RtwPerlin *t, const float *points, uint32_t n, uint32_t turb_depth, float *out) {
    if (!c || !t || !points || !out || n == 0) return RTW_E_INVALID;
    if (c->pend.active) return RTW_E_INVALID;
    HIP_TRY(hipSetDevice(c->device));
    const size_t pts_bytes = 3 * sizeof(float) * (size_t)n, out_bytes = sizeof(float) * (size_t)n;
    DevMem d_t, d_p, d_o;
    hipError_t e = d_t.reserve(sizeof(RtwPerlin));
    if (e == hipSuccess) e = d_p.reserve(pts_bytes);
    if (e == hipSuccess) e = d_o.reserve(out_bytes);
    if (e == hipSuccess) e = hipMemcpyAsync(d_t.ptr, t, sizeof(RtwPerlin), hipMemcpyHostToDevice, c->stream);
    if (e == hipSuccess) e = hipMemcpyAsync(d_p.ptr, points, pts_bytes, hipMemcpyHostToDevice, c->stream);
    if (e == hipSuccess) {
        launch_perlin_eval(d_t.as<const RtwPerlin>(), d_p.as<const float>(), n, turb_depth, d_o.as<float>(), c->stream);
        e = hipGetLastError();
    }
    if (e == hipSuccess) e = hipMemcpyAsync(out, d_o.ptr, out_bytes, hipMemcpyDeviceToHost, c->stream);
    if (e == hipSuccess) e = hipStreamSynchronize(c->stream);
    return call_status(c, e);
}

int rtw_ctx_bilateral_filter(rtw_ctx *c, const void *in, uint32_t w, uint32_t h, const RtwBilateral *p, uint8_t *out, RtwFilterStats *stats) {
    if (!c) return RTW_E_INVALID;
    if (c->pend.active) return RTW_E_INVALID;
    return bilateral_filter_device(c->device, c->stream, &c->filter, in, w, h, p, out, stats, &g_last_hip);
}

int rtw_ctx_guided_filter(rtw_ctx *c, const void *in, uint32_t w, uint32_t h, const float *depth, const float *normal, const int32_t *idx,
                          const RtwGuidedFilter *p, uint8_t *out, RtwFilterStats *stats) {
    if (!c) return RTW_E_INVALID;
    if (c->pend.active) return RTW_E_INVALID;
    return guided_filter_device(c->device, c->stream, &c->filter, c->opt_guided_layout, in, w, h, depth, normal, idx, p, out, stats, &g_last_hip);
}

}

static int scatter_rows(rtw_ctx *c, const float *src, float *dst, uint32_t width, uint32_t height, uint32_t row_block,
                        uint32_t part_index, uint32_t part_count) {
    const size_t row_bytes = (size_t)width * 3 * sizeof(float);
    if (part_count <= 1) { HIP_TRY(hipMemcpyAsync(dst, src, row_bytes * height, hipMemcpyDefault, c->stream)); return RTW_OK; }
    const uint32_t n_blocks = (height + row_block - 1) / row_block;
    uint32_t mine = 0, full = 0;
    if (part_index < n_blocks) mine = (n_blocks - 1 - part_index) / part_count + 1;
    const bool ragged = height % row_block != 0;
    const bool own_last = mine > 0 && (part_index + (mine - 1) * part_count) == n_blocks - 1;
    full = mine - ((ragged && own_last) ? 1u : 0u);
    const size_t block_bytes = row_bytes * row_block;
    if (full) HIP_TRY(hipMemcpy2DAsync((char *)dst + (size_t)part_index * block_bytes, (size_t)part_count * block_bytes, src, block_bytes,
                                       block_bytes, full, hipMemcpyDefault, c->stream));
    if (full < mine) {
        const uint32_t b = part_index + full * part_count;
        HIP_TRY(hipMemcpyAsync((char *)dst + (size_t)b * block_bytes, (const char *)src + (size_t)full * block_bytes,
                               row_bytes * (height - b * row_block), hipMemcpyDefault, c->stream));
    }
    return RTW_OK;
}

static void scatter_rows_host(const float *src, float *dst, uint32_t width, uint32_t height, uint32_t n_rows, uint32_t row_block, uint32_t part_index, uint32_t part_count) {
    const size_t row_floats = (size_t)width * 3;
    if (part_count <= 1) { std::memcpy(dst, src, row_floats * height * sizeof(float)); return; }
    for (uint32_t k = 0; k < n_rows; k += row_block) {
        const uint32_t j = ((k / row_block) * part_count + part_index) * row_block;
        const uint32_t rows = std::min(row_block, std::min(n_rows - k, height - j));
        std::memcpy(dst + (size_t)j * row_floats, src + (size_t)k * row_floats, rows * row_floats * sizeof(float));
    }
}

enum : unsigned { PH_PREPARE = 1u, PH_LAUNCH = 2u, PH_COPY = 4u, PH_ALL = 7u };
static int render_enqueue_impl(rtw_ctx *c, const RtwCamera *cam, const RtwParams *p, OutSpec out, unsigned phases);
static int render_copy(rtw_ctx *c);

static int render_enqueue(rtw_ctx *c, const RtwCamera *cam, const RtwParams *p, OutSpec out, unsigned phases = PH_ALL) {
    const int rc = render_enqueue_impl(c, cam, p, out, phases);
    if (rc != RTW_OK && c && c->stream && !c->pend.active) {
        const int keep = g_last_hip;
        if (hipStreamSynchronize(c->stream) != hipSuccess) (void)hipGetLastError();
        g_last_hip = keep;
    }
    return rc;
}

static int render_enqueue_impl(rtw_ctx *c, const RtwCamera *cam, const RtwParams *p, OutSpec out, unsigned phases) {
    if (!c || !cam || !p || !out.base) return RTW_E_INVALID;
    if (c->pend.active) return RTW_E_INVALID;
    if (!c->has_scene) return RTW_E_NO_SCENE;
    if (p->width == 0 || p->height == 0 || p->samples == 0) return RTW_E_INVALID;
    if (p->integrator > RTW_INTEGRATOR_LIGHT_BIASED || p->sampler > RTW_SAMPLER_NO_RAND || p->accel > RTW_ACCEL_BVH) return RTW_E_INVALID;
    if (p->part_count > 1 && (p->row_block == 0 || p->part_index >= p->part_count)) return RTW_E_INVALID;
    if (p->width > 65535u || p->height > 65535u) return RTW_E_INVALID;
    if (const int qrc = quats_render_check(c->inst_quats != nullptr, p->integrator, c->noise_active, c->tris.n != 0u)) return qrc;
    if (c->noise_active && p->integrator == RTW_INTEGRATOR_RUST2) return RTW_E_UNSUPPORTED;
    if (c->noise_active && c->tris.n) return RTW_E_UNSUPPORTED;
    const bool light_integrator = p->integrator == RTW_INTEGRATOR_LIGHT_CAST || p->integrator == RTW_INTEGRATOR_LIGHT_BIASED;
    if (light_integrator && (c->noise_active || c->tris.n || c->has_medium)) return RTW_E_UNSUPPORTED;
    if (const int mrc = mixed_check(p->flags, p->integrator, c->has_mixed, c->mixed_bad, c->noise_active, c->tris.n != 0u, c->has_medium)) return mrc;
    const bool mixed_active = (p->flags & RTW_FLAG_MIXED_MATERIAL) && c->has_mixed;
    if (!c->pend.marked) c->pend.t0 = std::chrono::steady_clock::now();
    HIP_TRY(hipSetDevice(c->device));

    uint32_t accel = p->accel;
    if (accel == RTW_ACCEL_BVH) {
        const double P[3] = { cam->pixel00[0], cam->pixel00[1], cam->pixel00[2] };
        const double U[3] = { cam->delta_u[0], cam->delta_u[1], cam->delta_u[2] }, V[3] = { cam->delta_v[0], cam->delta_v[1], cam->delta_v[2] };
        auto norm = [](const double *v) { return std::sqrt(v[0] * v[0] + v[1] * v[1] + v[2] * v[2]); };
        const double W = (double)p->width + 1.0, H = (double)p->height + 1.0;
        const double hi = norm(P) + W * norm(U) + H * norm(V);
        const double N[3] = { U[1] * V[2] - U[2] * V[1], U[2] * V[0] - U[0] * V[2], U[0] * V[1] - U[1] * V[0] };
        const double nn = norm(N);
        const double lo = nn > 0.0 ? std::fabs(P[0] * N[0] + P[1] * N[1] + P[2] * N[2]) / nn : 0.0;
        if (!(hi <= 1e15) || !(lo >= 1e-15)) accel = RTW_ACCEL_BRUTE;
        const double O[3] = { cam->origin[0], cam->origin[1], cam->origin[2] }, CU[3] = { cam->u[0], cam->u[1], cam->u[2] }, CV[3] = { cam->v[0], cam->v[1], cam->v[2] };
        if (!(norm(O) + std::fabs((double)cam->lens_radius) * (norm(CU) + norm(CV)) <= 0x1p60)) accel = RTW_ACCEL_BRUTE;
        if (!(std::fmax(hi, 2.0) * (c->scene_span + norm(O) + 1.0) <= 1e18)) accel = RTW_ACCEL_BRUTE;
        if (p->mint != p->mint || p->maxt != p->maxt) accel = RTW_ACCEL_BRUTE;
        if (c->sc.moving) {
            const float ta = cam->time0, tb = cam->time0 + cam->shutter;
            if (!(std::fmin(ta, tb) >= c->t_begin && std::fmax(ta, tb) <= c->t_end)) accel = RTW_ACCEL_BRUTE;
            if (ta != ta || tb != tb) accel = RTW_ACCEL_BRUTE;
            if ((light_integrator || mixed_active) && !(c->t_begin <= 0.0f && c->t_end >= 0.0f)) accel = RTW_ACCEL_BRUTE;
        }
        if (!c->bvh_ok) accel = RTW_ACCEL_BRUTE;
        if (c->sc.n <= c->opt_list_walk_max) accel = RTW_ACCEL_BRUTE;
    }

    KArgs a;
    std::memset(&a, 0, sizeof a);
    a.cam = *cam; a.sc = c->sc; a.bvh = c->bvh; a.geom = c->geom;
    if (p->flags & RTW_FLAG_GLOBAL_NODES) a.bvh.nodes16 = nullptr;
    a.flags = p->flags;
    if (!mixed_active) a.flags &= ~RTW_FLAG_MIXED_MATERIAL;
    a.width = p->width; a.height = p->height;
    const uint32_t n_rows = rtw_part_rows(p->height, p->row_block, p->part_index, p->part_count);
    a.row_block = p->row_block ? p->row_block : 1; a.part_index = p->part_index; a.part_count = p->part_count;
    a.tiles_x = (p->width + 7) / 8;
    a.n_samples = sampler_count(p->sampler, p->samples, &a.s_root);
    if (a.n_samples == 0 || a.n_samples >= (1u << 24)) return RTW_E_INVALID;
    a.sampler = p->sampler; a.integrator = p->integrator; a.depth = p->depth;
    a.has_textures = c->has_textures ? 1u : 0u;
    a.seed_lo = (uint32_t)p->seed; a.seed_hi = (uint32_t)(p->seed >> 32);
    a.inv_gamma = host_div(1.0f, p->gamma);
    a.mint = p->mint; a.maxt = p->maxt;
    std::memcpy(a.bg, c->bg, sizeof a.bg);
    a.queue = c->scr.queue.as<uint32_t>(); a.stats = c->scr.stats.as<unsigned long long>();
    if (c->noise_active) a.noise = c->noise;
    if (c->tris.n) a.tris = tri_view(c, p->accel, p->mint, p->maxt);
    if (light_integrator) a.lights = c->lights;
    a.inst_quats = c->inst_quats;
#ifdef RTW_ENDTIMES
    if (const char *e = getenv("RTW_ENDTIMES_REF")) a.endtimes_ref = std::strtoull(e, nullptr, 10);
#endif

    const bool sums = (p->flags & RTW_FLAG_CHUNK_SUMS) != 0;
    uint32_t chunk_len = (p->flags & RTW_FLAG_CHUNK_SUMS) ? RTW_SUM_CHUNK : c->opt_chunk_len;
    if (chunk_len == 0) {
        const uint64_t units4 = (uint64_t)a.tiles_x * ((n_rows + 7) / 8) * ((a.n_samples + 3) / 4) * 64ull;
        const uint64_t lanes = (uint64_t)c->n_cu * 1536ull;
        chunk_len = units4 >= 500ull * lanes ? 12u : units4 >= 200ull * lanes ? 8u : units4 >= 64ull * lanes ? 6u : (units4 * 6ull < 16ull * lanes ? 2u : 4u);
    }
    if (chunk_len > a.n_samples) chunk_len = a.n_samples;
    a.chunk_len = chunk_len;
    a.n_chunks = (a.n_samples + chunk_len - 1) / chunk_len;
    a.bank_len = sums ? 1u : 0u;
    const uint64_t slots_per_tile_row = (uint64_t)a.tiles_x * (sums ? a.n_chunks : a.n_samples) * 64ull;
    uint64_t max_slots = c->opt_bank_bytes / 12; if (max_slots > 0xFFFFFFF0ull) max_slots = 0xFFFFFFF0ull;
    const uint64_t items_per_tile_row = slots_per_tile_row;
    const uint32_t tile_rows = (n_rows + 7) / 8;
    uint64_t band_tile_rows = max_slots / (slots_per_tile_row ? slots_per_tile_row : 1);
    if (band_tile_rows > 0xFFFFFFF0ull / items_per_tile_row) band_tile_rows = 0xFFFFFFF0ull / items_per_tile_row;
    if (band_tile_rows == 0) return RTW_E_NOMEM;
    if (band_tile_rows > tile_rows) band_tile_rows = tile_rows;
    const size_t sample_bytes = (size_t)(band_tile_rows * slots_per_tile_row) * 12;
    if (c->scr.samples.reserve(sample_bytes) != hipSuccess) { (void)hipGetLastError(); return RTW_E_NOMEM; }
    a.samples = c->scr.samples.as<float>();

    const size_t out_bytes = (size_t)n_rows * p->width * 3 * sizeof(float);
    bool pinned_host = false;
    {
        hipPointerAttribute_t attr;
        c->attr_on_device = false; c->attr_device = -1;
        if (hipPointerGetAttributes(&attr, out.base) == hipSuccess) {
            c->attr_on_device = attr.type == hipMemoryTypeDevice || attr.type == hipMemoryTypeManaged;
            pinned_host = attr.type == hipMemoryTypeHost;
            c->attr_device = attr.device;
        } else (void)hipGetLastError();
    }
    const bool direct = c->attr_on_device && c->attr_device == c->device && !(out.scatter && p->part_count > 1);
    const bool staged = out.scatter && !c->attr_on_device && !pinned_host;
    if (staged && c->scr.h_out.reserve(out_bytes) != hipSuccess) { (void)hipGetLastError(); return RTW_E_NOMEM; }
    if (direct) a.out = out.base;
    else {
        HIP_TRY(c->scr.out.reserve(out_bytes));
        a.out = c->scr.out.as<float>();
    }

    if (accel == RTW_ACCEL_BVH) {
        const bool ldsn = a.bvh.nodes16 != nullptr;
        uint32_t levels = c->bvh.depth + 3; if (levels < 4) levels = 4;
        uint32_t off = 0;
        if (ldsn) { off = c->bvh.n_nodes * 32u; off = (off + 15u) & ~15u; }
        a.lds_stack_off = off;
        off += levels * RTW_BLOCK * (ldsn ? 2u : 4u);
        off = (off + 15u) & ~15u;
        if (ldsn) {
            bool geom = off + c->sc.n * 16u <= 160u * 1024u / (1536u / RTW_BLOCK);
            if (c->opt_lds_geom >= 0) geom = c->opt_lds_geom != 0 && c->sc.n <= RTW_LDS_GEOM_MAX;
            if (geom && kernel_has_lds_geom(a)) { a.lds_geom_off = off; off += c->sc.n * 16u; }
        }
        a.lds_bytes = off;
    }
    if (a.tris.n) { a.tris.lds_off = (a.lds_bytes + 15u) & ~15u; a.lds_bytes = a.tris.lds_off + 16u; }

    uint32_t per_cu = c->opt_blocks_per_cu;
    if (per_cu == 0) {
        const bool ldsn = c->bvh.nodes16 != nullptr && !(p->flags & RTW_FLAG_GLOBAL_NODES);
        const auto key = std::make_pair(kernel_id(a, c->sc.moving != 0, accel, ldsn), a.lds_bytes);
        auto it = c->occupancy.find(key);
        if (it == c->occupancy.end()) it = c->occupancy.emplace(key, kernel_blocks_per_cu(a, c->sc.moving != 0, accel, ldsn)).first;
        per_cu = it->second;
    }

    if (!(phases & PH_LAUNCH)) return RTW_OK;

    if (!c->pend.marked) HIP_TRY(hipEventRecord(c->ev_mark, c->stream));
    HIP_TRY(hipMemsetAsync(a.stats, 0, RTW_N_STATS * sizeof(unsigned long long), c->stream));
#ifdef RTW_ENDTIMES
    HIP_TRY(hipMemsetAsync(a.stats + 24, 0xFF, sizeof(unsigned long long), c->stream));
    HIP_TRY(hipMemsetAsync(a.stats + 26, 0xFF, sizeof(unsigned long long), c->stream));
    HIP_TRY(hipMemsetAsync(a.stats + 28, 0xFF, sizeof(unsigned long long), c->stream));
#endif
    HIP_TRY(hipEventRecord(c->ev0, c->stream));
    for (uint32_t tr0 = 0; tr0 < tile_rows || tr0 == 0; tr0 += (uint32_t)band_tile_rows) {
        const uint32_t tr1 = tr0 + (uint32_t)band_tile_rows < tile_rows ? tr0 + (uint32_t)band_tile_rows : tile_rows;
        a.k_base = tr0 * 8; a.k_end = tr1 * 8 < n_rows ? tr1 * 8 : n_rows;
        a.n_tiles = a.tiles_x * (tr1 - tr0);
        a.total_work = a.n_tiles * a.n_chunks * 64u;
        a.reg_q1 = a.reg_q2 = a.n_tiles;
        for (int r = 0; r < 3; r++) { a.reg_len[r] = a.chunk_len; a.reg_nc[r] = a.n_chunks; }
        a.tile_order = nullptr;
        if (c->opt_tile_order && a.n_tiles > 2u && !((c->opt_tile_order == 2u || c->opt_tile_order == 5u) && c->cull.n_other)) {
            const uint32_t tiles_y = a.n_tiles / a.tiles_x;
            TileOrderKey key;
            std::memset(&key, 0, sizeof key);
            key.mode = c->opt_tile_order; key.tiles_x = a.tiles_x; key.tiles_y = tiles_y; key.k_base = a.k_base;
            key.row_block = a.row_block; key.part_index = a.part_index; key.part_count = a.part_count; key.cam = *cam; key.scene_serial = c->scene_serial;
            key.cam.time0 = key.cam.shutter = key.cam.lens_radius = 0.0f;
            const uint64_t per_tile = 64ull * a.n_chunks;
            key.tail_tiles = (uint32_t)std::min<uint64_t>(a.n_tiles, ((uint64_t)c->n_cu * per_cu * RTW_BLOCK * 4ull + per_tile - 1) / per_tile);
            if (!c->scr.order.ptr || std::memcmp(&key, &c->order_key, sizeof key) != 0) {
                std::vector<uint32_t> order;
                build_tile_order(c->opt_tile_order, a.tiles_x, tiles_y, a.k_base, a.row_block, a.part_index, a.part_count, *cam, c->cull, key.tail_tiles, order);
                HIP_TRY(c->scr.order.reserve(order.size() * sizeof(uint32_t)));
                HIP_TRY(hipMemcpyAsync(c->scr.order.ptr, order.data(), order.size() * sizeof(uint32_t), hipMemcpyHostToDevice, c->stream));
                HIP_TRY(hipStreamSynchronize(c->stream));
                c->order_key = key;
            }
            a.tile_order = c->scr.order.as<uint32_t>();
        }
        uint32_t wg_per_cu = per_cu;
        if (c->opt_blocks_per_cu == 0) {
            const uint64_t lanes_per_wg_row = (uint64_t)c->n_cu * RTW_BLOCK * 16ull;
            const uint64_t want = ((uint64_t)a.total_work + lanes_per_wg_row - 1) / lanes_per_wg_row;
            if (want < wg_per_cu) wg_per_cu = (uint32_t)(want ? want : 1);
            if (wg_per_cu > 6u && (uint64_t)a.total_work < 40ull * c->n_cu * RTW_BLOCK * wg_per_cu) wg_per_cu = 6u;
        }
        uint32_t grid = (uint32_t)c->n_cu * wg_per_cu;
        {
            const uint32_t need = (a.total_work + RTW_BLOCK - 1) / RTW_BLOCK;
            if (grid > need) grid = need ? need : 1;
        }
        if (!sums && c->opt_tail_units > 0.0 && a.chunk_len > 1u && a.n_tiles > 1u) {
            const double waves = (double)grid * (RTW_BLOCK / 64u);
            const uint32_t L1 = a.chunk_len, L2 = L1 >= 12u ? 4u : (L1 >= 6u ? 2u : 1u), L3 = 1u;
            uint64_t t3 = (uint64_t)std::ceil(c->opt_tail_units * waves * L3 / (double)a.n_samples);
            uint64_t t2 = L2 > L3 ? (uint64_t)std::ceil(c->opt_tail_units * waves * L2 / (double)a.n_samples) : 0;
            if (t3 > a.n_tiles / 4u) t3 = a.n_tiles / 4u;
            if (t2 > a.n_tiles / 4u) t2 = a.n_tiles / 4u;
            a.reg_q2 = a.n_tiles - (uint32_t)t3; a.reg_q1 = a.reg_q2 - (uint32_t)t2;
            a.reg_len[1] = L2; a.reg_len[2] = L3;
            for (int r = 1; r < 3; r++) a.reg_nc[r] = (a.n_samples + a.reg_len[r] - 1u) / a.reg_len[r];
            a.total_work = (a.reg_q1 * a.reg_nc[0] + (a.reg_q2 - a.reg_q1) * a.reg_nc[1] + (a.n_tiles - a.reg_q2) * a.reg_nc[2]) * 64u;
        }
        {
            a.sub_shift = (c->opt_sub_queues != 1u && a.n_tiles >= 64u && grid >= 64u) ? RTW_SUB_SHIFT : 0u;
            const uint32_t waves4 = (grid * (RTW_BLOCK / 64u) * 4u) >> a.sub_shift;
            a.grab_shift = 0; while (a.grab_shift < 31u && (1u << a.grab_shift) < waves4) a.grab_shift++;
            uint32_t blocks = c->opt_grab_blocks ? c->opt_grab_blocks : a.n_chunks;
            if (blocks > a.n_chunks) blocks = a.n_chunks;
            a.grab_max = (blocks ? blocks : 1u) * 64u;
        }
        HIP_TRY(hipMemsetAsync(a.queue, 0, RTW_QUEUE_BYTES, c->stream));
        if (a.n_tiles) launch_render(a, c->sc.moving != 0, accel, grid, c->stream);
        HIP_TRY(hipGetLastError());
        if (tile_rows == 0) break;
    }
    HIP_TRY(hipEventRecord(c->ev1, c->stream));
    HIP_TRY(hipMemcpyAsync(c->scr.h_stats.ptr, a.stats, RTW_N_STATS * sizeof(unsigned long long), hipMemcpyDeviceToHost, c->stream));
    c->pend.active = true; c->pend.n_rows = n_rows;
    c->pend.dst = out.base; c->pend.scatter = out.scatter; c->pend.direct = direct; c->pend.staged = staged;
    c->pend.width = p->width; c->pend.height = p->height; c->pend.row_block = a.row_block; c->pend.part_index = p->part_index; c->pend.part_count = p->part_count;
    c->pend.out_bytes = out_bytes;
    c->pend.enqueue_ms = std::chrono::duration<float, std::milli>(std::chrono::steady_clock::now() - c->pend.t0).count();
    if (phases & PH_COPY) return render_copy(c);
    return RTW_OK;
}

static int render_copy(rtw_ctx *c) {
    if (!c || !c->pend.active) return RTW_E_INVALID;
    const rtw_ctx::Pending &q = c->pend;
    if (q.direct) return RTW_OK;
    HIP_TRY(hipSetDevice(c->device));
    if (q.staged) {
        HIP_TRY(hipMemcpyAsync(c->scr.h_out.ptr, c->scr.out.ptr, q.out_bytes, hipMemcpyDeviceToHost, c->stream));
    } else if (q.scatter) {
        const int rc = scatter_rows(c, c->scr.out.as<float>(), q.dst, q.width, q.height, q.row_block, q.part_index, q.part_count);
        if (rc != RTW_OK) return rc;
    } else HIP_TRY(hipMemcpyAsync(q.dst, c->scr.out.ptr, q.out_bytes, hipMemcpyDefault, c->stream));
    return RTW_OK;
}

static int render_wait(rtw_ctx *c, RtwStats *stats) {
    if (!c || !c->pend.active) return RTW_E_INVALID;
    c->pend.active = false; c->pend.marked = false;
    HIP_TRY(hipSetDevice(c->device));
    HIP_TRY(hipStreamSynchronize(c->stream));
    if (c->pend.staged)
        scatter_rows_host(c->scr.h_out.as<float>(), c->pend.dst, c->pend.width, c->pend.height, c->pend.n_rows, c->pend.row_block, c->pend.part_index, c->pend.part_count);
    float ms = 0.0f, start_ms = 0.0f;
    HIP_TRY(hipEventElapsedTime(&ms, c->ev0, c->ev1));
    HIP_TRY(hipEventElapsedTime(&start_ms, c->ev_mark, c->ev0));
    const unsigned long long *h_stats = c->scr.h_stats.as<unsigned long long>();
    const bool kernel_gave_up = h_stats[23] != 0ull;
    if (stats) {
        std::memset(stats, 0, sizeof *stats);
        stats->camera_rays = h_stats[0]; stats->segments = h_stats[1];
        stats->sphere_tests = h_stats[2]; stats->node_tests = h_stats[3];
        stats->nan_pixels = (uint32_t)h_stats[4]; stats->rows = c->pend.n_rows;
        stats->quad_tests = h_stats[14];
        stats->kernel_ms = ms;
        stats->enqueue_ms = c->pend.enqueue_ms; stats->start_ms = start_ms;
        for (int k = 0; k < 3; k++) { stats->phase_steps[k] = h_stats[5 + k]; stats->phase_lanes[k] = h_stats[8 + k]; }
        for (int k = 3; k < 5; k++) { stats->phase_steps[k] = h_stats[16 + 2 * (k - 3)]; stats->phase_lanes[k] = h_stats[17 + 2 * (k - 3)]; }
#ifdef RTW_CENSUS
        if (getenv("RTW_CENSUS_DUMP")) {
            static const char *names[CEN_N] = { "shading", "inflight (unit(d))", "miss (sky)", "hit (point, normal, material)", "dielectric branch", "schlick draw",
                                                "diffuse branch", "unit-vector loop trip", "bank store", "needs a work unit", "start_path", "lens-disk loop trip",
                                                "trav_begin", "depth exhausted", "trips through the scheduler (all phases)", "cooperative round" };
            std::fprintf(stderr, "rtw census: %llu SHADE steps\n", h_stats[7]);
            for (int k = 0; k < CEN_N; k++)
                if (h_stats[32 + 2 * k])
                    std::fprintf(stderr, "rtw census: %-32s executions %12llu (%.3f per SHADE step)  lanes %14llu  live fraction %.4f  lanes per SHADE step %.2f\n", names[k],
                                 h_stats[32 + 2 * k], (double)h_stats[32 + 2 * k] / (double)h_stats[7], h_stats[33 + 2 * k],
                                 (double)h_stats[33 + 2 * k] / (64.0 * (double)h_stats[32 + 2 * k]), (double)h_stats[33 + 2 * k] / (double)h_stats[7]);
        }
#endif
#if defined(RTW_STAMP) || defined(RTW_ENDTIMES)
        if (getenv("RTW_STAMP_DUMP")) std::fprintf(stderr, "rtw stamp: wave-ticks traverse %llu leaf %llu shade %llu   of shade (specialised builds): a. unit(d) + paths that end %llu, b. bank + next unit %llu, c-d. hit / path start + the rejection loop + second halves %llu, e. query begin %llu   (generic build: hit, bank + next unit, camera ray, query begin)\n",
                                                   h_stats[11], h_stats[12], h_stats[13], h_stats[16], h_stats[17], h_stats[18], h_stats[19]);
        if (getenv("RTW_ENDTIMES_DUMP") && h_stats[15] && getenv("RTW_ENDTIMES_REF")) {
            std::fprintf(stderr, "rtw endtimes histogram (waves ending in each 1/32 of the reference lifetime, bins 21/32 .. 32/32+; bin 0 also holds everything earlier):");
            for (int k = 0; k < 12; k++) std::fprintf(stderr, " %llu", h_stats[20 + k]);
            std::fprintf(stderr, "\n");
        }
        if (getenv("RTW_ENDTIMES_DUMP") && h_stats[15])
            std::fprintf(stderr, "rtw endtimes (100 MHz device clock): wave starts spread over %.1f us, first wave end %.1f us and last wave end %.1f us after the first start\n",
                         (double)(h_stats[25] - h_stats[24]) / 100.0, (double)(h_stats[26] - h_stats[24]) / 100.0, (double)(h_stats[27] - h_stats[24]) / 100.0);
        if (getenv("RTW_ENDTIMES_DUMP") && h_stats[15])
            std::fprintf(stderr, "rtw endtimes: the queue ran dry for the first wave %.1f us and for the last wave %.1f us after the first start; a wave then ran on for %.1f us on average, %.1f us at most\n",
                         (double)(h_stats[28] - h_stats[24]) / 100.0, (double)(h_stats[29] - h_stats[24]) / 100.0, (double)h_stats[31] / (double)h_stats[15] / 100.0, (double)h_stats[30] / 100.0);
        if (getenv("RTW_ENDTIMES_DUMP") && h_stats[15]) {
            if (h_stats[40]) {
                const double n = (double)h_stats[40];
                std::fprintf(stderr, "rtw endtimes: %llu waves ran on for 0.6 ms or more after finding the queue empty: on average %.0f us, %.0f scheduler trips (%.0f TRAVERSE steps with %.1f lanes, %.0f LEAF with %.1f, %.0f SHADE with %.1f), the busiest lane shaded %.1f queries, all lanes %.1f -> %.1f us per trip, %.1f us per query of the busiest lane\n",
                             h_stats[40], h_stats[41] / n / 100.0, h_stats[42] / n, h_stats[43] / n, h_stats[43] ? (double)h_stats[46] / h_stats[43] : 0.0, h_stats[44] / n, h_stats[44] ? (double)h_stats[47] / h_stats[44] : 0.0,
                             h_stats[45] / n, h_stats[45] ? (double)h_stats[48] / h_stats[45] : 0.0, h_stats[49] / n, h_stats[50] / n,
                             h_stats[42] ? h_stats[41] / 100.0 / h_stats[42] : 0.0, h_stats[49] ? h_stats[41] / 100.0 / h_stats[49] : 0.0);
            }
            std::fprintf(stderr, "rtw endtimes: %llu waves, longest lifetime %llu ticks, mean lifetime %.1f %% of it\n", h_stats[15], h_stats[12],
                         100.0 * (double)h_stats[13] / (double)h_stats[15] / (double)h_stats[12]);
        }
#endif
        stats->total_ms = std::chrono::duration<float, std::milli>(std::chrono::steady_clock::now() - c->pend.t0).count();
    }
    return kernel_gave_up ? RTW_E_INTERNAL : RTW_OK;
}

struct rtw_mgpu {
    std::vector<rtw_ctx *> ctx;
};

extern "C" {

int rtw_ctx_set_option(rtw_ctx *c, uint32_t key, double v) {
    if (!c || !(v == v)) return RTW_E_INVALID;
    switch (key) {
    case RTW_OPT_CHUNK_LEN:      if (!(v >= 0.0 && v <= 255.0)) return RTW_E_INVALID; c->opt_chunk_len = (uint32_t)v; return RTW_OK;
    case RTW_OPT_SAMPLE_BANK_GB: if (!(v > 0.0 && v <= 1048576.0)) return RTW_E_INVALID; c->opt_bank_bytes = (uint64_t)(v * (double)(1ull << 30)); return RTW_OK;
    case RTW_OPT_LDS_GEOM:       if (!(v >= -1.0 && v <= 1.0)) return RTW_E_INVALID; c->opt_lds_geom = (int)v; return RTW_OK;
    case RTW_OPT_BLOCKS_PER_CU:  if (!(v >= 0.0 && v <= 8.0)) return RTW_E_INVALID; c->opt_blocks_per_cu = (uint32_t)v; return RTW_OK;
    case RTW_OPT_LIST_WALK_MAX:  if (!(v >= 0.0 && v <= 4294967295.0)) return RTW_E_INVALID; c->opt_list_walk_max = (uint32_t)v; return RTW_OK;
    case RTW_OPT_TILE_ORDER:     if (!(v >= 0.0 && v <= 5.0 && v == (double)(uint32_t)v)) return RTW_E_INVALID; c->opt_tile_order = (uint32_t)v; return RTW_OK;
    case RTW_OPT_SUB_QUEUES:     if (!(v == 0.0 || v == 1.0)) return RTW_E_INVALID; c->opt_sub_queues = (uint32_t)v; return RTW_OK;
    case RTW_OPT_TAIL_UNITS:     if (!(v >= 0.0 && v <= 1024.0)) return RTW_E_INVALID; c->opt_tail_units = v; return RTW_OK;
    case RTW_OPT_GUIDED_LAYOUT:  if (!(v >= 0.0 && v <= 4.0 && v == (double)(uint32_t)v)) return RTW_E_INVALID; c->opt_guided_layout = (uint32_t)v; return RTW_OK;
    case RTW_OPT_GRAB_BLOCKS:    if (!(v >= 0.0 && v <= 65536.0 && v == (double)(uint32_t)v)) return RTW_E_INVALID; c->opt_grab_blocks = (uint32_t)v; return RTW_OK;
    default: return RTW_E_INVALID;
    }
}

int rtw_ctx_render(rtw_ctx *c, const RtwCamera *cam, const RtwParams *p, float *out_rgb, RtwStats *stats) {
    int rc = render_enqueue(c, cam, p, OutSpec{ out_rgb, false });
    if (rc != RTW_OK) return rc;
    return render_wait(c, stats);
}

int rtw_mgpu_create(const int *devices, uint32_t n, rtw_mgpu **out) {
    if (!out) return RTW_E_INVALID;
    *out = nullptr;
    if (!devices || n == 0 || n > 64) return RTW_E_INVALID;
    if (rtw_device_count() <= 0) return RTW_E_NO_DEVICE;
    rtw_mgpu *m = new (std::nothrow) rtw_mgpu();
    if (!m) return RTW_E_NOMEM;
    for (uint32_t k = 0; k < n; k++) {
        rtw_ctx *c = nullptr;
        int rc = rtw_ctx_create(devices[k], &c);
        if (rc != RTW_OK) { rtw_mgpu_destroy(m); return rc; }
        m->ctx.push_back(c);
    }
    for (uint32_t k = 0; k < n; k++) for (uint32_t j = 0; j < n; j++) {
        if (devices[k] == devices[j]) continue;
        int can = 0;
        if (hipDeviceCanAccessPeer(&can, devices[k], devices[j]) == hipSuccess && can) {
            (void)hipSetDevice(devices[k]);
            if (hipDeviceEnablePeerAccess(devices[j], 0) != hipSuccess) (void)hipGetLastError();
        } else (void)hipGetLastError();
    }
    *out = m;
    return RTW_OK;
}

void rtw_mgpu_destroy(rtw_mgpu *m) {
    if (!m) return;
    for (rtw_ctx *c : m->ctx) rtw_ctx_destroy(c);
    delete m;
}

int rtw_mgpu_set_scene(rtw_mgpu *m, const RtwScene *scene, float t_begin, float t_end) {
    if (!m) return RTW_E_INVALID;
    for (rtw_ctx *c : m->ctx) { int rc = rtw_ctx_set_scene(c, scene, t_begin, t_end); if (rc != RTW_OK) return rc; }
    return RTW_OK;
}

int rtw_mgpu_set_texture_noise(rtw_mgpu *m, const RtwPerlin *tables, uint32_t n_tables, const RtwTextureNoise *per_texture, uint32_t n_textures) {
    if (!m) return RTW_E_INVALID;
    for (rtw_ctx *c : m->ctx) { int rc = rtw_ctx_set_texture_noise(c, tables, n_tables, per_texture, n_textures); if (rc != RTW_OK) return rc; }
    return RTW_OK;
}

int rtw_mgpu_set_lights(rtw_mgpu *m, const RtwLight *lights, uint32_t n, float biased_weight) {
    if (!m) return RTW_E_INVALID;
    for (rtw_ctx *c : m->ctx) { int rc = rtw_ctx_set_lights(c, lights, n, biased_weight); if (rc != RTW_OK) return rc; }
    return RTW_OK;
}

int rtw_mgpu_set_instance_rotations(rtw_mgpu *m, const float (*qs)[4], uint32_t n) {
    if (!m) return RTW_E_INVALID;
    for (rtw_ctx *c : m->ctx) {
        if (!c->has_scene) return RTW_E_NO_SCENE;
        if (c->pend.active) return RTW_E_INVALID;
        if (qs || n) { const int rc = quats_check(c->h_instances.data(), (uint32_t)c->h_instances.size(), qs, n, nullptr); if (rc != RTW_OK) return rc; }
    }
    for (rtw_ctx *c : m->ctx) { int rc = rtw_ctx_set_instance_rotations(c, qs, n); if (rc != RTW_OK) return rc; }
    return RTW_OK;
}

int rtw_mgpu_set_triangles(rtw_mgpu *m, const RtwTriangle *tris, uint32_t n) {
    if (!m) return RTW_E_INVALID;
    for (rtw_ctx *c : m->ctx) { int rc = rtw_ctx_set_triangles(c, tris, n); if (rc != RTW_OK) return rc; }
    return RTW_OK;
}

int rtw_mgpu_set_option(rtw_mgpu *m, uint32_t key, double value) {
    if (!m) return RTW_E_INVALID;
    for (rtw_ctx *c : m->ctx) { int rc = rtw_ctx_set_option(c, key, value); if (rc != RTW_OK) return rc; }
    return RTW_OK;
}

int rtw_mgpu_render(rtw_mgpu *m, const RtwCamera *cam, const RtwParams *params, float *out_rgb, RtwStats *per_device, RtwStats *total) {
    if (!m || !cam || !params || !out_rgb || params->part_count > 1) return RTW_E_INVALID;
    const auto t0 = std::chrono::steady_clock::now();
    const uint32_t n = (uint32_t)m->ctx.size();
    int rc = RTW_OK;
    auto part = [&](uint32_t k) { RtwParams q = *params; q.row_block = params->row_block ? params->row_block : 8u; q.part_index = k; q.part_count = n; return q; };
    for (uint32_t k = 0; k < n && rc == RTW_OK; k++) {
        rtw_ctx *c = m->ctx[k];
        if (c->pend.active) { rc = RTW_E_INVALID; break; }
        c->pend.t0 = t0;
        if (hipSetDevice(c->device) != hipSuccess || hipEventRecord(c->ev_mark, c->stream) != hipSuccess) { (void)hipGetLastError(); rc = RTW_E_HIP; break; }
        c->pend.marked = true;
        const RtwParams q = part(k);
        rc = render_enqueue(c, cam, &q, OutSpec{ out_rgb, true }, PH_PREPARE);
    }
    uint32_t launched = 0;
    for (; launched < n && rc == RTW_OK; launched++) {
        const RtwParams q = part(launched);
        rc = render_enqueue(m->ctx[launched], cam, &q, OutSpec{ out_rgb, true }, PH_PREPARE | PH_LAUNCH);
        if (rc != RTW_OK) break;
    }
    for (uint32_t k = 0; k < launched && rc == RTW_OK; k++) rc = render_copy(m->ctx[k]);
    for (uint32_t k = 0; k < n; k++) m->ctx[k]->pend.marked = m->ctx[k]->pend.active && m->ctx[k]->pend.marked;
    RtwStats sum; std::memset(&sum, 0, sizeof sum);
    for (uint32_t k = 0; k < launched; k++) {
        RtwStats st;
        const int rw = render_wait(m->ctx[k], &st);
        if (rw != RTW_OK) { if (rc == RTW_OK) rc = rw; continue; }
        if (per_device) per_device[k] = st;
        sum.camera_rays += st.camera_rays; sum.segments += st.segments; sum.sphere_tests += st.sphere_tests;
        sum.node_tests += st.node_tests; sum.quad_tests += st.quad_tests; sum.nan_pixels += st.nan_pixels; sum.rows += st.rows;
        for (int i = 0; i < 6; i++) { sum.phase_steps[i] += st.phase_steps[i]; sum.phase_lanes[i] += st.phase_lanes[i]; }
        if (st.kernel_ms > sum.kernel_ms) sum.kernel_ms = st.kernel_ms;
        if (st.enqueue_ms > sum.enqueue_ms) sum.enqueue_ms = st.enqueue_ms;
        if (st.start_ms > sum.start_ms) sum.start_ms = st.start_ms;
    }
    sum.total_ms = std::chrono::duration<float, std::milli>(std::chrono::steady_clock::now() - t0).count();
    if (total) *total = sum;
    return rc;
}

int rtw_render_multi_gpu(const int *devices, uint32_t n_devices, const RtwCamera *cam, const RtwScene *scene,
                         const RtwParams *params, float *out_rgb, RtwStats *per_device) {
    if (!cam || !scene || !params) return RTW_E_INVALID;
    rtw_mgpu *m = nullptr;
    int rc = rtw_mgpu_create(devices, n_devices, &m);
    if (rc != RTW_OK) return rc;
    rc = rtw_mgpu_set_scene(m, scene, cam->time0, cam->time0 + cam->shutter);
    if (rc == RTW_OK) rc = rtw_mgpu_render(m, cam, params, out_rgb, per_device, nullptr);
    rtw_mgpu_destroy(m);
    return rc;
}

int rtw_ctx_render_multi(rtw_ctx *c, const RtwCamera *cam, const RtwParams *p, float fps, uint32_t start_frame, uint32_t n_frames,
                         float *out_rgb, RtwStats *stats) {
    if (!c || !cam || !p || !out_rgb || !(fps > 0.0f)) return RTW_E_INVALID;
    const size_t frame_floats = (size_t)rtw_part_rows(p->height, p->row_block, p->part_index, p->part_count) * p->width * 3;
    for (uint32_t i = 0; i < n_frames; i++) {
        RtwCamera cm = *cam;
        cm.time0 = host_div((float)(start_frame + i), fps);
        int rc = rtw_ctx_render(c, &cm, p, out_rgb + (size_t)i * frame_floats, stats ? stats + i : nullptr);
        if (rc != RTW_OK) return rc;
    }
    return RTW_OK;
}

int rtw_render(const RtwCamera *cam, const RtwScene *scene, const RtwParams *params, float *out_rgb, RtwStats *stats) {
    if (!cam || !scene || !params) return RTW_E_INVALID;
    int dev = 0;
    if (rtw_device_count() <= 0) return RTW_E_NO_DEVICE;
    if (hipGetDevice(&dev) != hipSuccess) dev = 0;
    rtw_ctx *c = nullptr;
    int rc = rtw_ctx_create(dev, &c);
// ... 9 lines not shown
```

Baseline: 38110.

## Fuse tile resolve into render kernel via per-wave completion logs

```diff
diff --git a/include/rtw.h b/include/rtw.h
--- a/include/rtw.h
+++ b/include/rtw.h
@@ -188,9 +188,12 @@
     RTW_OPT_GRAB_BLOCKS      = 7,
     RTW_OPT_TAIL_UNITS       = 9,
     RTW_OPT_SUB_QUEUES       = 8,
-    RTW_OPT_GUIDED_LAYOUT    = 10
+    RTW_OPT_GUIDED_LAYOUT    = 10,
+    RTW_OPT_RESOLVE_FUSED    = 11
 };
 int  rtw_ctx_set_option(rtw_ctx *ctx, uint32_t key, double value);
+int  rtw_ctx_debug_resolved(rtw_ctx *ctx, uint32_t *out, uint32_t cap, uint32_t *n_tiles);
+int  rtw_debug_queue_regions(uint32_t n_tiles, uint32_t n_samples, uint32_t chunk_len, double tail_units, uint32_t waves, uint32_t out[9]);
 
 typedef struct rtw_mgpu rtw_mgpu;
 int  rtw_mgpu_create(const int *devices, uint32_t n_devices, rtw_mgpu **out);
diff --git a/raytracing-in-a-weekend_amd/__init__.py b/raytracing-in-a-weekend_amd/__init__.py
--- a/raytracing-in-a-weekend_amd/__init__.py
+++ b/raytracing-in-a-weekend_amd/__init__.py
@@ -22,6 +22,8 @@
 OPT_CHUNK_LEN, OPT_SAMPLE_BANK_GB, OPT_LDS_GEOM, OPT_BLOCKS_PER_CU, OPT_LIST_WALK_MAX, OPT_TILE_ORDER, OPT_GRAB_BLOCKS, OPT_SUB_QUEUES = 1, 2, 3, 4, 5, 6, 7, 8
 OPT_TAIL_UNITS = 9
 OPT_GUIDED_LAYOUT = 10
+OPT_RESOLVE_FUSED = 11
+RESOLVED_BY_RENDER, RESOLVED_BY_SWEEP = 1, 0x10000
 SCENE_C1, SCENE_C2, SCENE_C4, SCENE_C5, SCENE_METAL_TEST, SCENE_QUAD_TEST, SCENE_PRESENTATION, SCENE_FIRST_FRAME = 1, 2, 4, 5, 6, 7, 8, 9
 MEDIUM_SURFACE, MEDIUM_CONST_DENSITY = 0, 1
 PROXIMITY_SQUARE, PROXIMITY_EDGES = 0, 1
@@ -159,6 +161,9 @@
                                        C.c_void_p, C.POINTER(RtwStats)]
     L.rtw_render.argtypes = [C.POINTER(RtwCamera), C.POINTER(RtwScene), C.POINTER(RtwParams), C.c_void_p, C.POINTER(RtwStats)]
     L.rtw_ctx_set_option.argtypes = [C.c_void_p, C.c_uint32, C.c_double]
+    if hasattr(L, "rtw_ctx_debug_resolved"):
+        L.rtw_ctx_debug_resolved.argtypes = [C.c_void_p, C.POINTER(C.c_uint32), C.c_uint32, C.POINTER(C.c_uint32)]
+        L.rtw_debug_queue_regions.argtypes = [C.c_uint32, C.c_uint32, C.c_uint32, C.c_double, C.c_uint32, C.POINTER(C.c_uint32)]
     L.rtw_mgpu_create.argtypes = [C.POINTER(C.c_int), C.c_uint32, C.POINTER(C.c_void_p)]
     L.rtw_mgpu_destroy.argtypes = [C.c_void_p]
     L.rtw_mgpu_destroy.restype = None
@@ -853,6 +858,12 @@
         return img
 
 
+def queue_regions(n_tiles: int, n_samples: int, chunk_len: int, tail_units: float, waves: int) -> dict:
+    out = (C.c_uint32 * 9)()
+    _check(lib().rtw_debug_queue_regions(int(n_tiles), int(n_samples), int(chunk_len), float(tail_units), int(waves), out), "rtw_debug_queue_regions")
+    return {"q1": out[0], "q2": out[1], "len": list(out[2:5]), "units": list(out[5:8]), "work": out[8]}
+
+
 class Renderer:
 
     def __init__(self, device: int = 0):
@@ -947,6 +958,14 @@
 
     def set_option(self, key: int, value: float):
         _check(lib().rtw_ctx_set_option(self._h, int(key), float(value)), "rtw_ctx_set_option")
+
+    def debug_resolved(self) -> np.ndarray:
+        n = C.c_uint32(0)
+        _check(lib().rtw_ctx_debug_resolved(self._h, None, 0, C.byref(n)), "rtw_ctx_debug_resolved")
+        out = np.zeros(n.value, np.uint32)
+        if n.value:
+            _check(lib().rtw_ctx_debug_resolved(self._h, out.ctypes.data_as(C.POINTER(C.c_uint32)), n.value, C.byref(n)), "rtw_ctx_debug_resolved")
+        return out
 
     def bilateral_filter(self, img, size: int, proximity: int = PROXIMITY_SQUARE, avg_gradient: float = 0.0, out=None, shape=None,
                          in_format: Optional[int] = None):
diff --git a/raytracing-in-a-weekend_amd/csrc/rtw_kernels.h b/raytracing-in-a-weekend_amd/csrc/rtw_kernels.h
--- a/raytracing-in-a-weekend_amd/csrc/rtw_kernels.h
+++ b/raytracing-in-a-weekend_amd/csrc/rtw_kernels.h
@@ -7,6 +7,10 @@
 
 #define RTW_QUEUE_BYTES 4096u
 #define RTW_QUEUE_STRIDE 256u
+#define RTW_TICKET_WORD (8u * RTW_QUEUE_STRIDE / 4u)
+#define RTW_LOG_N 10u
+#define RTW_LOG_WORDS 32u
+#define RTW_RESOLVED_BY_SWEEP 0x10000u
 #ifndef RTW_SUB_SHIFT
 #define RTW_SUB_SHIFT 3u
 #endif
@@ -74,6 +78,9 @@
     DevTris tris;
     DevLights lights;
     const f4 *inst_quats;
+    uint32_t *done;
+    uint32_t *resolved;
+    uint32_t *wave_log;
 };
 
 void launch_render(const KArgs &a, bool moving, uint32_t accel, uint32_t grid, hipStream_t stream);
diff --git a/raytracing-in-a-weekend_amd/csrc/rtw_kernels.hip b/raytracing-in-a-weekend_amd/csrc/rtw_kernels.hip
--- a/raytracing-in-a-weekend_amd/csrc/rtw_kernels.hip
+++ b/raytracing-in-a-weekend_amd/csrc/rtw_kernels.hip
@@ -66,10 +66,53 @@
     return q;
 }
 
+__device__ __forceinline__ uint32_t uni(uint32_t x) { return (uint32_t)__builtin_amdgcn_readfirstlane((int)x); }
+__device__ __noinline__ void log_step(const KArgs *Ap, bool flush_, bool holding, uint32_t slot, bool append_, uint32_t lo, uint32_t len, uint32_t tile) {
+    const KArgs &A = *Ap;
+    const bool flush = uni(flush_) != 0u, append = uni(append_) != 0u;
+    lo = uni(lo); len = uni(len); tile = uni(tile);
+    const uint32_t lane = threadIdx.x & 63u;
+    uint32_t *log = A.wave_log + (size_t)(blockIdx.x * (RTW_BLOCK / 64u) + (threadIdx.x >> 6)) * RTW_LOG_WORDS;
+    const uint32_t v = lane < RTW_LOG_WORDS ? __hip_atomic_load(log + lane, __ATOMIC_RELAXED, __HIP_MEMORY_SCOPE_AGENT) : 0u;
+    const uint32_t n = (uint32_t)__builtin_amdgcn_readlane((int)v, 0);
+    uint32_t keep = 0u;
+    if (!flush)
+        for (uint32_t e = 0; e < n; e++) {
+            const uint32_t e_lo = (uint32_t)__builtin_amdgcn_readlane((int)v, (int)(1u + e)), e_len = (uint32_t)__builtin_amdgcn_readlane((int)v, (int)(1u + RTW_LOG_N + e));
+            if (ballot64(holding && slot - e_lo < e_len) != 0ull) keep |= 1u << e;
+        }
+    const uint32_t retire = ((1u << n) - 1u) & ~keep;
+    if (retire == 0u && !append) return;
+    if (retire) {
+        __builtin_amdgcn_fence(__ATOMIC_RELEASE, "agent");
+        asm volatile("s_waitcnt vmcnt(0)" ::: "memory");
+        for (uint32_t e = 0; e < n; e++)
+            if ((retire >> e & 1u) && lane == 0u)
+                __hip_atomic_fetch_add(A.done + (uint32_t)__builtin_amdgcn_readlane((int)v, (int)(1u + 2u * RTW_LOG_N + e)), 64u, __ATOMIC_RELAXED, __HIP_MEMORY_SCOPE_AGENT);
+    }
+    uint32_t k = 0;
+    for (uint32_t e = 0; e < n; e++)
+        if (keep >> e & 1u) {
+            if (k != e && lane == 0u) {
+                log[1u + k] = (uint32_t)__builtin_amdgcn_readlane((int)v, (int)(1u + e));
+                log[1u + RTW_LOG_N + k] = (uint32_t)__builtin_amdgcn_readlane((int)v, (int)(1u + RTW_LOG_N + e));
+                log[1u + 2u * RTW_LOG_N + k] = (uint32_t)__builtin_amdgcn_readlane((int)v, (int)(1u + 2u * RTW_LOG_N + e));
+            }
+            k++;
+        }
+    if (append && k < RTW_LOG_N) {
+        if (lane == 0u) { log[1u + k] = lo; log[1u + RTW_LOG_N + k] = len; log[1u + 2u * RTW_LOG_N + k] = tile; }
+        k++;
+    }
+    if (lane == 0u) log[0] = k;
+}
+
+template <bool FUSE = false>
 __device__ __forceinline__ bool fetch_pixel(const KArgs &A, bool need, Pixel &px, bool &exhausted, Reserve &rs) {
     const unsigned long long m = ballot64(need);
     if (m == 0ull) return false;
     if (rs.next == rs.end) {
+        uint32_t blk_tile = 0u;
         if (rs.end == rs.limit) {
             const uint32_t n_sub = 1u << A.sub_shift;
             const uint32_t leader = (uint32_t)__ffsll((long long)m) - 1u;
@@ -109,6 +152,7 @@
             else { u -= sq.b2; lt = u / A.reg_nc[2]; chunk = u - lt * A.reg_nc[2]; lt += sq.t2; len = A.reg_len[2]; }
             const uint32_t qt = (lt << A.sub_shift) + rs.sub;
             const uint32_t tile = A.tile_order ? A.tile_order[qt] : qt;
+            blk_tile = tile;
             const uint32_t trow = tile / A.tiles_x, tcol = tile - trow * A.tiles_x;
             rs.i0 = tcol * 8u;
             rs.k0 = A.k_base + trow * 8u;
@@ -116,6 +160,7 @@
             rs.s1 = rs.s0 + len < A.n_samples ? rs.s0 + len : A.n_samples;
             rs.slot0 = (A.bank_len ? tile * A.n_chunks + chunk : tile * A.n_samples + rs.s0) * 64u;
         }
+        if constexpr (FUSE) log_step((const KArgs *)__builtin_amdgcn_kernarg_segment_ptr(), false, !need, px.slot, rs.next < rs.limit, rs.slot0, (rs.s1 - rs.s0) * 64u, blk_tile);
     }
     const uint32_t avail = rs.end - rs.next;
     const uint32_t rank = __builtin_amdgcn_mbcnt_hi((uint32_t)(m >> 32), __builtin_amdgcn_mbcnt_lo((uint32_t)m, 0u));
@@ -504,11 +549,9 @@
     return px_advance(px);
 }
 
-__global__ __launch_bounds__(RTW_BLOCK) void resolve_kernel(const KArgs A) {
-    const uint32_t w = blockIdx.x * RTW_BLOCK + threadIdx.x;
-    const uint32_t tile = w >> 6, p = w & 63u;
+__device__ __forceinline__ void resolve_tile(const KArgs &A, uint32_t tile, uint32_t p) {
     uint32_t nan = 0;
-    if (tile < A.n_tiles) {
+    {
         const uint32_t tcol = tile % A.tiles_x, trow = tile / A.tiles_x;
         const uint32_t i = tcol * 8u + (p & 7u), k = A.k_base + trow * 8u + (p >> 3);
         if (i < A.width && k < A.k_end) {
@@ -523,7 +566,34 @@
         }
     }
     const unsigned long long m = ballot64(nan != 0);
-    if ((threadIdx.x & 63u) == 0 && m) atomicAdd(&A.stats[4], (unsigned long long)__popcll(m));
+    if (p == 0 && m) atomicAdd(&A.stats[4], (unsigned long long)__popcll(m));
+}
+
+__global__ __launch_bounds__(RTW_BLOCK) void resolve_kernel(const KArgs A) {
+    const uint32_t w = blockIdx.x * RTW_BLOCK + threadIdx.x;
+    const uint32_t tile = w >> 6, p = w & 63u;
+    if (tile >= A.n_tiles || A.resolved[tile] != 0u) return;
+    resolve_tile(A, tile, p);
+    if (p == 0u) A.resolved[tile] = RTW_RESOLVED_BY_SWEEP;
+}
+
+__device__ __noinline__ void fused_epilogue(const KArgs *Ap) {
+    const KArgs &A = *Ap;
+    const uint32_t lane = threadIdx.x & 63u;
+    log_step(Ap, true, false, 0u, false, 0u, 0u, 0u);
+    const uint32_t n_tiles = uni(A.n_tiles);
+    for (uint32_t taken = 0; taken <= n_tiles; taken++) {
+        uint32_t t = 0;
+        if (lane == 0u) t = atomicAdd(A.queue + RTW_TICKET_WORD, 1u);
+        t = uni(t);
+        if (t >= n_tiles) break;
+        const uint32_t tile = uni(A.tile_order ? A.tile_order[t] : t);
+        const uint32_t units = uni((t < A.reg_q1 ? A.reg_nc[0] : t < A.reg_q2 ? A.reg_nc[1] : A.reg_nc[2]) * 64u);
+        if (uni(__hip_atomic_load(A.done + tile, __ATOMIC_RELAXED, __HIP_MEMORY_SCOPE_AGENT)) < units) continue;
+        __builtin_amdgcn_fence(__ATOMIC_ACQUIRE, "agent");
+        resolve_tile(A, tile, lane);
+        if (lane == 0u) atomicAdd(A.resolved + tile, 1u);
+    }
 }
 
 __device__ __forceinline__ void flush_counters(const KArgs &A, uint32_t n_seg, uint32_t n_rays,
@@ -913,6 +983,7 @@
 #ifndef RTW_BVH_WAVES_FOLDED
 #define RTW_BVH_WAVES_FOLDED RTW_BVH_WAVES
 #endif
+constexpr bool fused_resolve_build(int spec, bool geom) { return spec == 1 && !geom; }
 constexpr bool two_halves_step(int spec, bool geom, bool moving) {
 #ifdef RTW_NO_TWO_HALVES
     return false;
@@ -920,9 +991,10 @@
     return gradient_spec(spec) && !geom && !(moving && spec == 2);
 #endif
 }
-template <bool MOVING, int NODES, int SPEC, bool GEOM>
+template <bool MOVING, int NODES, int SPEC, bool GEOM, bool FUSE = false>
 __global__ __launch_bounds__(RTW_BLOCK, GEOM ? (!generic_spec(SPEC) ? RTW_BVH_WAVES_GEOM_SPEC : RTW_BVH_WAVES_GEOM) : (two_halves_step(SPEC, GEOM, MOVING) ? (SPEC == 2 ? RTW_BVH_WAVES_SPEC2 : RTW_BVH_WAVES_SPEC) : (gradient_spec(SPEC) ? RTW_BVH_WAVES_SPEC2 : (!generic_spec(SPEC) ? RTW_BVH_WAVES_FOLDED : RTW_BVH_WAVES)))) void render_bvh(const KArgs A) {
     constexpr bool LDSN = NODES != 0, geom_in_lds = NODES == 2;
+    static_assert(!FUSE || fused_resolve_build(SPEC, GEOM), "only the builds of the trait resolve tiles themselves");
     typedef typename std::conditional<LDSN, short, int>::type stack_t;
     extern __shared__ __attribute__((aligned(16))) unsigned char lds_raw[];
     *(stack_t *)(lds_raw + A.lds_stack_off + threadIdx.x * (uint32_t)sizeof(stack_t)) = (stack_t)Code<stack_t>::END;
@@ -1033,7 +1105,7 @@
                 if (need_unit) RTW_CEN(cn, CEN_NEED_UNIT);
             }
             bool exhausted = false;
-            const bool got = fetch_pixel(A, need_unit, px, exhausted, rs);
+            const bool got = fetch_pixel<FUSE>(A, need_unit, px, exhausted, rs);
             if (ballot64(exhausted) != 0ull) t_lo = RTW_T_LO_DRAIN;
             RTW_SUB_STAMP(1);
             if (shading) {
@@ -1070,7 +1142,7 @@
                 if (need_unit) RTW_CEN(cn, CEN_NEED_UNIT);
             }
             bool exhausted = false;
-            const bool got = fetch_pixel(A, need_unit, px, exhausted, rs);
+            const bool got = fetch_pixel<FUSE>(A, need_unit, px, exhausted, rs);
             if (ballot64(exhausted) != 0ull) t_lo = RTW_T_LO_DRAIN;
             RTW_SUB_STAMP(1);
 #ifdef RTW_STAMP
@@ -1196,6 +1268,7 @@
         }
 #endif
     }
+    if constexpr (FUSE) if (!aborted) fused_epilogue((const KArgs *)__builtin_amdgcn_kernarg_segment_ptr());
 }
 
 typedef void (*kernel_fn)(const KArgs);
@@ -1216,7 +1289,13 @@
            (a.flags & (RTW_FLAG_CPP_DIELECTRIC | RTW_FLAG_CPP_DIFFUSE)) == 0u;
 }
 template <int SPEC>
-static kernel_fn pick_kernel_spec(bool moving, uint32_t accel, int nodes) {
+static kernel_fn pick_kernel_spec(bool moving, uint32_t accel, int nodes, bool fuse = false) {
+    if constexpr (fused_resolve_build(SPEC, false))
+        if (accel == RTW_ACCEL_BVH && fuse) {
+            if (nodes == 2) return moving ? render_bvh<true, 2, SPEC, false, true> : render_bvh<false, 2, SPEC, false, true>;
+            if (nodes == 1) return moving ? render_bvh<true, 1, SPEC, false, true> : render_bvh<false, 1, SPEC, false, true>;
+            return moving ? render_bvh<true, 0, SPEC, false, true> : render_bvh<false, 0, SPEC, false, true>;
+        }
     if (accel == RTW_ACCEL_BVH) {
         if (nodes == 2) return moving ? render_bvh<true, 2, SPEC, false> : render_bvh<false, 2, SPEC, false>;
         if (nodes == 1) return moving ? render_bvh<true, 1, SPEC, false> : render_bvh<false, 1, SPEC, false>;
@@ -1257,7 +1336,7 @@
 #endif
     if (!is_common_config(a)) return pick_kernel_spec<0>(moving, accel, nodes);
     if (a.flags & RTW_FLAG_CHUNK_SUMS) return a.has_textures ? pick_kernel_spec<0>(moving, accel, nodes) : pick_kernel_spec<3>(moving, accel, nodes);
-    return a.has_textures ? pick_kernel_spec<2>(moving, accel, nodes) : pick_kernel_spec<1>(moving, accel, nodes);
+    return a.has_textures ? pick_kernel_spec<2>(moving, accel, nodes) : pick_kernel_spec<1>(moving, accel, nodes, a.wave_log != nullptr);
 }
 
 __global__ __launch_bounds__(RTW_BLOCK) void perlin_eval_kernel(const RtwPerlin *t, const float *points, uint32_t n, uint32_t depth, float *out) {
diff --git a/raytracing-in-a-weekend_amd/csrc/rtw_shim.hip b/raytracing-in-a-weekend_amd/csrc/rtw_shim.hip
--- a/raytracing-in-a-weekend_amd/csrc/rtw_shim.hip
+++ b/raytracing-in-a-weekend_amd/csrc/rtw_shim.hip
@@ -43,6 +43,7 @@
     PinnedMem h_out;
     DevMem order;
     DevMem samples;
+    DevMem tilesync;
 };
 
 struct rtw_ctx {
@@ -91,6 +92,8 @@
     uint32_t opt_sub_queues = 0;
     double opt_tail_units = 0.0;
     uint32_t opt_guided_layout = 0;
+    uint32_t opt_resolve_fused = 1;
+    uint32_t resolved_tiles = 0;
     uint32_t opt_grab_blocks = 2;
 
     std::map<std::pair<const void *, uint32_t>, uint32_t> occupancy;
@@ -887,6 +890,7 @@
 enum : unsigned { PH_PREPARE = 1u, PH_LAUNCH = 2u, PH_COPY = 4u, PH_ALL = 7u };
 static int render_enqueue_impl(rtw_ctx *c, const RtwCamera *cam, const RtwParams *p, OutSpec out, unsigned phases);
 static int render_copy(rtw_ctx *c);
+static void tail_regions(KArgs &a, double tail_units, double waves);
 
 static int render_enqueue(rtw_ctx *c, const RtwCamera *cam, const RtwParams *p, OutSpec out, unsigned phases = PH_ALL) {
     const int rc = render_enqueue_impl(c, cam, p, out, phases);
@@ -1027,6 +1031,17 @@
         a.lds_bytes = off;
     }
     if (a.tris.n) { a.tris.lds_off = (a.lds_bytes + 15u) & ~15u; a.lds_bytes = a.tris.lds_off + 16u; }
+
+    const size_t band_tiles = (size_t)a.tiles_x * band_tile_rows, log_words = (size_t)c->n_cu * 8u * (RTW_BLOCK / 64u) * RTW_LOG_WORDS;
+    HIP_TRY(c->scr.tilesync.reserve((2 * band_tiles + RTW_LOG_WORDS + log_words) * sizeof(uint32_t)));
+    bool fused = false;
+    if (c->opt_resolve_fused && accel == RTW_ACCEL_BVH && !sums) {
+        const bool ldsn = c->bvh.nodes16 != nullptr && !(p->flags & RTW_FLAG_GLOBAL_NODES);
+        const void *plain = kernel_id(a, c->sc.moving != 0, accel, ldsn);
+        a.wave_log = c->scr.tilesync.as<uint32_t>();
+        fused = kernel_id(a, c->sc.moving != 0, accel, ldsn) != plain;
+        if (!fused) a.wave_log = nullptr;
+    }
 
     uint32_t per_cu = c->opt_blocks_per_cu;
     if (per_cu == 0) {
@@ -1086,18 +1101,7 @@
             const uint32_t need = (a.total_work + RTW_BLOCK - 1) / RTW_BLOCK;
             if (grid > need) grid = need ? need : 1;
         }
-        if (!sums && c->opt_tail_units > 0.0 && a.chunk_len > 1u && a.n_tiles > 1u) {
-            const double waves = (double)grid * (RTW_BLOCK / 64u);
-            const uint32_t L1 = a.chunk_len, L2 = L1 >= 12u ? 4u : (L1 >= 6u ? 2u : 1u), L3 = 1u;
-            uint64_t t3 = (uint64_t)std::ceil(c->opt_tail_units * waves * L3 / (double)a.n_samples);
-            uint64_t t2 = L2 > L3 ? (uint64_t)std::ceil(c->opt_tail_units * waves * L2 / (double)a.n_samples) : 0;
-            if (t3 > a.n_tiles / 4u) t3 = a.n_tiles / 4u;
-            if (t2 > a.n_tiles / 4u) t2 = a.n_tiles / 4u;
-            a.reg_q2 = a.n_tiles - (uint32_t)t3; a.reg_q1 = a.reg_q2 - (uint32_t)t2;
-            a.reg_len[1] = L2; a.reg_len[2] = L3;
-            for (int r = 1; r < 3; r++) a.reg_nc[r] = (a.n_samples + a.reg_len[r] - 1u) / a.reg_len[r];
-            a.total_work = (a.reg_q1 * a.reg_nc[0] + (a.reg_q2 - a.reg_q1) * a.reg_nc[1] + (a.n_tiles - a.reg_q2) * a.reg_nc[2]) * 64u;
-        }
+        if (!sums && c->opt_tail_units > 0.0 && a.chunk_len > 1u && a.n_tiles > 1u) tail_regions(a, c->opt_tail_units, (double)grid * (RTW_BLOCK / 64u));
         {
             a.sub_shift = (c->opt_sub_queues != 1u && a.n_tiles >= 64u && grid >= 64u) ? RTW_SUB_SHIFT : 0u;
             const uint32_t waves4 = (grid * (RTW_BLOCK / 64u) * 4u) >> a.sub_shift;
@@ -1107,6 +1111,11 @@
             a.grab_max = (blocks ? blocks : 1u) * 64u;
         }
         HIP_TRY(hipMemsetAsync(a.queue, 0, RTW_QUEUE_BYTES, c->stream));
+        a.done = c->scr.tilesync.as<uint32_t>(); a.resolved = a.done + a.n_tiles;
+        const size_t log_at = (2 * (size_t)a.n_tiles + RTW_LOG_WORDS - 1) / RTW_LOG_WORDS * RTW_LOG_WORDS;
+        if (fused) a.wave_log = a.done + log_at;
+        c->resolved_tiles = a.n_tiles;
+        if (a.n_tiles) HIP_TRY(hipMemsetAsync(a.done, 0, (fused ? log_at + (size_t)grid * (RTW_BLOCK / 64u) * RTW_LOG_WORDS : 2 * (size_t)a.n_tiles) * sizeof(uint32_t), c->stream));
         if (a.n_tiles) launch_render(a, c->sc.moving != 0, accel, grid, c->stream);
         HIP_TRY(hipGetLastError());
         if (tile_rows == 0) break;
@@ -1120,6 +1129,18 @@
     c->pend.enqueue_ms = std::chrono::duration<float, std::milli>(std::chrono::steady_clock::now() - c->pend.t0).count();
     if (phases & PH_COPY) return render_copy(c);
     return RTW_OK;
+}
+
+static void tail_regions(KArgs &a, double tail_units, double waves) {
+    const uint32_t L1 = a.chunk_len, L2 = L1 >= 12u ? 4u : (L1 >= 6u ? 2u : 1u), L3 = 1u;
+    uint64_t t3 = (uint64_t)std::ceil(tail_units * waves * L3 / (double)a.n_samples);
+    uint64_t t2 = L2 > L3 ? (uint64_t)std::ceil(tail_units * waves * L2 / (double)a.n_samples) : 0;
+    if (t3 > a.n_tiles / 4u) t3 = a.n_tiles / 4u;
+    if (t2 > a.n_tiles / 4u) t2 = a.n_tiles / 4u;
+    a.reg_q2 = a.n_tiles - (uint32_t)t3; a.reg_q1 = a.reg_q2 - (uint32_t)t2;
+    a.reg_len[1] = L2; a.reg_len[2] = L3;
+    for (int r = 1; r < 3; r++) a.reg_nc[r] = (a.n_samples + a.reg_len[r] - 1u) / a.reg_len[r];
+    a.total_work = (a.reg_q1 * a.reg_nc[0] + (a.reg_q2 - a.reg_q1) * a.reg_nc[1] + (a.n_tiles - a.reg_q2) * a.reg_nc[2]) * 64u;
 }
 
 static int render_copy(rtw_ctx *c) {
@@ -1220,9 +1241,33 @@
     case RTW_OPT_SUB_QUEUES:     if (!(v == 0.0 || v == 1.0)) return RTW_E_INVALID; c->opt_sub_queues = (uint32_t)v; return RTW_OK;
     case RTW_OPT_TAIL_UNITS:     if (!(v >= 0.0 && v <= 1024.0)) return RTW_E_INVALID; c->opt_tail_units = v; return RTW_OK;
     case RTW_OPT_GUIDED_LAYOUT:  if (!(v >= 0.0 && v <= 4.0 && v == (double)(uint32_t)v)) return RTW_E_INVALID; c->opt_guided_layout = (uint32_t)v; return RTW_OK;
+    case RTW_OPT_RESOLVE_FUSED:  if (!(v == 0.0 || v == 1.0)) return RTW_E_INVALID; c->opt_resolve_fused = (uint32_t)v; return RTW_OK;
     case RTW_OPT_GRAB_BLOCKS:    if (!(v >= 0.0 && v <= 65536.0 && v == (double)(uint32_t)v)) return RTW_E_INVALID; c->opt_grab_blocks = (uint32_t)v; return RTW_OK;
     default: return RTW_E_INVALID;
     }
+}
+
+int rtw_debug_queue_regions(uint32_t n_tiles, uint32_t n_samples, uint32_t chunk_len, double tail_units, uint32_t waves, uint32_t out[9]) {
+    if (!out || n_tiles == 0 || n_samples == 0 || chunk_len == 0 || chunk_len > n_samples || !(tail_units >= 0.0)) return RTW_E_INVALID;
+    KArgs a{};
+    a.n_tiles = n_tiles; a.n_samples = n_samples; a.chunk_len = chunk_len; a.n_chunks = (n_samples + chunk_len - 1) / chunk_len;
+    a.total_work = a.n_tiles * a.n_chunks * 64u;
+    a.reg_q1 = a.reg_q2 = a.n_tiles;
+    for (int r = 0; r < 3; r++) { a.reg_len[r] = a.chunk_len; a.reg_nc[r] = a.n_chunks; }
+    if (tail_units > 0.0 && a.chunk_len > 1u && a.n_tiles > 1u) tail_regions(a, tail_units, (double)waves);
+    out[0] = a.reg_q1; out[1] = a.reg_q2; out[8] = a.total_work;
+    for (int r = 0; r < 3; r++) { out[2 + r] = a.reg_len[r]; out[5 + r] = a.reg_nc[r]; }
+    return RTW_OK;
+}
+
+int rtw_ctx_debug_resolved(rtw_ctx *c, uint32_t *out, uint32_t cap, uint32_t *n_tiles) {
+    if (!c || !n_tiles || c->pend.active) return RTW_E_INVALID;
+    *n_tiles = c->resolved_tiles;
+    if (!out || cap < c->resolved_tiles || c->resolved_tiles == 0) return out && cap < c->resolved_tiles ? RTW_E_INVALID : RTW_OK;
+    HIP_TRY(hipSetDevice(c->device));
+    HIP_TRY(hipStreamSynchronize(c->stream));
+    HIP_TRY(hipMemcpy(out, c->scr.tilesync.as<uint32_t>() + c->resolved_tiles, (size_t)c->resolved_tiles * sizeof(uint32_t), hipMemcpyDeviceToHost));
+    return RTW_OK;
 }
 
 int rtw_ctx_render(rtw_ctx *c, const RtwCamera *cam, const RtwParams *p, float *out_rgb, RtwStats *stats) {
```

After: 34390. 0.902x the previous value.
